# tusen-ai/RangeDet

Hardware: AMD Instinct MI355X
Metric: range-image frames/sec (64x2650, 8ch) at 1/2/4/8 GPU; Meta-Kernel HBM GB/s vs peak (higher is better)
Workload: dtype bf16

## Files before the change

include/rangedet_hip.h:

```cpp
#ifndef RANGEDET_HIP_H_
#define RANGEDET_HIP_H_
#include <stddef.h>
#include <stdint.h>

#ifdef __cplusplus
extern "C" {
#endif

#define RD_OK 0
#define RD_EINVAL (-1)
#define RD_ESHAPE (-2)
#define RD_EWORKSPACE (-3)
#define RD_EHIP (-4)

#define RD_F32 0
#define RD_BF16 1
#define RD_F16 2

#define RD_RELU_PRE 1
#define RD_ADD 2
#define RD_RELU_POST 4
#define RD_SCALE_FOLDED 8
#define RD_MFMA16 16

int rd_version(void);
const char* rd_last_error_string(void);

int rd_nchw_to_nhwc(const float* src, void* dst, int B, int C, int H, int W, int dst_cstride, int dst_coff,
                    int zero_pad, int dst_dtype, void* stream);
int rd_nhwc_to_nchw(const void* src, float* dst, int B, int C, int H, int W, int src_cstride, int src_coff,
                    int src_dtype, void* stream);

int rd_copy_rows(const void* src, long src_row_bytes, void* dst, long dst_row_bytes, long dst_offset_bytes, long bytes,
                 int rows, void* stream);

size_t rd_conv_packed_bytes(int ntaps, int cin, int cout, int dtype);
int rd_pack_conv_weight_host(const float* w_oihw_host, int cout, int cin, int kh, int kw, int dtype,
                             void* packed_host);
int rd_deconv_phase_taps(int kh, int kw, int stride_w, int pad_w, int phase);
int rd_pack_deconv_weight_host(const float* w_iohw_host, int cin, int cout, int kh, int kw, int stride_w,
                               int pad_w, int phase, int dtype, void* packed_host);
int rd_pack_deconv_weight_folded_host(const float* w_iohw_host, const float* fold_scale_host, int cin, int cout, int kh, int kw,
                                      int stride_w, int pad_w, int phase, int dtype, void* packed_host);

int rd_conv2d_bn_act(const void* x, int x_cstride, int x_coff, const void* w_packed, const float* scale,
                     const float* shift, const void* residual, int r_cstride, int r_coff, void* y,
                     int y_cstride, int y_coff, int B, int H, int Win, int cin, int cout, int kh, int kw,
                     int stride_w, int flags, int dtype, void* stream);
size_t rd_conv3x3_ex_packed_bytes(int cin, int cout, int stride_w, int x_cstride);
int rd_pack_conv3x3_ex_host(const float* w_oihw_host, const float* fold_scale_host, int cout, int cin, int stride_w,
                            int x_cstride, int dtype, void* packed_host);
int rd_pack_conv3x3_m16_host(const float* w_oihw_host, const float* fold_scale_host, int cout, int cin, int dtype, void* packed_host);
int rd_conv3x3_mfma16_ok(int cin, int cout, int stride_w, int W, int fused_output_conv);
size_t rd_conv1x1_sc_packed_bytes(int cin, int cout);
int rd_pack_conv1x1_sc_host(const float* w_oi_host, const float* fold_scale_host, int cout, int cin, int dtype,
                            void* packed_host);
int rd_conv3x3_bn_act_ex(const void* x, int x_cstride, int x_coff, const void* w_packed, const float* scale, const float* shift,
                         const void* residual, int r_cstride, int r_coff, const void* sc_x, int sc_cstride, int sc_coff,
                         int sc_cin, const void* sc_w_packed, void* y, int y_cstride, int y_coff, int B, int H, int Win, int cin,
                         int cout, int stride_w, int flags, int dtype, void* stream);
size_t rd_block64_packed_bytes(int cin);
int rd_pack_block64_host(const float* w1_oihw_host, const float* fold_scale1_host, const float* w2_oihw_host,
                         const float* fold_scale2_host, int cin, int dtype, void* packed_host);
int rd_block64_bn_act(const void* x, int x_cstride, int x_coff, int cin, const void* w_packed, const float* shift1, const float* shift2,
                      const void* sc_w_packed, void* y, int y_cstride, int y_coff, int B, int H, int W, int dtype, void* stream);
int rd_pack_block64_m16_host(const float* w1_oihw_host, const float* fold_scale1_host, const float* w2_oihw_host,
                             const float* fold_scale2_host, int dtype, void* packed_host);
int rd_pack_conv1x1_sc_m16_host(const float* w_oi_host, const float* fold_scale_host, int dtype, void* packed_host);
int rd_block64_m16_bn_act(const void* x, int x_cstride, int x_coff, const void* w_packed, const float* shift1, const float* shift2,
                          const void* sc_w_packed, void* y, int y_cstride, int y_coff, int B, int H, int W, int dtype, void* stream);

size_t rd_head_packed_bytes(void);
int rd_pack_head_weight_host(const float* w, int nout, int cin, int dtype, void* out_host);
size_t rd_head_m16_packed_bytes(void);
int rd_pack_head_weight_m16_host(const float* w, int nout, int cin, int dtype, void* out_host);
int rd_conv2d_bn_act_head_out(const void* x, int x_cstride, int x_coff, const void* w_packed, const float* scale,
                              const float* shift, int B, int H, int W, int cin, int flags, const void* head_w_packed,
                              const float* head_bias, float* out, long out_batch_stride, long n_off, int nout, int dtype,
                              void* stream);

int rd_conv3x3_bn_act_pair(const void* x0, int x0_coff, const void* w0_packed, const float* shift0, void* y0, int y0_coff,
                           const void* x1, int x1_coff, const void* w1_packed, const float* shift1, void* y1, int y1_coff,
                           int x_cstride, int y_cstride, int B, int H, int W, int cin, int flags, int dtype, void* stream);
int rd_conv2d_bn_act_head_out_pair(const void* x0, int x0_coff, const void* w0_packed, const float* shift0, const void* head_w0_packed,
                                   const float* head_bias0, float* out0, long out0_batch_stride, int nout0,
                                   const void* x1, int x1_coff, const void* w1_packed, const float* shift1, const void* head_w1_packed,
                                   const float* head_bias1, float* out1, long out1_batch_stride, int nout1,
                                   int x_cstride, long n_off, int B, int H, int W, int cin, int flags, int dtype, void* stream);

size_t rd_conv3x3_cat_packed_bytes(int cin1, int cin2, int cout);
int rd_pack_conv3x3_cat_host(const float* w, const float* fold_scale, int cout, int cin1, int cin2, int dtype, void* out_host);
int rd_conv3x3_bn_act_cat(const void* x1, int x1_cstride, int x1_coff, int cin1, const void* x2, int x2_cstride, int x2_coff, int cin2,
                          const void* w_packed, const float* shift, void* y, int y_cstride, int y_coff, int B, int H, int W, int cout,
                          int flags, int dtype, void* stream);

int rd_deconv2d_bn_act(const void* x, int x_cstride, int x_coff, const void* w_packed_phase,
                       const float* scale, const float* shift, const void* residual, int r_cstride,
                       int r_coff, void* y, int y_cstride, int y_coff, int B, int H, int Win, int cin,
                       int cout, int kh, int kw, int stride_w, int pad_w, int phase, int flags, int dtype,
                       void* stream);

int rd_deconv2d_all_phases_ok(int kh, int kw, int stride_w, int pad_w, int cout, int dtype);
int rd_deconv2d_bn_act_all(const void* x, int x_cstride, int x_coff, const void* w_packed_all, long w_phase_bytes,
                           const float* shift, const void* residual, int r_cstride, int r_coff, void* y, int y_cstride,
                           int y_coff, int B, int H, int Win, int cin, int cout, int kh, int kw, int stride_w, int pad_w,
                           int flags, int dtype, void* stream);

int rd_deconv2d_phase_pairs_ok(int kh, int kw, int stride_w, int pad_w, int cout, int dtype);
int rd_pack_deconv_phase_pair_host(const void* phase_a, const void* phase_b, int cin, int dtype, void* out);
int rd_deconv2d_bn_act_pairs(const void* x, int x_cstride, int x_coff, const void* w_packed_pairs, long w_pair_bytes,
                             const float* shift2, const void* residual, int r_cstride, int r_coff, void* y, int y_cstride,
                             int y_coff, int B, int H, int Win, int cin, int cout, int kh, int kw, int stride_w, int pad_w,
                             int flags, int dtype, void* stream);

int rd_head_out(const void* x, int x_cstride, int x_coff, const float* w, const float* bias, float* out,
                long out_batch_stride, long n_off, int B, int H, int W, int cin, int nout, int dtype,
                void* stream);

size_t rd_meta_packed_bytes(int dtype);
int rd_pack_meta_host(const float* w0, const float* b0, const float* w1, const float* b1, const float* s1,
                      const float* t1, const float* agg, const float* s2, const float* t2, int dtype,
                      void* packed_host);
int rd_meta_kernel_fwd(const void* data, int d_cstride, int d_coff, const float* coord_nchw,
                       const void* packed, void* y, int y_cstride, int y_coff, int B, int H, int W, int dtype,
                       void* stream);

size_t rd_sorted_foreground_workspace_bytes(long N, long k);
int rd_sorted_foreground(const float* cls_score, const float* bbox_delta, const float* pc, const float* mask,
                         int B, long N, long k, int D, int apply_sigmoid, float* out_score, float* out_delta,
                         float* out_pc, int* out_idx, void* ws, size_t ws_bytes, void* stream);

int rd_decode3d_bbox(const float* bbox_delta, const float* pc, float* out, int B, long N, int box_type,
                     int is_bin, void* stream);

size_t rd_score_filter_workspace_bytes(long n);
int rd_score_filter_dets(const float* scores, const float* boxes10, long n, float min_score, float* dets,
                         int* d_count, void* ws, size_t ws_bytes, void* stream);
int rd_score_filter_dets_batched(const float* scores, long scores_bstride, const float* boxes10, long boxes_bstride,
                                 long n, float min_score, float* dets, long dets_bstride, int* d_count, void* ws,
                                 size_t ws_bytes, int B, void* stream);

#define RD_WNMS_MAX_K 65536
#define RD_TIE_STABLE 0
#define RD_TIE_REFERENCE 1
#define RD_WNMS_DIAG_NO_SKIP 0x100
#define RD_WNMS_DIAG_TILE_W(n) (((n) & 0xff) << 16)
#define RD_WNMS_DIAG_MERGE_LDS(n) (((n) & 0x7f) << 24)
size_t rd_wnms_workspace_bytes(int Kcap);
int rd_wnms_4c(const float* dets, int Kcap, const int* d_count, const int* order, int tie_order, float thresh,
               float thresh_vote, int is3d, int hash_scale, float* out_dets, int* keep, int* d_nkeep, void* ws,
               size_t ws_bytes, void* stream);
int rd_wnms_4c_batched(const float* dets, long dets_bstride, int Kcap, const int* d_count, const int* order,
                       long order_bstride, int tie_order, float thresh, float thresh_vote, int is3d, int hash_scale,
                       float* out_dets, long out_bstride, int* keep, long keep_bstride, int* d_nkeep, void* ws,
                       size_t ws_bytes, int B, void* stream);
int rd_single_overlap(const float* dets_a, const float* dets_b, long n, int is3d, float* out, void* stream);
int rd_wnms_pair_skippable(const float* dets_a, const float* dets_b, long n, unsigned char* out, void* stream);

int rd_edge_atan2f(const float* y, const float* x, long n, float* out, void* stream);

int rd_wnms_order_host(const float* dets_host, int K, int* order_host);

int rd_dets12_to_8(const float* dets12, int Mcap, const int* d_count, float* out8, void* stream);
int rd_dets12_to_8_batched(const float* dets12, long dets12_bstride, int Mcap, const int* d_count, float* out8,
                           long out8_bstride, int B, void* stream);

int rd_rotated_iou_8pt(const float* boxes1, const float* boxes2, float* ious, long n1, long n2, void* stream);
int rd_batch_rotated_iou(const float* proposal, int p_stride, const float* gt_bbox, float* iou_map, int* argmax, int B, long N,
                         int n_gt, void* stream);
int rd_batch_rotated_iou_3d(const float* proposal, int p_stride, const float* gt_bbox7, float* iou_map, int* argmax, int B, long N,
                            int n_gt, void* stream);
int rd_rotated_iou_7(const float* boxes1, const float* boxes2, float* ious, long n1, long n2, void* stream);
int rd_batch_max_iou(const float* proposals, int p_stride, const float* gt8, float* out, long n, int n_gt,
                     void* stream);

size_t rd_nms3d_workspace_bytes(long N, int B);
int rd_gather_keep_scores(const float* score, long score_bstride, int k, const int* keep_idx, int max_keep, float* out, int B,
                          void* stream);
int rd_nms3d(const float* boxes, int B, long N, float iou_thres, int max_keep, int normal_iou, int* keep_idx,
             float* bbox_after_nms, void* ws, size_t ws_bytes, void* stream);

int rd_assign3d_v2(const float* pc, const float* bbox, const float* bbox_center, const float* bbox_radius, const float* mask,
                   const float* is_in_nlz, long N, int M, float max_x, float min_x, float max_y, float min_y, float max_z,
                   float min_z, float max_dist, int* out, void* stream);
size_t rd_get_point_num_workspace_bytes(void);
int rd_get_point_num(const float* bbox_inds, long N, float* out, void* ws, size_t ws_bytes, void* stream);

typedef struct {
  float clip_lo[7], clip_hi[7];
  float mean[8], sd[8];
  float interval_lo[3], interval_hi[3];
} rd_input_norm_t;
int rd_input_transform(const float* range_image, const float* pc_vehicle_frame, const float* inclination,
                       const rd_input_norm_t* norm_host, int B, int H, int W, int Hp, int Wp, float* input_data,
                       float* coord_s1, float* pc_s1, float* pc_s2, float* pc_s4, float* mask_s1, float* mask_s2,
                       float* mask_s4, void* stream);

#define RD_PROF_CONV 0
#define RD_PROF_META 1
#define RD_PROF_HEAD_OUT 2
#define RD_PROF_SORT 3
#define RD_PROF_DECODE 4
#define RD_PROF_WNMS 5
#define RD_PROF_LAYOUT 6
#define RD_PROF_CONV3 7
#define RD_PROF_BLOCK 8
#define RD_PROF_NKINDS 9
int rd_prof_enable(int on);
int rd_prof_reset(void);
int rd_prof_get(int kind, double* total_ms, long* launches);

#ifdef __cplusplus
}
#endif
#endif
```

rangedet_amd/csrc/k_block.h:

```cpp
#pragma once
#include "k_conv3.h"

namespace rd {

struct BlockArgs {
  const bf16_t* x; int x_cs, x_co; long x_bs;
  const unsigned char* w;
  const float* shift1; const float* shift2;
  const unsigned char* scw;
  bf16_t* y; int y_cs, y_co; long y_bs;
  const unsigned char* zero16;
  int H, W, B, ncol, nrow, ntiles, xcd;
  int nslots1;
};

constexpr int BK_R = 6;
constexpr int BK_XP = 36;
constexpr int BK_XPIECES = 7;
constexpr int BK_BUF = 4 * BK_XPIECES * 1024;
constexpr int BK_TP = 34;
constexpr int BK_SLAB = 4096;
constexpr size_t BK_LDS = 2 * BK_BUF + BK_R * BK_SLAB;

constexpr int bk_nsteps(bool first) { return first ? 23 : 36; }
constexpr int bk_unit(bool first, int g) { return first ? (g < 5 ? 0 : g < 14 ? 2 : 3) : g / 9; }
constexpr int bk_ord(bool first, int g) { return first ? (g < 5 ? g : (g - 5) % 9) : g % 9; }
constexpr bool bk_fetches(bool first, int g) { return bk_unit(first, g) == 3 || (!first && bk_unit(first, g) == 0); }
constexpr int bk_pieces_u(int s) { return s <= 1 ? 2 : s <= 4 ? 1 : 0; }
constexpr int bk_first_u(int s) { int n = 0; for (int t = 0; t < s; ++t) n += bk_pieces_u(t); return n; }
constexpr int bk_pieces(bool first, int g) { return bk_fetches(first, g) ? bk_pieces_u(bk_ord(first, g)) : 0; }
constexpr int bk_younger(bool first, int g) {
  const int G = bk_nsteps(first);
  int n = BK_R - 3;
  for (int d = 1; d <= BK_R - 2; ++d) n += bk_pieces(first, ((g - d) % G + G) % G);
  const int cap = 9 - 3 - 4;
  return (bk_fetches(first, g) && bk_ord(first, g) == 7 && n > cap) ? cap : n;
}

template <int DT, bool SC, bool FIRST = false, bool M16 = false>
__global__ __launch_bounds__(256, 2) void block64_stream_kernel(BlockArgs a) {
  static_assert(!FIRST || SC, "the first block changes the channel count: projection shortcut");
  static_assert(!(FIRST && M16), "the first block (five two-tap steps on one 16-channel slot) stays in the 32 x 32 x 16 form");
  HIP_DYNAMIC_SHARED(unsigned char, smem);
  constexpr int R = BK_R, SLAB = BK_SLAB, RING = 2 * BK_BUF, NCT = 2;
  constexpr int ROWB2 = BK_TP * 64;
  const int tid = threadIdx.x, lane = tid & 63, wave = __builtin_amdgcn_readfirstlane(tid >> 6);
  const int m = lane & 31, hi = lane >> 5;

  unsigned bz1[NCT], bz2[NCT];
#pragma unroll
  for (int j = 0; j < NCT; ++j) {
    const float t1 = a.shift1[32 * j + conv_row_perm(m)], t2 = a.shift2[32 * j + conv_row_perm(m)];
    const bf16_t h1 = H16<DT>::from_f32(t1), h2 = H16<DT>::from_f32(t2);
    const bf16_t l1 = H16<DT>::from_f32(t1 - H16<DT>::to_f32(h1)), l2 = H16<DT>::from_f32(t2 - H16<DT>::to_f32(h2));
    bz1[j] = hi ? 0u : ((unsigned)h1 | ((unsigned)l1 << 16));
    bz2[j] = hi ? 0u : ((unsigned)h2 | ((unsigned)l2 << 16));
  }

  unsigned bz1m = 0u, bz2m = 0u;
  if constexpr (M16) {
    const float t1 = a.shift1[conv_row16(lane >> 4, lane & 15)], t2 = a.shift2[conv_row16(lane >> 4, lane & 15)];
    const bf16_t h1 = H16<DT>::from_f32(t1), h2 = H16<DT>::from_f32(t2);
    const bf16_t l1 = H16<DT>::from_f32(t1 - H16<DT>::to_f32(h1)), l2 = H16<DT>::from_f32(t2 - H16<DT>::to_f32(h2));
    bz1m = (unsigned)h1 | ((unsigned)l1 << 16);
    bz2m = (unsigned)h2 | ((unsigned)l2 << 16);
  }

  const int G = gridDim.x, wg = blockIdx.x;
  const int ntl = (a.ntiles - wg + G - 1) / G;
  const int tiles_img = a.ncol * a.nrow;

#if defined(__HIP_DEVICE_COMPILE__)
  const unsigned lds0 = __builtin_amdgcn_readfirstlane((unsigned)(uintptr_t)(__attribute__((address_space(3))) void*)smem);
#endif
  auto dma_s = [&](const unsigned char* sbase, unsigned voff, int lds_off) {
#if defined(__HIP_DEVICE_COMPILE__)
    asm volatile("s_mov_b32 m0, %2\n\ts_nop 0\n\tglobal_load_lds_dwordx4 %0, %1"
                 :: "v"(voff), "s"(sbase), "s"(__builtin_amdgcn_readfirstlane(lds0 + (unsigned)lds_off)) : "memory");
#else
    __builtin_amdgcn_global_load_lds(sbase + voff, smem + lds_off, 16, 0, 0);
#endif
  };
  auto dma_v = [&](const void* vptr, int lds_off) {
#if defined(__HIP_DEVICE_COMPILE__)
    asm volatile("s_mov_b32 m0, %1\n\ts_nop 0\n\tglobal_load_lds_dwordx4 %0, off"
                 :: "v"(vptr), "s"(__builtin_amdgcn_readfirstlane(lds0 + (unsigned)lds_off)) : "memory");
#else
    __builtin_amdgcn_global_load_lds(vptr, smem + lds_off, 16, 0, 0);
#endif
  };

  const int xdq = (G >> 3) / a.nrow;
  const int g_ct = a.xcd ? (8 * xdq) % a.ncol : G % a.ncol, g_rb = a.xcd ? (G >> 3) % a.nrow : (G / a.ncol) % a.nrow,
            g_b = a.xcd ? (8 * xdq) / a.ncol : G / tiles_img;
  const int g_ct1 = (8 * xdq + 8) % a.ncol, g_b1 = (8 * xdq + 8) / a.ncol;
  auto tile_advance = [&](int& ct, int& rb, int& b) __attribute__((always_inline)) {
    int& d0 = a.xcd ? rb : ct;
    int& d1 = a.xcd ? ct : rb;
    const int r0 = a.xcd ? a.nrow : a.ncol, r1 = a.xcd ? a.ncol : a.nrow;
    d0 += a.xcd ? g_rb : g_ct;
    const int c1 = d0 >= r0 ? 1 : 0;
    d0 -= c1 ? r0 : 0;
    d1 += a.xcd ? (c1 ? g_ct1 : g_ct) : g_rb + c1;
    const int c2 = d1 >= r1 ? 1 : 0;
    d1 -= c2 ? r1 : 0;
    b += (a.xcd && c1 ? g_b1 : g_b) + c2;
  };
  const int xs0 = ((wg >> 3) / a.nrow) * 8 + (wg & 7);
  int f_ct = a.xcd ? xs0 % a.ncol : wg % a.ncol, f_rb = a.xcd ? (wg >> 3) % a.nrow : (wg / a.ncol) % a.nrow,
      f_b = a.xcd ? xs0 / a.ncol : wg / tiles_img;
  int c_ct = f_ct, c_rb = f_rb, c_b = f_b;

  int hk = 0, hc = 0;
  int hh0 = 0, hw0 = 0;
  const unsigned char* htile = nullptr;
  const unsigned char* hbase = nullptr;
  bool hnew = true;
  auto halo_begin = [&]() {
    if (hnew) {
      hh0 = f_rb * 8 - 2; hw0 = f_ct * 32 - 2;
      htile = (const unsigned char*)(a.x + (size_t)f_b * a.x_bs + a.x_co) + ((long)hh0 * a.W + hw0) * (long)a.x_cs * 2;
      hnew = false;
    }
    hbase = htile + hc * 64;
    if (!FIRST && hc == 0) hc = 1;
    else if (hk + 1 < ntl) { ++hk; hc = 0; tile_advance(f_ct, f_rb, f_b); hnew = true; }
  };
  auto halo_piece = [&](int buf, int j) {
    const int q = wave * BK_XPIECES + j;
    int ol = lane;
    asm volatile("" : "+v"(ol));
    const int pp = 16 * q + (ol >> 2), r = (pp * 1821) >> 16, cc = pp - BK_XP * r;
    const int hs = (ol & 3) ^ ((ol >> 4) & 3);
    const bool ok = pp < 12 * BK_XP && (unsigned)(hh0 + r) < (unsigned)a.H && (unsigned)(hw0 + cc) < (unsigned)a.W && (!FIRST || hs < a.nslots1);
    const unsigned char* src = hbase + (long)((r * a.W + cc) * a.x_cs * 2 + hs * 16);
    dma_v(ok ? (const void*)src : (const void*)a.zero16, buf + q * 1024);
  };
  int fslot = 0, fslab = 0;
  auto slab_piece = [&]() { dma_s(a.w + (size_t)fslab * SLAB + wave * 1024, lane * 16, RING + fslot * SLAB + wave * 1024); };
  auto slab_advance = [&]() {
    fslot = fslot + 1 == R ? 0 : fslot + 1;
    fslab = fslab + 1 == bk_nsteps(FIRST) ? 0 : fslab + 1;
  };

  int a1[3][3], a2[3];
#pragma unroll
  for (int dh = 0; dh < 3; ++dh)
#pragma unroll
    for (int dw = 0; dw < 3; ++dw) {
      const int P = 96 * wave + m + BK_XP * dh + dw;
      a1[dh][dw] = P * 64 + (((hi ^ (P >> 2)) & 3) << 4);
    }
#pragma unroll
  for (int d = 0; d < 3; ++d) {
    const int c = d + m;
    a2[d] = c * 64 + (((hi ^ (c >> 2)) & 3) << 4) + wave * 2 * ROWB2;
  }
  if constexpr (M16) {
    const int n16 = lane & 15, q16 = lane >> 4;
#pragma unroll
    for (int dh = 0; dh < 3; ++dh)
#pragma unroll
      for (int dw = 0; dw < 3; ++dw) {
        const int P = 96 * wave + n16 + BK_XP * dh + dw;
        a1[dh][dw] = P * 64 + (((q16 ^ (P >> 2)) & 3) << 4);
      }
#pragma unroll
    for (int d = 0; d < 3; ++d) {
      const int c = d + n16;
      a2[d] = c * 64 + (((q16 ^ (c >> 2)) & 3) << 4) + wave * 2 * ROWB2;
    }
  }
  const int boff = RING + lane * 16;

  f32x16 acc[M16 ? 1 : 3][M16 ? 1 : NCT];
  f32x4 acc6[M16 ? 6 : 1][M16 ? 4 : 1];
  s16x8 fa[2][3], fb[2][NCT];
  s16x8 fa16[6];
#define BK_FENCE() __builtin_amdgcn_sched_barrier(0)
#define BK_RD(F, FS, BUF, K, AADDR, BADDR, KS)                                                              \
  {                                                                                                         \
    if ((K) == 0) fa[BUF][0] = *(const s16x8*)(smem + (AADDR));                                              \
    else if ((K) <= NCT) fb[BUF][(K) - 1] = *(const s16x8*)(smem + (BADDR) + ((KS) * NCT + (K) - 1) * 1024);  \
    else fa[BUF][(K) - NCT] = *(const s16x8*)(smem + (AADDR) + ((K) - NCT) * (FS));                          \
    BK_FENCE();                                                                                             \
  }
#define BK_MM(BUF, N)                                                                                       \
  {                                                                                                         \
    acc[(N) / NCT][(N) % NCT] = H16<DT>::mfma(fb[BUF][(N) % NCT], fa[BUF][(N) / NCT], acc[(N) / NCT][(N) % NCT]); \
    BK_FENCE();                                                                                             \
  }
#define BK_SYNC(VMCNT, LGKM)                                      \
  {                                                               \
    asm volatile("" ::: "memory");                                \
    __builtin_amdgcn_s_waitcnt(C3_WAIT_IMM(VMCNT, LGKM));         \
    __builtin_amdgcn_s_barrier();                                 \
    asm volatile("" ::: "memory");                                \
    BK_FENCE();                                                   \
  }
#define BK_STEP(F, FS, G_, HB_, NF_, NFS_, A1_, ANEXT_)                                                            \
  {                                                                                                                \
    constexpr int NM_ = (F) * NCT, NR_ = (F) + NCT, NRN_ = (NF_) ? (NF_) + NCT : 0;                                \
    constexpr int NH_ = bk_pieces(FIRST, G_), NP_ = 1 + NH_, HF_ = bk_first_u(bk_ord(FIRST, G_)), YG_ = bk_younger(FIRST, G_); \
    const int acur_ = (A1_);                                                                                       \
    const int bcur_ = boff + rslot * SLAB;                                                                         \
    const int rnext_ = rslot + 1 == R ? 0 : rslot + 1;                                                             \
    const int anext_ = (ANEXT_);                                                                                   \
    const int bnext_ = boff + rnext_ * SLAB;                                                                       \
    BK_FENCE();                                                                                                    \
    _Pragma("unroll") for (int n = 0; n < NM_; ++n) {                                                              \
      BK_MM(0, n)                                                                                                  \
      if (n < NR_) BK_RD(F, FS, 1, n, acur_, bcur_, 1)                                                             \
    }                                                                                                              \
    _Pragma("unroll") for (int n = 0; n < NM_ / 2; ++n) {                                                          \
      BK_MM(1, n)                                                                                                  \
      if (n < NRN_) BK_RD(NF_, NFS_, 0, n, anext_, bnext_, 0)                                                      \
    }                                                                                                              \
    { _Pragma("unroll") for (int n = NM_ / 2; n < NRN_; ++n) BK_RD(NF_, NFS_, 0, n, anext_, bnext_, 0) }           \
    BK_SYNC(YG_, NRN_)                                                                                             \
    if (NH_ > 0 && bk_ord(FIRST, G_) == 0) halo_begin();                                                           \
    _Pragma("unroll") for (int n = NM_ / 2; n < NM_; ++n) {                                                        \
      BK_MM(1, n)                                                                                                  \
      _Pragma("unroll") for (int p = 0; p < NP_; ++p)                                                              \
        if (p * (NM_ / 2) / NP_ == n - NM_ / 2) {                                                                  \
          if (p == 0) slab_piece(); else halo_piece(HB_, HF_ + p - 1);                                             \
          BK_FENCE();                                                                                              \
        }                                                                                                          \
    }                                                                                                              \
    slab_advance();                                                                                                \
    rslot = rnext_;                                                                                                \
  }
#define BK_C1(U_, S_)                                                                                              \
  BK_STEP(3, 2048, 9 * (U_) + (S_), BK_BUF, (((U_) == 1 && (S_) == 8) ? 0 : 3), 2048,                              \
          (a1[(S_) / 3][(S_) % 3] + (U_) * BK_BUF) ^ 32,                                                           \
          ((S_) == 8 ? a1[0][0] + BK_BUF : a1[(((S_) + 1) % 9) / 3][((S_) + 1) % 3] + (U_) * BK_BUF))
#define BK_P1(S_)                                                                                                  \
  BK_STEP(3, 2048, (S_), 0, ((S_) == 4 ? 0 : 3), 2048, a1[((2 * (S_) + 1) % 9) / 3][(2 * (S_) + 1) % 3],           \
          a1[((2 * (S_) + 2) % 9) / 3][(2 * (S_) + 2) % 3])
#define BK_C2(C_, S_)                                                                                              \
  BK_STEP(2, ROWB2, (FIRST ? 5 : 18) + 9 * (C_) + (S_), 0, (((C_) == 1 && (S_) == 8) ? 3 : 2), (((C_) == 1 && (S_) == 8) ? 2048 : ROWB2), \
          (a2[(S_) % 3] + ((S_) / 3) * ROWB2 + (C_) * BK_BUF) ^ 32,                                                \
          ((S_) == 8 ? ((C_) == 1 ? a1[0][0] : a2[0] + BK_BUF) : a2[((S_) + 1) % 3] + ((((S_) + 1) % 9) / 3) * ROWB2 + (C_) * BK_BUF))

#define BK_RDW16(BUF, C, BADDR) { fb[BUF][C] = *(const s16x8*)(smem + (BADDR) + (C) * 1024); BK_FENCE(); }
#define BK_RDP16(HX, AADDR, FS) { fa16[HX] = *(const s16x8*)(smem + (AADDR) + ((HX) >> 1) * (FS) + ((HX) & 1) * 1024); BK_FENCE(); }
#define BK_MM16(BK, N)                                                                                             \
  {                                                                                                                \
    acc6[(N) >> 1][2 * (BK) + ((N) & 1)] = H16<DT>::mfma16(fb[BK][(N) & 1], fa16[(N) >> 1], acc6[(N) >> 1][2 * (BK) + ((N) & 1)]); \
    BK_FENCE();                                                                                                    \
  }
#define BK_STEP16(F, G_, HB_, NF_, NFS_, ANEXT_)                                                                   \
  {                                                                                                                \
    constexpr int NM_ = 2 * (F);                                                                                   \
    constexpr int NX_ = (NF_) > (F) ? (NF_) - (F) : 0;                                                             \
    constexpr int LG_ = (NF_) ? 2 + NX_ + ((NF_) < (F) / 2 ? (NF_) : (F) / 2) : 0;                                 \
    constexpr int NH_ = bk_pieces(FIRST, G_), NP_ = 1 + NH_, HF_ = bk_first_u(bk_ord(FIRST, G_)), YG_ = bk_younger(FIRST, G_); \
    const int bcur_ = boff + rslot * SLAB;                                                                         \
    const int rnext_ = rslot + 1 == R ? 0 : rslot + 1;                                                             \
    const int anext_ = (ANEXT_);                                                                                   \
    const int bnext_ = boff + rnext_ * SLAB;                                                                       \
    BK_FENCE();                                                                                                    \
    _Pragma("unroll") for (int n = 0; n < NM_; ++n) {                                                              \
      BK_MM16(0, n)                                                                                                \
      if (n < 2) BK_RDW16(1, n, bcur_ + 2048)                                                                      \
    }                                                                                                              \
    _Pragma("unroll") for (int n = 0; n < NM_ / 2; ++n) {                                                          \
      BK_MM16(1, n)                                                                                                \
      if ((NF_) && n < 2) BK_RDW16(0, n, bnext_)                                                                   \
      if (n < NX_) BK_RDP16((F) + n, anext_, NFS_)                                                                 \
      if ((n & 1) && (n >> 1) < (NF_)) BK_RDP16(n >> 1, anext_, NFS_)                                              \
    }                                                                                                              \
    BK_SYNC(YG_, LG_)                                                                                              \
    if (NH_ > 0 && bk_ord(FIRST, G_) == 0) halo_begin();                                                           \
    _Pragma("unroll") for (int n = NM_ / 2; n < NM_; ++n) {                                                        \
      BK_MM16(1, n)                                                                                                \
      _Pragma("unroll") for (int p = 0; p < NP_; ++p)                                                              \
        if (p * (NM_ / 2) / NP_ == n - NM_ / 2) {                                                                  \
          if (p == 0) slab_piece(); else halo_piece(HB_, HF_ + p - 1);                                             \
          BK_FENCE();                                                                                              \
        }                                                                                                          \
      if ((n & 1) && (n >> 1) < (NF_) && (n >> 1) < (F)) BK_RDP16(n >> 1, anext_, NFS_)                            \
    }                                                                                                              \
    slab_advance();                                                                                                \
    rslot = rnext_;                                                                                                \
  }
#define BK_C1M(U_, S_)                                                                                             \
  BK_STEP16(6, 9 * (U_) + (S_), BK_BUF, (((U_) == 1 && (S_) == 8) ? 0 : 6), 2048,                                  \
            ((S_) == 8 ? a1[0][0] + BK_BUF : a1[(((S_) + 1) % 9) / 3][((S_) + 1) % 3] + (U_) * BK_BUF))
#define BK_C2M(C_, S_)                                                                                             \
  BK_STEP16(4, 18 + 9 * (C_) + (S_), 0, (((C_) == 1 && (S_) == 8) ? 6 : 4), (((C_) == 1 && (S_) == 8) ? 2048 : ROWB2), \
            ((S_) == 8 ? ((C_) == 1 ? a1[0][0] : a2[0] + BK_BUF) : a2[((S_) + 1) % 3] + ((((S_) + 1) % 9) / 3) * ROWB2 + (C_) * BK_BUF))

  halo_begin();
#pragma unroll
  for (int j = 0; j < BK_XPIECES; ++j) halo_piece(0, j);
#pragma unroll 1
  for (int s0 = 0; s0 < R; ++s0) { slab_piece(); slab_advance(); }
  BK_SYNC(0, 0)
  int rslot = 0;
  if constexpr (M16) {
#pragma unroll
    for (int kk = 0; kk < 2; ++kk) BK_RDW16(0, kk, boff + rslot * SLAB)
#pragma unroll
    for (int kk = 0; kk < 6; ++kk) BK_RDP16(kk, a1[0][0], 2048)
  } else {
#pragma unroll
  for (int kk = 0; kk < 3 + NCT; ++kk) BK_RD(3, 2048, 0, kk, a1[0][0], boff + rslot * SLAB, 0)
  }

  for (int k = 0; k < ntl; ++k) {
    if constexpr (M16) {
      unsigned z0 = 0u, b1 = bz1m, b2 = bz2m;
      int oq = lane >> 4;
      asm volatile("" : "+v"(z0), "+v"(b1), "+v"(b2), "+v"(oq));
      typedef short s16x2 __attribute__((ext_vector_type(2)));
      typedef float f32x2 __attribute__((ext_vector_type(2)));
      auto init_acc = [&](unsigned bz, int NH) {
#pragma unroll
        for (int cb = 0; cb < 4; ++cb) {
          unsigned ob[4] = {oq == cb ? H16<DT>::ONE * 0x10001u : z0, z0, z0, z0};
          unsigned ab[4] = {bz, z0, z0, z0};
          s16x8 ones, bzv;
          memcpy(&ones, ob, 16);
          memcpy(&bzv, ab, 16);
          acc6[0][cb] = H16<DT>::mfma16(bzv, ones, f32x4{});
          BK_FENCE();
        }
#pragma unroll
        for (int h = 1; h < 6; ++h)
          if (h < NH) {
#pragma unroll
            for (int cb = 0; cb < 4; ++cb) acc6[h][cb] = acc6[0][cb];
          }
        BK_FENCE();
      };
      init_acc(b1, 6);
      BK_C1M(0, 0) BK_C1M(0, 1) BK_C1M(0, 2) BK_C1M(0, 3) BK_C1M(0, 4) BK_C1M(0, 5) BK_C1M(0, 6) BK_C1M(0, 7) BK_C1M(0, 8)
      BK_C1M(1, 0) BK_C1M(1, 1) BK_C1M(1, 2) BK_C1M(1, 3) BK_C1M(1, 4) BK_C1M(1, 5) BK_C1M(1, 6) BK_C1M(1, 7) BK_C1M(1, 8)
      const int ct = c_ct, rb = c_rb, b = c_b;
      tile_advance(c_ct, c_rb, c_b);
      {
        int el = lane;
        asm volatile("" : "+v"(el));
        const int en = el & 15, eq = el >> 4;
#pragma unroll
        for (int h = 0; h < 6; ++h) {
          const int J = 96 * wave + 16 * h + en, rr = (J * 1821) >> 16, cc = J - BK_XP * rr;
          const bool keep = cc < BK_TP && rr < 10;
          const bool inside = (unsigned)(rb * 8 - 1 + rr) < (unsigned)a.H && (unsigned)(ct * 32 - 1 + cc) < (unsigned)a.W;
          const int doff = (rr * BK_TP + cc) * 64 + (((eq ^ (cc >> 2)) & 3) << 4);
#pragma unroll
          for (int j = 0; j < 2; ++j) {
            BK_FENCE();
            unsigned pk[4];
#pragma unroll
            for (int w2 = 0; w2 < 4; ++w2) {
              const f32x4 av = acc6[h][2 * j + (w2 >> 1)];
              unsigned p2 = H16<DT>::pk(av[2 * (w2 & 1)], av[2 * (w2 & 1) + 1]);
              p2 = __builtin_bit_cast(unsigned, __builtin_elementwise_max(__builtin_bit_cast(s16x2, p2), (s16x2){0, 0}));
              pk[w2] = inside ? p2 : 0u;
            }
            if (keep) *(Slot16*)(smem + j * BK_BUF + doff) = Slot16{pk[0], pk[1], pk[2], pk[3]};
          }
        }
      }
      init_acc(b2, 4);
      BK_SYNC(63, 0)
#pragma unroll
      for (int kk = 0; kk < 2; ++kk) BK_RDW16(0, kk, boff + rslot * SLAB)
#pragma unroll
      for (int kk = 0; kk < 4; ++kk) BK_RDP16(kk, a2[0], ROWB2)
      BK_C2M(0, 0) BK_C2M(0, 1) BK_C2M(0, 2) BK_C2M(0, 3) BK_C2M(0, 4) BK_C2M(0, 5) BK_C2M(0, 6) BK_C2M(0, 7) BK_C2M(0, 8)
      BK_C2M(1, 0) BK_C2M(1, 1) BK_C2M(1, 2) BK_C2M(1, 3) BK_C2M(1, 4) BK_C2M(1, 5) BK_C2M(1, 6) BK_C2M(1, 7) BK_C2M(1, 8)
      {
        const int oh0 = rb * 8 + 2 * wave;
        int el = lane;
        asm volatile("" : "+v"(el));
        const int en = el & 15, eq = el >> 4;
        unsigned char* scr = smem + BK_BUF + wave * (BK_BUF / 4);
        bf16_t* __restrict__ yrow0 = a.y + (size_t)b * a.y_bs + (size_t)oh0 * a.W * a.y_cs + a.y_co;
        const bf16_t* __restrict__ rimg0 = a.x + (size_t)b * a.x_bs + a.x_co;
        if constexpr (SC) {
          const unsigned char* __restrict__ wq = a.scw + el * 16;
          s16x8 sxq[4][2];
#pragma unroll
          for (int h = 0; h < 4; ++h) {
            const int ow = ct * 32 + 16 * (h & 1) + en, oh = oh0 + (h >> 1);
            const bool live = ow < a.W && oh < a.H;
            const bf16_t* sp = rimg0 + (live ? ((size_t)oh * a.W + ow) * a.x_cs : 0) + 8 * eq;
#pragma unroll
            for (int ks = 0; ks < 2; ++ks) sxq[h][ks] = *(const s16x8*)(sp + 32 * ks);
          }
#pragma unroll
          for (int ks = 0; ks < 2; ++ks)
#pragma unroll
            for (int cb = 0; cb < 4; ++cb) {
              const s16x8 wf = *(const s16x8*)(wq + (size_t)(ks * 4 + cb) * 1024);
#pragma unroll
              for (int h = 0; h < 4; ++h) acc6[h][cb] = H16<DT>::mfma16(wf, sxq[h][ks], acc6[h][cb]);
            }
          BK_FENCE();
        }
        Slot16 rv[2][2][2];
        auto res_load = [&](int i, Slot16 (&dst)[2][2]) {
#pragma unroll
          for (int hf = 0; hf < 2; ++hf) {
            const int ow = ct * 32 + 16 * hf + en, oh = oh0 + i;
            const bool live = ow < a.W && oh < a.H;
            const bf16_t* rp = rimg0 + (live ? ((size_t)oh * a.W + (size_t)ow) * a.x_cs : 0) + 8 * eq;
#pragma unroll
            for (int p2 = 0; p2 < 2; ++p2) dst[hf][p2] = *(const Slot16*)(rp + 32 * p2);
          }
        };
        if constexpr (!SC) res_load(0, rv[0]);
#pragma unroll
        for (int i = 0; i < 2; ++i) {
          if constexpr (!SC) { if (i + 1 < 2) res_load(i + 1, rv[(i + 1) & 1]); }
#pragma unroll
          for (int hf = 0; hf < 2; ++hf)
#pragma unroll
            for (int p2 = 0; p2 < 2; ++p2) {
              BK_FENCE();
              unsigned pk[4];
#pragma unroll
              for (int w2 = 0; w2 < 4; ++w2) {
                const f32x4 av = acc6[2 * i + hf][2 * p2 + (w2 >> 1)];
                f32x2 v = {av[2 * (w2 & 1)], av[2 * (w2 & 1) + 1]};
                if constexpr (!SC) v += H16<DT>::unpk(rv[i & 1][hf][p2][w2]);
                const unsigned q2 = H16<DT>::pk(v[0], v[1]);
                pk[w2] = __builtin_bit_cast(unsigned, __builtin_elementwise_max(__builtin_bit_cast(s16x2, q2), (s16x2){0, 0}));
              }
              const int px = 16 * hf + en;
              *(Slot16*)(scr + px * 128 + (((4 * p2 + eq) ^ (px & 7)) << 4)) = Slot16{pk[0], pk[1], pk[2], pk[3]};
            }
          BK_FENCE();
          __builtin_amdgcn_wave_barrier();
#pragma unroll
          for (int it = 0; it < 4; ++it) {
            const int pr = it * 8 + el / 8, sl = el % 8;
            const Slot16 v = *(const Slot16*)(scr + pr * 128 + ((sl ^ (pr & 7)) << 4));
            const int ows = ct * 32 + pr;
            if (ows < a.W && oh0 + i < a.H)
              __builtin_nontemporal_store(v, (Slot16*)(yrow0 + (size_t)i * a.W * a.y_cs + (size_t)ows * a.y_cs + sl * 8));
          }
          __builtin_amdgcn_wave_barrier();
          BK_FENCE();
        }
      }
    } else {
    unsigned z0 = 0u;
    asm volatile("" : "+v"(z0));
    const unsigned one2 = hi ? z0 : H16<DT>::ONE * 0x10001u;
    s16x8 ones;
    {
      unsigned ob[4] = {one2, z0, z0, z0};
      memcpy(&ones, ob, 16);
    }
#pragma unroll
    for (int n = 0; n < 3 * NCT; ++n) {
      unsigned ab[4] = {bz1[n % NCT], z0, z0, z0};
      s16x8 bz;
      memcpy(&bz, ab, 16);
      acc[n / NCT][n % NCT] = H16<DT>::mfma(bz, ones, f32x16{});
    }
    BK_FENCE();
    if constexpr (FIRST) {
      BK_P1(0) BK_P1(1) BK_P1(2) BK_P1(3) BK_P1(4)
    } else {
      BK_C1(0, 0) BK_C1(0, 1) BK_C1(0, 2) BK_C1(0, 3) BK_C1(0, 4) BK_C1(0, 5) BK_C1(0, 6) BK_C1(0, 7) BK_C1(0, 8)
      BK_C1(1, 0) BK_C1(1, 1) BK_C1(1, 2) BK_C1(1, 3) BK_C1(1, 4) BK_C1(1, 5) BK_C1(1, 6) BK_C1(1, 7) BK_C1(1, 8)
    }

    const int ct = c_ct, rb = c_rb, b = c_b;
    tile_advance(c_ct, c_rb, c_b);
    {
      int em = m, ehi = hi;
      asm volatile("" : "+v"(em), "+v"(ehi));
      typedef short s16x2 __attribute__((ext_vector_type(2)));
#pragma unroll
      for (int i = 0; i < 3; ++i) {
        const int J = 96 * wave + 32 * i + em, rr = (J * 1821) >> 16, cc = J - BK_XP * rr;
        const bool keep = cc < BK_TP && rr < 10;
        const bool inside = (unsigned)(rb * 8 - 1 + rr) < (unsigned)a.H && (unsigned)(ct * 32 - 1 + cc) < (unsigned)a.W;
        const int doff = (rr * BK_TP + cc) * 64 + ((((2 * ehi) ^ (cc >> 2)) & 3) << 4);
#pragma unroll
        for (int j = 0; j < NCT; ++j) {
          BK_FENCE();
          unsigned pk[8];
#pragma unroll
          for (int q = 0; q < 8; ++q) {
            unsigned p2 = H16<DT>::pk(acc[i][j][2 * q], acc[i][j][2 * q + 1]);
            p2 = __builtin_bit_cast(unsigned, __builtin_elementwise_max(__builtin_bit_cast(s16x2, p2), (s16x2){0, 0}));
            pk[q] = inside ? p2 : 0u;
          }
          if (keep) {
            *(Slot16*)(smem + j * BK_BUF + doff) = Slot16{pk[0], pk[1], pk[2], pk[3]};
            *(Slot16*)(smem + j * BK_BUF + (doff ^ 16)) = Slot16{pk[4], pk[5], pk[6], pk[7]};
          }
        }
      }
    }
#pragma unroll
    for (int n = 0; n < 2 * NCT; ++n) {
      unsigned ab[4] = {bz2[n % NCT], z0, z0, z0};
      s16x8 bz;
      memcpy(&bz, ab, 16);
      acc[n / NCT][n % NCT] = H16<DT>::mfma(bz, ones, f32x16{});
    }
    BK_FENCE();
    BK_SYNC(63, 0)
#pragma unroll
    for (int kk = 0; kk < 2 + NCT; ++kk) BK_RD(2, ROWB2, 0, kk, a2[0], boff + rslot * SLAB, 0)
    BK_C2(0, 0) BK_C2(0, 1) BK_C2(0, 2) BK_C2(0, 3) BK_C2(0, 4) BK_C2(0, 5) BK_C2(0, 6) BK_C2(0, 7) BK_C2(0, 8)
    BK_C2(1, 0) BK_C2(1, 1) BK_C2(1, 2) BK_C2(1, 3) BK_C2(1, 4) BK_C2(1, 5) BK_C2(1, 6) BK_C2(1, 7) BK_C2(1, 8)

    {
      const int oh0 = rb * 8 + 2 * wave;
      int em = m, ehi = hi, el = lane;
      asm volatile("" : "+v"(em), "+v"(ehi), "+v"(el));
      typedef float f32x2 __attribute__((ext_vector_type(2)));
      typedef short s16x2 __attribute__((ext_vector_type(2)));
      unsigned char* scr = smem + BK_BUF + wave * (BK_BUF / 4);
      bf16_t* __restrict__ yrow0 = a.y + (size_t)b * a.y_bs + (size_t)oh0 * a.W * a.y_cs + a.y_co;
      const bf16_t* __restrict__ rimg0 = a.x + (size_t)b * a.x_bs + a.x_co;
      if constexpr (SC) {
        const bf16_t* __restrict__ sb = a.x + (size_t)b * a.x_bs + a.x_co + 8 * ehi;
        const unsigned char* __restrict__ wq = a.scw + el * 16;
        constexpr int SNK = FIRST ? 1 : 4;
        s16x8 sxq[2][SNK];
#pragma unroll
        for (int i = 0; i < 2; ++i) {
          const int ow = ct * 32 + em, oh = oh0 + i;
          const bool live = ow < a.W && oh < a.H;
          const bf16_t* sp = sb + (live ? ((size_t)oh * a.W + ow) * a.x_cs : 0);
#pragma unroll
          for (int ks = 0; ks < SNK; ++ks) sxq[i][ks] = *(const s16x8*)(sp + 16 * ks);
        }
#pragma unroll
        for (int ks = 0; ks < SNK; ++ks)
#pragma unroll
          for (int j = 0; j < NCT; ++j) {
            const s16x8 wf = *(const s16x8*)(wq + (size_t)(ks * NCT + j) * 1024);
#pragma unroll
            for (int i = 0; i < 2; ++i) acc[i][j] = H16<DT>::mfma(wf, sxq[i][ks], acc[i][j]);
          }
        BK_FENCE();
      }
      Slot16 rv[2][NCT][2];
      auto res_load = [&](int i, Slot16 (&dst)[NCT][2]) {
        const int ow = ct * 32 + em, oh = oh0 + i;
        const bool live = ow < a.W && oh < a.H;
        const bf16_t* rp = rimg0 + (live ? ((size_t)oh * a.W + (size_t)ow) * a.x_cs : 0) + 16 * ehi;
#pragma unroll
        for (int j = 0; j < NCT; ++j) {
          dst[j][0] = *(const Slot16*)(rp + j * 32);
          dst[j][1] = *(const Slot16*)(rp + j * 32 + 8);
        }
      };
      if constexpr (!SC) res_load(0, rv[0]);
#pragma unroll
      for (int i = 0; i < 2; ++i) {
        if constexpr (!SC) { if (i + 1 < 2) res_load(i + 1, rv[(i + 1) & 1]); }
#pragma unroll
        for (int j = 0; j < NCT; ++j) {
          BK_FENCE();
          const int cb = j * 32 + 16 * ehi;
          unsigned pk[8];
#pragma unroll
          for (int q = 0; q < 8; ++q) {
            f32x2 v = {acc[i][j][2 * q], acc[i][j][2 * q + 1]};
            if constexpr (!SC) v += H16<DT>::unpk(rv[i & 1][j][q >> 2][q & 3]);
            unsigned p2 = H16<DT>::pk(v[0], v[1]);
            pk[q] = __builtin_bit_cast(unsigned, __builtin_elementwise_max(__builtin_bit_cast(s16x2, p2), (s16x2){0, 0}));
          }
#pragma unroll
          for (int u = 0; u < 2; ++u)
            *(Slot16*)(scr + em * 128 + ((((cb >> 3) + u) ^ (em & 7)) << 4)) = Slot16{pk[4 * u], pk[4 * u + 1], pk[4 * u + 2], pk[4 * u + 3]};
        }
        BK_FENCE();
        __builtin_amdgcn_wave_barrier();
#pragma unroll
        for (int it = 0; it < 4; ++it) {
          const int pr = it * 8 + el / 8, sl = el % 8;
          const Slot16 v = *(const Slot16*)(scr + pr * 128 + ((sl ^ (pr & 7)) << 4));
          const int ows = ct * 32 + pr;
          if (ows < a.W && oh0 + i < a.H)
            __builtin_nontemporal_store(v, (Slot16*)(yrow0 + (size_t)i * a.W * a.y_cs + (size_t)ows * a.y_cs + sl * 8));
        }
        __builtin_amdgcn_wave_barrier();
        BK_FENCE();
      }
    }
    }
  }
  __builtin_amdgcn_s_waitcnt(RD_VMCNT_IMM(0));
#undef BK_C2M
#undef BK_C1M
#undef BK_STEP16
#undef BK_MM16
#undef BK_RDP16
#undef BK_RDW16
#undef BK_C2
#undef BK_P1
#undef BK_C1
#undef BK_STEP
#undef BK_SYNC
#undef BK_MM
#undef BK_RD
#undef BK_FENCE
}

inline bool block64_first(int cin) { return cin <= 16; }
inline size_t block64_body_bytes(int cin) { return (size_t)bk_nsteps(block64_first(cin)) * BK_SLAB; }
inline size_t block64_packed_bytes(int cin) { return block64_body_bytes(cin) + RD_CONV_TAIL; }
inline void pack_block64_m16(const float* w1, const float* s1, const float* w2, const float* s2, int dt, void* out) {
  memset(out, 0, block64_packed_bytes(64));
  pack_taps_frag16(9, 64, 64, out, [&](int co, int ci, int t) { return (s1 ? s1[co] : 1.f) * w1[((size_t)co * 64 + ci) * 9 + t]; }, dt);
  pack_taps_frag16(9, 64, 64, (unsigned char*)out + 18 * BK_SLAB, [&](int co, int ci, int t) { return (s2 ? s2[co] : 1.f) * w2[((size_t)co * 64 + ci) * 9 + t]; }, dt);
}
inline void pack_sc_frag16(const float* w, const float* scale, void* out, int dt = RD_BF16) {
  bf16_t* o = (bf16_t*)out;
  for (int ks = 0; ks < 2; ++ks)
    for (int cb = 0; cb < 4; ++cb)
      for (int lane = 0; lane < 64; ++lane) {
        const int co = conv_row16(cb, lane & 15);
        for (int j = 0; j < 8; ++j) {
          const int ci = 32 * ks + 8 * (lane >> 4) + j;
          *o++ = h16_from_f32(dt, (scale ? scale[co] : 1.f) * w[(size_t)co * 64 + ci]);
        }
      }
}
inline void pack_block64(const float* w1, const float* s1, const float* w2, const float* s2, int cin, int dt, void* out) {
  memset(out, 0, block64_packed_bytes(cin));
  if (block64_first(cin))
    pack_body_frag(3, cin, 64, out, [&](int co, int ci, int dh, int dw) { return (s1 ? s1[co] : 1.f) * w1[(((size_t)co * cin + ci) * 3 + dh) * 3 + dw]; }, dt);
  else
    pack_taps_frag(9, 64, 64, out, [&](int co, int ci, int t) { return (s1 ? s1[co] : 1.f) * w1[((size_t)co * 64 + ci) * 9 + t]; }, dt);
  pack_taps_frag(9, 64, 64, (unsigned char*)out + block64_body_bytes(cin) - 18 * BK_SLAB,
                 [&](int co, int ci, int t) { return (s2 ? s2[co] : 1.f) * w2[((size_t)co * 64 + ci) * 9 + t]; }, dt);
}

inline int launch_block64(const void* x, int x_cs, int x_co, int cin, const void* w, const float* shift1, const float* shift2, const void* sc_w,
                          void* y, int y_cs, int y_co, int B, int H, int W, int dt, hipStream_t st, bool m16 = false) {
  RD_REQUIRE(is_h16(dt), RD_EINVAL, "block64: dtype %d (RD_BF16 or RD_F16)", dt);
  const bool first = block64_first(cin);
  RD_REQUIRE(!m16 || !first, RD_ESHAPE, "block64: the 16 x 16 x 32 form takes 64 input channels");
  RD_REQUIRE(cin == 64 || (first && cin >= 1), RD_ESHAPE, "block64: %d input channels (64, or at most 16 for the network's first block)", cin);
  RD_REQUIRE(!first || sc_w, RD_EINVAL, "block64: a block that changes the channel count needs its projection shortcut");
  BlockArgs a;
  memset(&a, 0, sizeof(a));
  a.x = (const bf16_t*)x; a.x_cs = x_cs; a.x_co = x_co; a.x_bs = (long)H * W * x_cs;
  a.w = (const unsigned char*)w; a.shift1 = shift1; a.shift2 = shift2; a.scw = (const unsigned char*)sc_w;
  a.y = (bf16_t*)y; a.y_cs = y_cs; a.y_co = y_co; a.y_bs = (long)H * W * y_cs;
  a.zero16 = (const unsigned char*)w + block64_body_bytes(cin);
  a.H = H; a.W = W; a.B = B;
  a.nslots1 = std::min(2, (x_cs - x_co) / 8);
  a.ncol = (W + 31) / 32; a.nrow = (H + 7) / 8; a.ntiles = a.ncol * a.nrow * B;
  const int grid = std::min(a.ntiles, conv_num_cus() * 2);
  a.xcd = dev_switches().conv_xcd && (a.ncol * B) % 8 == 0 && grid % 8 == 0;
  ProfScope ps(RD_PROF_BLOCK, st);
  static std::atomic<unsigned long long> seen{0};
  once_per_device(seen, [] {
    allow_big_lds(block64_stream_kernel<RD_F16, false>); allow_big_lds(block64_stream_kernel<RD_BF16, false>);
    allow_big_lds(block64_stream_kernel<RD_F16, true>); allow_big_lds(block64_stream_kernel<RD_BF16, true>);
    allow_big_lds(block64_stream_kernel<RD_F16, true, true>); allow_big_lds(block64_stream_kernel<RD_BF16, true, true>);
    allow_big_lds(block64_stream_kernel<RD_F16, false, false, true>); allow_big_lds(block64_stream_kernel<RD_BF16, false, false, true>);
    allow_big_lds(block64_stream_kernel<RD_F16, true, false, true>); allow_big_lds(block64_stream_kernel<RD_BF16, true, false, true>);
  });
#define BK_GO(DT_)                                                                                                         \
  {                                                                                                                        \
    if (m16 && sc_w) hipLaunchKernelGGL((block64_stream_kernel<DT_, true, false, true>), dim3(grid), dim3(256), BK_LDS, st, a);  \
    else if (m16) hipLaunchKernelGGL((block64_stream_kernel<DT_, false, false, true>), dim3(grid), dim3(256), BK_LDS, st, a);    \
    else if (first) hipLaunchKernelGGL((block64_stream_kernel<DT_, true, true>), dim3(grid), dim3(256), BK_LDS, st, a);    \
    else if (sc_w) hipLaunchKernelGGL((block64_stream_kernel<DT_, true>), dim3(grid), dim3(256), BK_LDS, st, a);           \
    else hipLaunchKernelGGL((block64_stream_kernel<DT_, false>), dim3(grid), dim3(256), BK_LDS, st, a);                    \
  }
  if (dt == RD_F16) BK_GO(RD_F16) else BK_GO(RD_BF16)
#undef BK_GO
  return check_launch("block64_stream_kernel");
}

}
```

rangedet_amd/csrc/rd_api.hip:

```cpp
#include "k_conv1.h"
#include "k_block.h"
#include "k_assign.h"
#include "k_input.h"
#include "k_nms3d.h"
#include "k_meta.h"
#include "k_misc.h"
#include "k_riou.h"
#include "k_sort.h"
#include "k_wnms.h"

#include <algorithm>
#include <string>
#include <numeric>

using namespace rd;

namespace rd {
inline size_t align256(size_t v) { return (v + 255) & ~(size_t)255; }
inline size_t wnms_ws_bytes(int cap) {
  const size_t nw = (size_t)(cap + 63) / 64;
  return align256((size_t)cap * PREP_F * 4) + 3 * align256((size_t)cap * nw * 8) + 4 * align256((size_t)cap * 4) +
         align256(((size_t)cap + 2) * 8 + 3 * ((size_t)cap / 32 + 2) * 4) + align256(nw * 8) + 256 + align256(sort_ws_bytes(cap)) + 256;
}
inline WnmsWs wnms_ws_carve(void* ws, int cap) {
  WnmsWs w;
  const size_t nw = (size_t)(cap + 63) / 64;
  unsigned char* p = (unsigned char*)(((uintptr_t)ws + 255) & ~(uintptr_t)255);
  w.nwcap = (int)nw;
  w.prep = (float*)p; p += align256((size_t)cap * PREP_F * 4);
  w.thr = (unsigned long long*)p; p += align256((size_t)cap * nw * 8);
  w.vote = (unsigned long long*)p; p += align256((size_t)cap * nw * 8);
  w.snap = (unsigned long long*)p; p += align256((size_t)cap * nw * 8);
  w.keep_q = (int*)p; p += align256((size_t)cap * 4);
  w.order = (int*)p; p += align256((size_t)cap * 4);
  w.alive = (int*)p; p += align256((size_t)cap * 4);
  w.ovf = (int*)p; p += align256((size_t)cap * 4);
  w.scratch = (int*)p; p += align256(((size_t)cap + 2) * 8 + 3 * ((size_t)cap / 32 + 2) * 4);
  w.supp_state = (unsigned long long*)p; p += align256(nw * 8);
  w.nalive = (int*)p; w.novf = (int*)p + 1; p += 256;
  w.sort_ws = p;
  return w;
}
inline void allow_conv_lds() {
  static std::atomic<unsigned long long> seen{0};
  once_per_device(seen, [] {
    allow_big_lds(conv_taps_kernel<RD_BF16, 4, 3>); allow_big_lds(conv_taps_kernel<RD_BF16, 4, 8>);
    allow_big_lds(conv_taps_kernel<RD_F16, 4, 3>); allow_big_lds(conv_taps_kernel<RD_F16, 4, 8>);
    allow_big_lds(conv_taps_kernel<RD_F32, 4, 8>); allow_big_lds(conv_taps_kernel<RD_F32, 4, 3>);
  });
}
}

extern "C" {

int rd_version(void) { return 100; }
const char* rd_last_error_string(void) { return rd::err_buf(); }

int rd_nchw_to_nhwc(const float* src, void* dst, int B, int C, int H, int W, int dst_cstride, int dst_coff,
                    int zero_pad, int dst_dtype, void* stream) {
  RD_REQUIRE(src && dst, RD_EINVAL, "nchw_to_nhwc: null pointer");
  RD_REQUIRE(B > 0 && C > 0 && H > 0 && W > 0 && zero_pad >= 0, RD_ESHAPE, "nchw_to_nhwc: bad shape");
  RD_REQUIRE(dst_coff >= 0 && dst_coff + C + zero_pad <= dst_cstride, RD_ESHAPE, "nchw_to_nhwc: channels exceed stride");
  hipStream_t st = (hipStream_t)stream;
  const long HW = (long)H * W, total = (long)B * (C + zero_pad) * HW;
  const int grid = (int)std::min<long>((total + 255) / 256, 8192);
  ProfScope ps(RD_PROF_LAYOUT, st);
  {
    const int ch = ch_per_slot(dst_dtype), ctot = C + zero_pad;
    if ((is_h16(dst_dtype) || dst_dtype == RD_F32) && ctot % ch == 0 && ctot / ch <= 2 && dst_cstride % ch == 0 && dst_coff % ch == 0) {
      const long npix = (long)B * HW;
      const int g2 = (int)std::min<long>((npix + 255) / 256, 8192);
#define RD_PX(DT, NS) hipLaunchKernelGGL((nchw_to_nhwc_px_kernel<DT, NS>), dim3(g2), dim3(256), 0, st, src, dst, C, HW, dst_cstride, dst_coff, npix)
      if (dst_dtype == RD_BF16) { if (ctot / ch == 1) RD_PX(RD_BF16, 1); else RD_PX(RD_BF16, 2); }
      else if (dst_dtype == RD_F16) { if (ctot / ch == 1) RD_PX(RD_F16, 1); else RD_PX(RD_F16, 2); }
      else { if (ctot / ch == 1) RD_PX(RD_F32, 1); else RD_PX(RD_F32, 2); }
#undef RD_PX
      return check_launch("nchw_to_nhwc");
    }
  }
  if (dst_dtype == RD_BF16)
    hipLaunchKernelGGL(nchw_to_nhwc_kernel<RD_BF16>, dim3(grid), dim3(256), 0, st, src, dst, C, HW, dst_cstride, dst_coff, zero_pad, total);
  else if (dst_dtype == RD_F16)
    hipLaunchKernelGGL(nchw_to_nhwc_kernel<RD_F16>, dim3(grid), dim3(256), 0, st, src, dst, C, HW, dst_cstride, dst_coff, zero_pad, total);
  else if (dst_dtype == RD_F32)
    hipLaunchKernelGGL(nchw_to_nhwc_kernel<RD_F32>, dim3(grid), dim3(256), 0, st, src, dst, C, HW, dst_cstride, dst_coff, zero_pad, total);
  else
    return rd::fail(RD_EINVAL, "nchw_to_nhwc: dtype %d", dst_dtype);
  return check_launch("nchw_to_nhwc");
}
int rd_copy_rows(const void* src, long src_row_bytes, void* dst, long dst_row_bytes, long dst_offset_bytes, long bytes,
                 int rows, void* stream) {
  RD_REQUIRE(src && dst, RD_EINVAL, "copy_rows: null pointer");
  RD_REQUIRE(rows > 0 && bytes > 0 && src_row_bytes >= bytes && dst_row_bytes >= dst_offset_bytes + bytes && dst_offset_bytes >= 0,
             RD_ESHAPE, "copy_rows: bad geometry");
  ProfScope ps(RD_PROF_LAYOUT, (hipStream_t)stream);
  if (hipMemcpy2DAsync((char*)dst + dst_offset_bytes, (size_t)dst_row_bytes, src, (size_t)src_row_bytes, (size_t)bytes,
                       (size_t)rows, hipMemcpyDeviceToDevice, (hipStream_t)stream) != hipSuccess)
    return rd::fail(RD_EHIP, "copy_rows: hipMemcpy2DAsync failed");
  return RD_OK;
}
int rd_nhwc_to_nchw(const void* src, float* dst, int B, int C, int H, int W, int src_cstride, int src_coff,
                    int src_dtype, void* stream) {
  RD_REQUIRE(src && dst, RD_EINVAL, "nhwc_to_nchw: null pointer");
  RD_REQUIRE(B > 0 && C > 0 && H > 0 && W > 0, RD_ESHAPE, "nhwc_to_nchw: bad shape");
  RD_REQUIRE(src_coff >= 0 && src_coff + C <= src_cstride, RD_ESHAPE, "nhwc_to_nchw: channels exceed stride");
  hipStream_t st = (hipStream_t)stream;
  const long HW = (long)H * W, total = (long)B * C * HW;
  const int grid = (int)std::min<long>((total + 255) / 256, 8192);
  ProfScope ps(RD_PROF_LAYOUT, st);
  if (src_dtype == RD_BF16)
    hipLaunchKernelGGL(nhwc_to_nchw_kernel<RD_BF16>, dim3(grid), dim3(256), 0, st, src, dst, C, HW, src_cstride, src_coff, total);
  else if (src_dtype == RD_F16)
    hipLaunchKernelGGL(nhwc_to_nchw_kernel<RD_F16>, dim3(grid), dim3(256), 0, st, src, dst, C, HW, src_cstride, src_coff, total);
  else if (src_dtype == RD_F32)
    hipLaunchKernelGGL(nhwc_to_nchw_kernel<RD_F32>, dim3(grid), dim3(256), 0, st, src, dst, C, HW, src_cstride, src_coff, total);
  else
    return rd::fail(RD_EINVAL, "nhwc_to_nchw: dtype %d", src_dtype);
  return check_launch("nhwc_to_nchw");
}

size_t rd_conv_packed_bytes(int ntaps, int cin, int cout, int dtype) { return conv_packed_bytes(ntaps, cin, cout, dtype); }
int rd_pack_conv_weight_host(const float* w, int cout, int cin, int kh, int kw, int dtype, void* out) {
  RD_REQUIRE(w && out, RD_EINVAL, "pack_conv: null pointer");
  RD_REQUIRE(dtype == RD_F32 || is_h16(dtype), RD_EINVAL, "pack_conv: dtype");
  RD_REQUIRE(kh * kw >= 1 && kh * kw <= 9 && (kh & 1) && (kw & 1), RD_ESHAPE, "pack_conv: kernel (%d,%d)", kh, kw);
  TapList tl = conv_taps(kh, kw);
  auto get = [&](int co, int ci, int t) { return w[(((size_t)co * cin + ci) * kh + tl.kh[t]) * kw + tl.kw[t]]; };
  memset(out, 0, conv_packed_bytes(tl.n, cin, cout, dtype));
  if (is_h16(dtype)) pack_taps_frag(tl.n, cin, cout, out, get, dtype);
  else pack_taps(tl.n, cin, cout, dtype, out, get);
  return RD_OK;
}
static bool deconv_embeds_3x3(const TapList& tl) {
  for (int t = 0; t < tl.n; ++t)
    if (tl.dh[t] < -1 || tl.dh[t] > 1 || tl.dw[t] < -1 || tl.dw[t] > 1) return false;
  return tl.n >= 1 && tl.n <= 9;
}
static int deconv_tap_set(const TapList& tl) {
  if (tl.n != 6 || !deconv_embeds_3x3(tl)) return 0;
  for (int ts = 1; ts <= 2; ++ts) {
    bool seen[6] = {false, false, false, false, false, false};
    bool ok = true;
    for (int t = 0; t < 6 && ok; ++t) {
      const int c = tl.dw[t] - (ts == 1 ? -1 : 0);
      if (c < 0 || c > 1) ok = false;
      else seen[(tl.dh[t] + 1) * 2 + c] = true;
    }
    for (int i = 0; i < 6 && ok; ++i) ok = seen[i];
    if (ok) return ts;
  }
  return 0;
}
static TapList deconv_taps_sorted(int kh, int kw, int s, int pad_w, int phase) {
  TapList tl = deconv_taps(kh, kw, s, pad_w, phase);
  if (tl.n > 9) return tl;
  for (int i = 1; i < tl.n; ++i)
    for (int j = i; j > 0 && (tl.dh[j] < tl.dh[j - 1] || (tl.dh[j] == tl.dh[j - 1] && tl.dw[j] < tl.dw[j - 1])); --j) {
      std::swap(tl.dh[j], tl.dh[j - 1]); std::swap(tl.dw[j], tl.dw[j - 1]);
      std::swap(tl.kh[j], tl.kh[j - 1]); std::swap(tl.kw[j], tl.kw[j - 1]);
    }
  return tl;
}
int rd_deconv_phase_taps(int kh, int kw, int stride_w, int pad_w, int phase) {
  if (stride_w < 1 || phase < 0 || phase >= stride_w) return RD_EINVAL;
  TapList tl = deconv_taps(kh, kw, stride_w, pad_w, phase);
  if (tl.n > 9) return RD_ESHAPE;
  return (deconv_embeds_3x3(tl) && !deconv_tap_set(tl)) ? 9 : tl.n;
}
int rd_pack_deconv_weight_host(const float* w, int cin, int cout, int kh, int kw, int stride_w, int pad_w,
                               int phase, int dtype, void* out) {
  return rd_pack_deconv_weight_folded_host(w, nullptr, cin, cout, kh, kw, stride_w, pad_w, phase, dtype, out);
}
int rd_pack_deconv_weight_folded_host(const float* w, const float* fold_scale, int cin, int cout, int kh, int kw, int stride_w,
                                      int pad_w, int phase, int dtype, void* out) {
  RD_REQUIRE(w && out, RD_EINVAL, "pack_deconv: null pointer");
  RD_REQUIRE(dtype == RD_F32 || is_h16(dtype), RD_EINVAL, "pack_deconv: dtype");
  RD_REQUIRE(stride_w >= 1 && phase >= 0 && phase < stride_w, RD_EINVAL, "pack_deconv: phase");
  TapList tl = deconv_taps_sorted(kh, kw, stride_w, pad_w, phase);
  RD_REQUIRE(tl.n >= 1 && tl.n <= 9, RD_ESHAPE, "pack_deconv: %d taps", tl.n);
  const bool emb = deconv_embeds_3x3(tl) && !deconv_tap_set(tl);
  auto get = [&](int co, int ci, int t) -> float {
    if (emb) {
      int src = -1;
      for (int u = 0; u < tl.n; ++u)
        if (tl.dh[u] == t / 3 - 1 && tl.dw[u] == t % 3 - 1) src = u;
      if (src < 0) return 0.f;
      t = src;
    }
    return (fold_scale ? fold_scale[co] : 1.f) * w[(((size_t)ci * cout + co) * kh + tl.kh[t]) * kw + tl.kw[t]];
  };
  const int nt = emb ? 9 : tl.n;
  memset(out, 0, conv_packed_bytes(nt, cin, cout, dtype));
  if (is_h16(dtype)) pack_taps_frag(nt, cin, cout, out, get, dtype);
  else pack_taps(nt, cin, cout, dtype, out, get);
  return RD_OK;
}

int rd_conv2d_bn_act(const void* x, int x_cstride, int x_coff, const void* w_packed, const float* scale,
                     const float* shift, const void* residual, int r_cstride, int r_coff, void* y, int y_cstride,
                     int y_coff, int B, int H, int Win, int cin, int cout, int kh, int kw, int stride_w, int flags,
                     int dtype, void* stream) {
  RD_REQUIRE(x && w_packed && y, RD_EINVAL, "conv2d: null pointer");
  RD_REQUIRE((kh == 1 && kw == 1) || (kh == 3 && kw == 3), RD_ESHAPE, "conv2d: kernel (%d,%d) not in {1x1,3x3}", kh, kw);
  RD_REQUIRE(stride_w == 1 || stride_w == 2, RD_ESHAPE, "conv2d: stride_w %d", stride_w);
  RD_REQUIRE(y_coff >= 0 && y_coff + cout <= y_cstride, RD_ESHAPE, "conv2d: y channels exceed stride");
  const int pad = (kw - 1) / 2;
  const int Wout = (Win + 2 * pad - kw) / stride_w + 1;
  RD_REQUIRE(!(flags & RD_SCALE_FOLDED), RD_EINVAL, "conv2d: RD_SCALE_FOLDED is taken by rd_conv3x3_bn_act_ex / rd_conv2d_bn_act_head_out / rd_deconv2d_bn_act");
  TapList tl = conv_taps(kh, kw);
  allow_conv_lds();
  return launch_conv(tl, x, x_cstride, x_coff, w_packed, scale, shift, residual, r_cstride, r_coff, y, y_cstride,
                     y_coff, B, H, Win, Wout, Wout, cin, cout, stride_w, 1, 0, flags, dtype, (hipStream_t)stream);
}
static int ex_view_cin(int cin, int x_cstride, int stride_w) { return stride_w == 2 ? x_cstride + cin : cin; }
size_t rd_conv3x3_ex_packed_bytes(int cin, int cout, int stride_w, int x_cstride) {
  return conv_packed_bytes(stride_w == 2 ? 6 : 9, ex_view_cin(cin, x_cstride, stride_w), cout, RD_BF16);
}
int rd_pack_conv3x3_ex_host(const float* w, const float* fold_scale, int cout, int cin, int stride_w, int x_cstride, int dtype,
                            void* out) {
  RD_REQUIRE(w && out, RD_EINVAL, "pack_conv3x3_ex: null pointer");
  RD_REQUIRE(is_h16(dtype), RD_EINVAL, "pack_conv3x3_ex: dtype %d (RD_BF16 or RD_F16)", dtype);
  RD_REQUIRE(stride_w == 1 || stride_w == 2, RD_ESHAPE, "pack_conv3x3_ex: stride_w %d", stride_w);
  RD_REQUIRE(cout == 64 || cout == 128, RD_ESHAPE, "pack_conv3x3_ex: cout %d", cout);
  RD_REQUIRE(stride_w == 1 || (x_cstride >= cin && x_cstride % 8 == 0), RD_ESHAPE, "pack_conv3x3_ex: x_cstride %d for cin %d", x_cstride, cin);
  auto wv = [&](int co, int ci, int dh, int dw) {
    return (fold_scale ? fold_scale[co] : 1.f) * w[(((size_t)co * cin + ci) * 3 + (dh + 1)) * 3 + (dw + 1)];
  };
  memset(out, 0, rd_conv3x3_ex_packed_bytes(cin, cout, stride_w, x_cstride));
  auto wv2 = [&](int co, int c2, int dh, int dw2) -> float {
    if (c2 < cin) return dw2 == 0 ? wv(co, c2, dh, 0) : 0.f;
    if (c2 >= x_cstride && c2 - x_cstride < cin) return wv(co, c2 - x_cstride, dh, dw2 == -1 ? -1 : 1);
    return 0.f;
  };
  if (stride_w == 1) {
    if (conv3_body_small(cin, fold_scale != nullptr))
      pack_body_frag(3, cin, cout, out, [&](int co, int ci, int dh, int dw) { return wv(co, ci, dh - 1, dw - 1); }, dtype);
    else
      pack_taps_frag(9, cin, cout, out, [&](int co, int ci, int t) { return wv(co, ci, t / 3 - 1, t % 3 - 1); }, dtype);
  } else if (conv3_body_s2(cin, x_cstride, fold_scale != nullptr)) {
    pack_body_frag(1, x_cstride + cin, cout, out, [&](int co, int c2, int dh, int dw) { return wv2(co, c2, dh - 1, dw - 1); }, dtype);
  } else {
    pack_taps_frag(6, x_cstride + cin, cout, out, [&](int co, int c2, int s) -> float { return wv2(co, c2, s / 2 - 1, s % 2 - 1); }, dtype);
  }
  return RD_OK;
}
int rd_pack_conv3x3_m16_host(const float* w, const float* fold_scale, int cout, int cin, int dtype, void* out) {
  RD_REQUIRE(w && out, RD_EINVAL, "pack_conv3x3_m16: null pointer");
  RD_REQUIRE(is_h16(dtype), RD_EINVAL, "pack_conv3x3_m16: dtype %d (RD_BF16 or RD_F16)", dtype);
  RD_REQUIRE(cout == 128 && cin >= 32 && cin % 32 == 0, RD_ESHAPE, "pack_conv3x3_m16: cout %d (128), cin %d (a multiple of 32)", cout, cin);
  memset(out, 0, rd_conv3x3_ex_packed_bytes(cin, cout, 1, cin));
  pack_taps_frag16(9, cin, cout, out, [&](int co, int ci, int t) {
    return (fold_scale ? fold_scale[co] : 1.f) * w[(((size_t)co * cin + ci) * 3 + t / 3) * 3 + t % 3];
  }, dtype);
  return RD_OK;
}
int rd_conv3x3_mfma16_ok(int cin, int cout, int stride_w, int W, int fused_output_conv) {
  return conv3_mfma16_ok(cin, cout, stride_w, W, fused_output_conv != 0) ? 1 : 0;
}
size_t rd_conv1x1_sc_packed_bytes(int cin, int cout) { return sc_frag_bytes(cin, cout); }
int rd_pack_conv1x1_sc_host(const float* w, const float* fold_scale, int cout, int cin, int dtype, void* out) {
  RD_REQUIRE(w && out, RD_EINVAL, "pack_conv1x1_sc: null pointer");
  RD_REQUIRE(is_h16(dtype), RD_EINVAL, "pack_conv1x1_sc: dtype %d (RD_BF16 or RD_F16)", dtype);
  RD_REQUIRE((cout == 64 || cout == 128) && cin >= 1 && cin <= 128, RD_ESHAPE, "pack_conv1x1_sc: cout %d, cin %d (1..128)", cout, cin);
  pack_sc_frag(w, fold_scale, cin, cout, out, dtype);
  return RD_OK;
}
int rd_conv3x3_bn_act_ex(const void* x, int x_cstride, int x_coff, const void* w_packed, const float* scale, const float* shift,
                         const void* residual, int r_cstride, int r_coff, const void* sc_x, int sc_cstride, int sc_coff,
                         int sc_cin, const void* sc_w_packed, void* y, int y_cstride, int y_coff, int B, int H, int Win, int cin,
                         int cout, int stride_w, int flags, int dtype, void* stream) {
  RD_REQUIRE(x && w_packed && y, RD_EINVAL, "conv3x3_ex: null pointer");
  RD_REQUIRE(is_h16(dtype), RD_EINVAL, "conv3x3_ex: dtype %d (RD_BF16 or RD_F16)", dtype);
  RD_REQUIRE(B > 0 && H > 0 && Win > 0 && cin > 0 && (cout == 64 || cout == 128), RD_ESHAPE, "conv3x3_ex: shape / cout %d", cout);
  RD_REQUIRE(stride_w == 1 || (stride_w == 2 && Win % 2 == 0), RD_ESHAPE, "conv3x3_ex: stride_w %d with Win %d (stride 2 needs an even width)", stride_w, Win);
  RD_REQUIRE(y_coff >= 0 && y_coff + cout <= y_cstride, RD_ESHAPE, "conv3x3_ex: y channels exceed stride");
  RD_REQUIRE(x_cstride % 8 == 0 && x_coff % 8 == 0 && x_coff + cin_slots(cin, RD_BF16) * 8 <= x_cstride, RD_ESHAPE, "conv3x3_ex: x channel stride/offset");
  RD_REQUIRE(!(sc_x && residual) && !(sc_x && !sc_w_packed), RD_EINVAL, "conv3x3_ex: shortcut conv and residual are exclusive");
  RD_REQUIRE(!((flags & RD_ADD) && !residual && !sc_x), RD_EINVAL, "conv3x3_ex: RD_ADD without residual / shortcut");
  RD_REQUIRE(!dev_switches().conv_v1, RD_EINVAL, "conv3x3_ex: needs the persistent 3x3 kernel (RD_CONV_V1 is set)");
  allow_conv_lds();
  const int v = stride_w;
  const int Wv = Win / v;
  Conv3Args e;
  memset(&e, 0, sizeof(e));
  int fl = flags;
  if (sc_x) {
    RD_REQUIRE(sc_cin >= 1 && sc_cin <= 128 && sc_cstride % 8 == 0 && sc_coff % 8 == 0 && sc_coff + ((sc_cin + 15) / 16) * 16 <= sc_cstride,
               RD_ESHAPE, "conv3x3_ex: shortcut input channels %d (stride %d, offset %d)", sc_cin, sc_cstride, sc_coff);
    e.sx = (const bf16_t*)sc_x; e.s_cs = sc_cstride * v; e.s_co = sc_coff; e.s_bs = (long)H * Wv * sc_cstride * v;
    e.scw = (const unsigned char*)sc_w_packed; e.s_nks = (sc_cin + 15) / 16;
    fl &= ~RD_ADD;
    fl |= RD_SCALE_FOLDED;
  }
  RD_REQUIRE(!(fl & RD_SCALE_FOLDED) || !scale, RD_EINVAL, "conv3x3_ex: folded weights take no scale array");
  const bool m16 = (fl & RD_MFMA16) != 0;
  fl &= ~RD_MFMA16;
  const bool folded = (fl & RD_SCALE_FOLDED) != 0;
  RD_REQUIRE(!m16 || (folded && !sc_x && conv3_mfma16_ok(cin, cout, stride_w, Win, false)), RD_ESHAPE,
             "conv3x3_ex: RD_MFMA16 takes folded weights of rd_pack_conv3x3_m16_host: stride 1, cout 128, cin a multiple of 32, no fused shortcut (rd_conv3x3_mfma16_ok)");
  const int body = m16 ? C3_BODY_M16 : stride_w == 2 ? conv3_body_s2(cin, x_cstride, folded) : (sc_x ? 0 : conv3_body_small(cin, folded));
  RD_REQUIRE(!(stride_w == 1 && sc_x && conv3_body_small(cin, folded)), RD_ESHAPE, "conv3x3_ex: at most 16 input channels together with a fused shortcut is not a launch form");
  return launch_conv3(x, x_cstride * v, x_coff, w_packed, scale, shift, residual, r_cstride, r_coff, y, y_cstride, y_coff, B, H,
                      Wv, ex_view_cin(cin, x_cstride, stride_w), cout, fl, 1, (hipStream_t)stream, stride_w == 2 ? 1 : 0,
                      sc_x ? &e : nullptr, dtype, nullptr, nullptr, nullptr, body);
}

size_t rd_block64_packed_bytes(int cin) { return block64_packed_bytes(cin); }
int rd_pack_block64_host(const float* w1, const float* fold_scale1, const float* w2, const float* fold_scale2, int cin, int dtype, void* out) {
  RD_REQUIRE(w1 && w2 && out, RD_EINVAL, "pack_block64: null pointer");
  RD_REQUIRE(is_h16(dtype), RD_EINVAL, "pack_block64: dtype %d (RD_BF16 or RD_F16)", dtype);
  RD_REQUIRE(cin == 64 || (cin >= 1 && cin <= 16), RD_ESHAPE, "pack_block64: %d input channels (64, or at most 16)", cin);
  pack_block64(w1, fold_scale1, w2, fold_scale2, cin, dtype, out);
  return RD_OK;
}
int rd_block64_bn_act(const void* x, int x_cstride, int x_coff, int cin, const void* w_packed, const float* shift1, const float* shift2,
                      const void* sc_w_packed, void* y, int y_cstride, int y_coff, int B, int H, int W, int dtype, void* stream) {
  RD_REQUIRE(x && w_packed && shift1 && shift2 && y, RD_EINVAL, "block64: null pointer");
  RD_REQUIRE(is_h16(dtype), RD_EINVAL, "block64: dtype %d (RD_BF16 or RD_F16)", dtype);
  RD_REQUIRE(B > 0 && H > 0 && W > 0, RD_ESHAPE, "block64: shape");
  RD_REQUIRE(cin == 64 || (cin >= 1 && cin <= 16), RD_ESHAPE, "block64: %d input channels (64, or at most 16 for the network's first block)", cin);
  RD_REQUIRE(x_cstride % 8 == 0 && x_coff % 8 == 0 && x_coff >= 0 && x_coff + cin_slots(cin, RD_BF16) * 8 <= x_cstride, RD_ESHAPE, "block64: x channel stride / offset");
  RD_REQUIRE(cin > 16 || x_coff + 16 <= x_cstride, RD_ESHAPE, "block64: the first block reads 16 channels per pixel (x_coff %d + 16 > x_cstride %d)", x_coff, x_cstride);
  RD_REQUIRE(y_cstride % 8 == 0 && y_coff % 8 == 0 && y_coff >= 0 && y_coff + 64 <= y_cstride, RD_ESHAPE, "block64: y channel stride / offset");
  RD_REQUIRE(x != y, RD_EINVAL, "block64: in-place (a tile's halo is another tile's output)");
  return launch_block64(x, x_cstride, x_coff, cin, w_packed, shift1, shift2, sc_w_packed, y, y_cstride, y_coff, B, H, W, dtype, (hipStream_t)stream);
}

int rd_pack_block64_m16_host(const float* w1, const float* fold_scale1, const float* w2, const float* fold_scale2, int dtype, void* out) {
  RD_REQUIRE(w1 && w2 && out, RD_EINVAL, "pack_block64_m16: null pointer");
  RD_REQUIRE(is_h16(dtype), RD_EINVAL, "pack_block64_m16: dtype %d (RD_BF16 or RD_F16)", dtype);
  pack_block64_m16(w1, fold_scale1, w2, fold_scale2, dtype, out);
  return RD_OK;
}
int rd_pack_conv1x1_sc_m16_host(const float* w, const float* fold_scale, int dtype, void* out) {
  RD_REQUIRE(w && out, RD_EINVAL, "pack_conv1x1_sc_m16: null pointer");
  RD_REQUIRE(is_h16(dtype), RD_EINVAL, "pack_conv1x1_sc_m16: dtype %d (RD_BF16 or RD_F16)", dtype);
  pack_sc_frag16(w, fold_scale, out, dtype);
  return RD_OK;
}
int rd_block64_m16_bn_act(const void* x, int x_cstride, int x_coff, const void* w_packed, const float* shift1, const float* shift2,
                          const void* sc_w_packed, void* y, int y_cstride, int y_coff, int B, int H, int W, int dtype, void* stream) {
  RD_REQUIRE(x && w_packed && shift1 && shift2 && y, RD_EINVAL, "block64_m16: null pointer");
  RD_REQUIRE(is_h16(dtype), RD_EINVAL, "block64_m16: dtype %d (RD_BF16 or RD_F16)", dtype);
  RD_REQUIRE(B > 0 && H > 0 && W > 0, RD_ESHAPE, "block64_m16: shape");
  RD_REQUIRE(x_cstride % 8 == 0 && x_coff % 8 == 0 && x_coff >= 0 && x_coff + 64 <= x_cstride, RD_ESHAPE, "block64_m16: x channel stride / offset");
  RD_REQUIRE(y_cstride % 8 == 0 && y_coff % 8 == 0 && y_coff >= 0 && y_coff + 64 <= y_cstride, RD_ESHAPE, "block64_m16: y channel stride / offset");
  RD_REQUIRE(x != y, RD_EINVAL, "block64_m16: in-place (a tile's halo is another tile's output)");
  return launch_block64(x, x_cstride, x_coff, 64, w_packed, shift1, shift2, sc_w_packed, y, y_cstride, y_coff, B, H, W, dtype, (hipStream_t)stream, true);
}

size_t rd_conv3x3_cat_packed_bytes(int cin1, int cin2, int cout) { return conv_packed_bytes(9, cin1 + cin2, cout, RD_BF16); }
int rd_pack_conv3x3_cat_host(const float* w, const float* fold_scale, int cout, int cin1, int cin2, int dtype, void* out) {
  RD_REQUIRE(w && out, RD_EINVAL, "pack_conv3x3_cat: null pointer");
  RD_REQUIRE(is_h16(dtype), RD_EINVAL, "pack_conv3x3_cat: dtype %d (RD_BF16 or RD_F16)", dtype);
  RD_REQUIRE((cout == 64 || cout == 128) && cin1 > 0 && cin1 % 32 == 0 && cin2 > 0 && cin2 % 8 == 0, RD_ESHAPE,
             "pack_conv3x3_cat: cout %d, cin1 %d (multiple of 32), cin2 %d (multiple of 8)", cout, cin1, cin2);
  const int cin = cin1 + cin2;
  auto wv = [&](int co, int ci, int dh, int dw) {
    return (fold_scale ? fold_scale[co] : 1.f) * w[(((size_t)co * cin + ci) * 3 + (dh + 1)) * 3 + (dw + 1)];
  };
  memset(out, 0, rd_conv3x3_cat_packed_bytes(cin1, cin2, cout));
  const int body = conv3_body_cat(cin1, cin2, fold_scale != nullptr);
  if (body) pack_body_frag(body, cin, cout, out, [&](int co, int ci, int dh, int dw) { return wv(co, ci, dh - 1, dw - 1); }, dtype);
  else pack_taps_frag(9, cin, cout, out, [&](int co, int ci, int t) { return wv(co, ci, t / 3 - 1, t % 3 - 1); }, dtype);
  return RD_OK;
}
int rd_conv3x3_bn_act_cat(const void* x1, int x1_cstride, int x1_coff, int cin1, const void* x2, int x2_cstride, int x2_coff, int cin2,
                          const void* w_packed, const float* shift, void* y, int y_cstride, int y_coff, int B, int H, int W, int cout,
                          int flags, int dtype, void* stream) {
  RD_REQUIRE(x1 && x2 && w_packed && y && shift, RD_EINVAL, "conv3x3_cat: null pointer");
  RD_REQUIRE(is_h16(dtype), RD_EINVAL, "conv3x3_cat: dtype %d (RD_BF16 or RD_F16)", dtype);
  RD_REQUIRE((flags & RD_SCALE_FOLDED) && !(flags & RD_ADD), RD_EINVAL, "conv3x3_cat: needs RD_SCALE_FOLDED weights, takes no residual");
  RD_REQUIRE(B > 0 && H > 0 && W > 0 && (cout == 64 || cout == 128), RD_ESHAPE, "conv3x3_cat: shape / cout %d", cout);
  RD_REQUIRE(cin1 > 0 && cin1 % 32 == 0 && cin2 > 0 && cin2 % 8 == 0, RD_ESHAPE, "conv3x3_cat: cin1 %d (multiple of 32), cin2 %d (multiple of 8)", cin1, cin2);
  RD_REQUIRE(y_coff >= 0 && y_coff + cout <= y_cstride, RD_ESHAPE, "conv3x3_cat: y channels exceed stride");
  RD_REQUIRE(x1_cstride % 8 == 0 && x1_coff % 8 == 0 && x1_coff + cin1 <= x1_cstride && x2_cstride % 8 == 0 && x2_coff % 8 == 0 &&
             x2_coff + cin2 <= x2_cstride, RD_ESHAPE, "conv3x3_cat: channel stride/offset");
  const DevSwitches& sw_ = dev_switches();
  RD_REQUIRE(!sw_.conv_v1 && sw_.conv_wide && sw_.conv_w30 && (cout == 64 ? sw_.conv_th4 != 3 : (sw_.conv_th4 && sw_.conv_w30 == 2)), RD_ESHAPE,
             "conv3x3_cat: needs the 8 x 32 tile form of the persistent 3x3 kernel (a dev switch turned it off)");
  allow_conv_lds();
  Conv3Src2 s2;
  s2.x = x2; s2.cs = x2_cstride; s2.co = x2_coff; s2.cin1 = cin1; s2.cin2 = cin2;
  return launch_conv3(x1, x1_cstride, x1_coff, w_packed, nullptr, shift, nullptr, 0, 0, y, y_cstride, y_coff, B, H, W, cin1 + cin2, cout, flags,
                      1, (hipStream_t)stream, 0, nullptr, dtype, nullptr, nullptr, &s2, conv3_body_cat(cin1, cin2, true));
}

size_t rd_head_packed_bytes(void) { return 16384; }
int rd_pack_head_weight_host(const float* w, int nout, int cin, int dtype, void* out_host) {
  RD_REQUIRE(w && out_host, RD_EINVAL, "pack_head_weight: null pointer");
  RD_REQUIRE(is_h16(dtype), RD_EINVAL, "pack_head_weight: dtype %d (RD_BF16 or RD_F16)", dtype);
  RD_REQUIRE(nout >= 1 && nout <= 8 && cin >= 1 && cin <= 128, RD_ESHAPE, "pack_head_weight: nout %d (1..8), cin %d (1..128)", nout, cin);
  pack_head_frag(w, nout, cin, out_host, dtype);
  return RD_OK;
}
size_t rd_head_m16_packed_bytes(void) { return 8192; }
int rd_pack_head_weight_m16_host(const float* w, int nout, int cin, int dtype, void* out_host) {
  RD_REQUIRE(w && out_host, RD_EINVAL, "pack_head_weight_m16: null pointer");
  RD_REQUIRE(is_h16(dtype), RD_EINVAL, "pack_head_weight_m16: dtype %d (RD_BF16 or RD_F16)", dtype);
  RD_REQUIRE(nout >= 1 && nout <= 8 && cin >= 1 && cin <= 128, RD_ESHAPE, "pack_head_weight_m16: nout %d (1..8), cin %d (1..128)", nout, cin);
  pack_head_frag16(w, nout, cin, out_host, dtype);
  return RD_OK;
}
int rd_conv2d_bn_act_head_out(const void* x, int x_cstride, int x_coff, const void* w_packed, const float* scale,
                              const float* shift, int B, int H, int W, int cin, int flags, const void* head_w_packed,
                              const float* head_bias, float* out, long out_batch_stride, long n_off, int nout, int dtype,
                              void* stream) {
  RD_REQUIRE(x && w_packed && head_w_packed && head_bias && out, RD_EINVAL, "conv2d_head_out: null pointer");
  RD_REQUIRE(is_h16(dtype), RD_EINVAL, "conv2d_head_out: dtype %d (RD_BF16 or RD_F16)", dtype);
  RD_REQUIRE(B > 0 && H > 0 && W > 0 && cin > 0 && nout >= 1 && nout <= 8, RD_ESHAPE, "conv2d_head_out: shape / nout %d (1..8)", nout);
  RD_REQUIRE(!(flags & RD_ADD), RD_EINVAL, "conv2d_head_out: no residual in a head tower");
  RD_REQUIRE(x_cstride % 8 == 0 && x_coff % 8 == 0 && x_coff + cin_slots(cin, RD_BF16) * 8 <= x_cstride, RD_ESHAPE,
             "conv2d_head_out: x channel stride/offset");
  RD_REQUIRE(!dev_switches().conv_v1, RD_EINVAL, "conv2d_head_out: needs the persistent 3x3 kernel (RD_CONV_V1 is set)");
  RD_REQUIRE(!conv3_body_small(cin, (flags & RD_SCALE_FOLDED) != 0), RD_ESHAPE, "conv2d_head_out: cin %d (the packed image of a conv with <= 16 input channels is not this launch form's)", cin);
  const bool m16 = (flags & RD_MFMA16) != 0;
  RD_REQUIRE(!m16 || ((flags & RD_SCALE_FOLDED) && conv3_mfma16_ok(cin, 128, 1, W, true)), RD_ESHAPE,
             "conv2d_head_out: RD_MFMA16 (weights of rd_pack_conv3x3_m16_host) is not a launch form for cin %d at width %d (rd_conv3x3_mfma16_ok)", cin, W);
  allow_conv_lds();
  Conv3Args h;
  memset(&h, 0, sizeof(h));
  h.hw = (const unsigned char*)head_w_packed; h.hb = head_bias; h.ho = out; h.ho_bs = out_batch_stride; h.ho_off = n_off; h.hn = nout;
  return launch_conv3(x, x_cstride, x_coff, w_packed, scale, shift, nullptr, 0, 0, nullptr, 128, 0, B, H, W, cin, 128, flags & ~RD_MFMA16, 1,
                      (hipStream_t)stream, 0, &h, dtype, nullptr, nullptr, nullptr, m16 ? C3_BODY_M16 : 0);
}

static int pair_checks(const char* fn, const void* x0, const void* x1, const void* w0, const void* w1, const float* shift0,
                       const float* shift1, int x_cstride, int x0_coff, int x1_coff, int B, int H, int W, int cin, int flags,
                       int dtype) {
  RD_REQUIRE(x0 && x1 && w0 && w1 && shift0 && shift1, RD_EINVAL, "%s: null pointer", fn);
  RD_REQUIRE(is_h16(dtype), RD_EINVAL, "%s: dtype %d (RD_BF16 or RD_F16)", fn, dtype);
  RD_REQUIRE(B > 0 && H > 0 && W > 0 && cin > 0, RD_ESHAPE, "%s: shape", fn);
  RD_REQUIRE((flags & RD_SCALE_FOLDED) && !(flags & RD_ADD), RD_EINVAL, "%s: needs RD_SCALE_FOLDED weights, takes no residual", fn);
  RD_REQUIRE(x_cstride % 8 == 0 && x0_coff % 8 == 0 && x1_coff % 8 == 0 && x0_coff + cin_slots(cin, RD_BF16) * 8 <= x_cstride &&
             x1_coff + cin_slots(cin, RD_BF16) * 8 <= x_cstride, RD_ESHAPE, "%s: x channel stride/offset", fn);
  RD_REQUIRE(!dev_switches().conv_v1, RD_EINVAL, "%s: needs the persistent 3x3 kernel (RD_CONV_V1 is set)", fn);
  RD_REQUIRE(cin > 16, RD_ESHAPE, "%s: cin %d (more than 16 input channels)", fn, cin);
  return RD_OK;
}
int rd_conv3x3_bn_act_pair(const void* x0, int x0_coff, const void* w0_packed, const float* shift0, void* y0, int y0_coff,
                           const void* x1, int x1_coff, const void* w1_packed, const float* shift1, void* y1, int y1_coff,
                           int x_cstride, int y_cstride, int B, int H, int W, int cin, int flags, int dtype, void* stream) {
  if (int rc = pair_checks("conv3x3_pair", x0, x1, w0_packed, w1_packed, shift0, shift1, x_cstride, x0_coff, x1_coff, B, H, W, cin, flags, dtype)) return rc;
  RD_REQUIRE(y0 && y1, RD_EINVAL, "conv3x3_pair: null output");
  RD_REQUIRE(y0_coff >= 0 && y1_coff >= 0 && y0_coff + 128 <= y_cstride && y1_coff + 128 <= y_cstride, RD_ESHAPE, "conv3x3_pair: y channels exceed stride");
  allow_conv_lds();
  if (!conv3_pair_eligible(128, flags, W)) {
    if (int rc = launch_conv3(x0, x_cstride, x0_coff, w0_packed, nullptr, shift0, nullptr, 0, 0, y0, y_cstride, y0_coff, B, H, W, cin, 128,
                              flags, 1, (hipStream_t)stream, 0, nullptr, dtype)) return rc;
    return launch_conv3(x1, x_cstride, x1_coff, w1_packed, nullptr, shift1, nullptr, 0, 0, y1, y_cstride, y1_coff, B, H, W, cin, 128, flags, 1,
                        (hipStream_t)stream, 0, nullptr, dtype);
  }
  Conv3Second g;
  memset(&g, 0, sizeof(g));
  g.x = x1; g.x_co = x1_coff; g.w = w1_packed; g.shift = shift1; g.y = y1; g.y_co = y1_coff;
  return launch_conv3(x0, x_cstride, x0_coff, w0_packed, nullptr, shift0, nullptr, 0, 0, y0, y_cstride, y0_coff, B, H, W, cin, 128, flags, 1,
                      (hipStream_t)stream, 0, nullptr, dtype, &g);
}
int rd_conv2d_bn_act_head_out_pair(const void* x0, int x0_coff, const void* w0_packed, const float* shift0, const void* head_w0_packed,
                                   const float* head_bias0, float* out0, long out0_batch_stride, int nout0,
                                   const void* x1, int x1_coff, const void* w1_packed, const float* shift1, const void* head_w1_packed,
                                   const float* head_bias1, float* out1, long out1_batch_stride, int nout1,
                                   int x_cstride, long n_off, int B, int H, int W, int cin, int flags, int dtype, void* stream) {
  if (int rc = pair_checks("conv2d_head_out_pair", x0, x1, w0_packed, w1_packed, shift0, shift1, x_cstride, x0_coff, x1_coff, B, H, W, cin, flags, dtype)) return rc;
  RD_REQUIRE(head_w0_packed && head_w1_packed && head_bias0 && head_bias1 && out0 && out1, RD_EINVAL, "conv2d_head_out_pair: null pointer");
  RD_REQUIRE(nout0 >= 1 && nout0 <= 8 && nout1 >= 1 && nout1 <= 8, RD_ESHAPE, "conv2d_head_out_pair: nout %d / %d (1..8)", nout0, nout1);
  allow_conv_lds();
  Conv3Args h;
  memset(&h, 0, sizeof(h));
  h.hw = (const unsigned char*)head_w0_packed; h.hb = head_bias0; h.ho = out0; h.ho_bs = out0_batch_stride; h.ho_off = n_off; h.hn = nout0;
  if (!conv3_pair_eligible(128, flags, W, true)) {
    if (int rc = launch_conv3(x0, x_cstride, x0_coff, w0_packed, nullptr, shift0, nullptr, 0, 0, nullptr, 128, 0, B, H, W, cin, 128, flags, 1,
                              (hipStream_t)stream, 0, &h, dtype)) return rc;
    h.hw = (const unsigned char*)head_w1_packed; h.hb = head_bias1; h.ho = out1; h.ho_bs = out1_batch_stride; h.hn = nout1;
    return launch_conv3(x1, x_cstride, x1_coff, w1_packed, nullptr, shift1, nullptr, 0, 0, nullptr, 128, 0, B, H, W, cin, 128, flags, 1,
                        (hipStream_t)stream, 0, &h, dtype);
  }
  Conv3Second g;
  memset(&g, 0, sizeof(g));
  g.x = x1; g.x_co = x1_coff; g.w = w1_packed; g.shift = shift1;
  g.hw = head_w1_packed; g.hb = head_bias1; g.ho = out1; g.ho_bs = out1_batch_stride; g.hn = nout1;
  return launch_conv3(x0, x_cstride, x0_coff, w0_packed, nullptr, shift0, nullptr, 0, 0, nullptr, 128, 0, B, H, W, cin, 128, flags, 1,
                      (hipStream_t)stream, 0, &h, dtype, &g);
}

int rd_deconv2d_bn_act(const void* x, int x_cstride, int x_coff, const void* w_packed_phase, const float* scale,
                       const float* shift, const void* residual, int r_cstride, int r_coff, void* y, int y_cstride,
                       int y_coff, int B, int H, int Win, int cin, int cout, int kh, int kw, int stride_w, int pad_w,
                       int phase, int flags, int dtype, void* stream) {
  RD_REQUIRE(x && w_packed_phase && y, RD_EINVAL, "deconv2d: null pointer");
  RD_REQUIRE(kh == 3, RD_ESHAPE, "deconv2d: kernel height %d (only 3, pad 1, stride 1)", kh);
  RD_REQUIRE(stride_w >= 1 && phase >= 0 && phase < stride_w, RD_EINVAL, "deconv2d: phase %d of stride %d", phase, stride_w);
  RD_REQUIRE(y_coff >= 0 && y_coff + cout <= y_cstride, RD_ESHAPE, "deconv2d: y channels exceed stride");
  const int Wout = (Win - 1) * stride_w - 2 * pad_w + kw;
  RD_REQUIRE(Wout > phase, RD_ESHAPE, "deconv2d: empty phase");
  const int Wq = (Wout - phase + stride_w - 1) / stride_w;
  TapList tl = deconv_taps_sorted(kh, kw, stride_w, pad_w, phase);
  RD_REQUIRE(tl.n >= 1 && tl.n <= 9, RD_ESHAPE, "deconv2d: %d taps per phase unsupported", tl.n);
  allow_conv_lds();
  if (deconv_embeds_3x3(tl)) {
    const int ts = deconv_tap_set(tl);
    if (!ts) tl = conv_taps(3, 3);
    if (is_h16(dtype) && Wout == stride_w * Win && (cout == 64 || cout == 128) && !dev_switches().conv_v1 &&
        conv3_has_form(dtype, (flags & RD_SCALE_FOLDED) != 0)) {
      const bf16_t* r = (const bf16_t*)residual;
      return launch_conv3(x, x_cstride, x_coff, w_packed_phase, scale, shift, r, r_cstride * stride_w,
                          r_coff + phase * r_cstride, y, y_cstride * stride_w, y_coff + phase * y_cstride, B, H, Win, cin,
                          cout, flags, 1, (hipStream_t)stream, ts, nullptr, dtype);
    }
  }
  RD_REQUIRE(!(flags & RD_SCALE_FOLDED), RD_ESHAPE, "deconv2d: RD_SCALE_FOLDED needs the persistent 3x3 kernel (bf16, cout 64/128, "
             "taps inside the 3x3 window, Wout == stride_w * Win)");
  return launch_conv(tl, x, x_cstride, x_coff, w_packed_phase, scale, shift, residual, r_cstride, r_coff, y,
                     y_cstride, y_coff, B, H, Win, Wq, Wout, cin, cout, 1, stride_w, phase, flags, dtype,
                     (hipStream_t)stream);
}

int rd_deconv2d_all_phases_ok(int kh, int kw, int stride_w, int pad_w, int cout, int dtype) {
  if (!is_h16(dtype) || kh != 3 || stride_w < 2 || stride_w > 8 || !conv3_phases_eligible(cout, RD_SCALE_FOLDED)) return 0;
  if (kw - 2 * pad_w != stride_w) return 0;
  for (int p = 0; p < stride_w; ++p)
    if (!deconv_tap_set(deconv_taps_sorted(kh, kw, stride_w, pad_w, p))) return 0;
  return 1;
}
int rd_deconv2d_bn_act_all(const void* x, int x_cstride, int x_coff, const void* w_packed_all, long w_phase_bytes,
                           const float* shift, const void* residual, int r_cstride, int r_coff, void* y, int y_cstride,
                           int y_coff, int B, int H, int Win, int cin, int cout, int kh, int kw, int stride_w, int pad_w,
                           int flags, int dtype, void* stream) {
  RD_REQUIRE(x && w_packed_all && y, RD_EINVAL, "deconv2d_all: null pointer");
  RD_REQUIRE(is_h16(dtype), RD_EINVAL, "deconv2d_all: dtype %d (RD_BF16 or RD_F16)", dtype);
  RD_REQUIRE(flags & RD_SCALE_FOLDED, RD_EINVAL, "deconv2d_all: needs RD_SCALE_FOLDED weights (rd_pack_deconv_weight_folded_host)");
  RD_REQUIRE(!((flags & RD_ADD) && !residual), RD_EINVAL, "deconv2d_all: RD_ADD without residual");
  RD_REQUIRE(B > 0 && H > 0 && Win > 0 && cin > 0, RD_ESHAPE, "deconv2d_all: shape");
  RD_REQUIRE(y_coff >= 0 && y_coff + cout <= y_cstride, RD_ESHAPE, "deconv2d_all: y channels exceed stride");
  RD_REQUIRE(x_cstride % 8 == 0 && x_coff % 8 == 0 && x_coff + cin_slots(cin, RD_BF16) * 8 <= x_cstride, RD_ESHAPE, "deconv2d_all: x channel stride/offset");
  RD_REQUIRE(rd_deconv2d_all_phases_ok(kh, kw, stride_w, pad_w, cout, dtype), RD_ESHAPE,
             "deconv2d_all: kernel (%d,%d) stride %d pad %d cout %d is not a set of two-column 3x2 phases (use rd_deconv2d_bn_act per phase)",
             kh, kw, stride_w, pad_w, cout);
  RD_REQUIRE(w_phase_bytes >= (long)conv_packed_bytes(6, cin, cout, RD_BF16) && w_phase_bytes % 16 == 0, RD_EINVAL, "deconv2d_all: w_phase_bytes");
  allow_conv_lds();
  Conv3Phases ph;
  ph.nph = stride_w; ph.ts_mask = 0; ph.y_pc = y_cstride; ph.r_pc = r_cstride; ph.w_pb = w_phase_bytes;
  for (int p = 0; p < stride_w; ++p)
    if (deconv_tap_set(deconv_taps_sorted(kh, kw, stride_w, pad_w, p)) == 2) ph.ts_mask |= 1 << p;
  return launch_conv3(x, x_cstride, x_coff, w_packed_all, nullptr, shift, residual, r_cstride * stride_w, r_coff, y, y_cstride * stride_w,
                      y_coff, B, H, Win, cin, cout, flags, 1, (hipStream_t)stream, 3, nullptr, dtype, nullptr, &ph);
}

int rd_deconv2d_phase_pairs_ok(int kh, int kw, int stride_w, int pad_w, int cout, int dtype) {
  if (!rd_deconv2d_all_phases_ok(kh, kw, stride_w, pad_w, cout, dtype) || cout != 64 || stride_w % 2) return 0;
  if (!rd_deconv2d_all_phases_ok(kh, kw, stride_w, pad_w, 128, dtype)) return 0;
  for (int p = 0; p < stride_w; p += 2)
    if (deconv_tap_set(deconv_taps_sorted(kh, kw, stride_w, pad_w, p)) != deconv_tap_set(deconv_taps_sorted(kh, kw, stride_w, pad_w, p + 1))) return 0;
  return 1;
}
int rd_pack_deconv_phase_pair_host(const void* phase_a, const void* phase_b, int cin, int dtype, void* out) {
  RD_REQUIRE(phase_a && phase_b && out, RD_EINVAL, "pack_deconv_pair: null pointer");
  RD_REQUIRE(is_h16(dtype) && cin > 0, RD_EINVAL, "pack_deconv_pair: dtype %d / cin %d", dtype, cin);
  const size_t body = conv_packed_body_bytes(6, cin, 64, RD_BF16), blocks = body / 2048;
  for (size_t i = 0; i < blocks; ++i) {
    memcpy((unsigned char*)out + i * 4096, (const unsigned char*)phase_a + i * 2048, 2048);
    memcpy((unsigned char*)out + i * 4096 + 2048, (const unsigned char*)phase_b + i * 2048, 2048);
  }
  memset((unsigned char*)out + 2 * body, 0, 2 * RD_CONV_TAIL);
  return RD_OK;
}
int rd_deconv2d_bn_act_pairs(const void* x, int x_cstride, int x_coff, const void* w_packed_pairs, long w_pair_bytes,
                             const float* shift2, const void* residual, int r_cstride, int r_coff, void* y, int y_cstride,
                             int y_coff, int B, int H, int Win, int cin, int cout, int kh, int kw, int stride_w, int pad_w,
                             int flags, int dtype, void* stream) {
  RD_REQUIRE(x && w_packed_pairs && y && shift2, RD_EINVAL, "deconv2d_pairs: null pointer");
  RD_REQUIRE(is_h16(dtype), RD_EINVAL, "deconv2d_pairs: dtype %d (RD_BF16 or RD_F16)", dtype);
  RD_REQUIRE(flags & RD_SCALE_FOLDED, RD_EINVAL, "deconv2d_pairs: needs RD_SCALE_FOLDED weights (rd_pack_deconv_weight_folded_host)");
  RD_REQUIRE(!((flags & RD_ADD) && !residual), RD_EINVAL, "deconv2d_pairs: RD_ADD without residual");
  RD_REQUIRE(B > 0 && H > 0 && Win > 0 && cin > 0, RD_ESHAPE, "deconv2d_pairs: shape");
  RD_REQUIRE(x_cstride % 8 == 0 && x_coff % 8 == 0 && x_coff + cin_slots(cin, RD_BF16) * 8 <= x_cstride, RD_ESHAPE, "deconv2d_pairs: x channel stride/offset");
  RD_REQUIRE(rd_deconv2d_phase_pairs_ok(kh, kw, stride_w, pad_w, cout, dtype), RD_ESHAPE,
             "deconv2d_pairs: kernel (%d,%d) stride %d pad %d cout %d has no phase pairs (use rd_deconv2d_bn_act_all)", kh, kw, stride_w, pad_w, cout);
  RD_REQUIRE(y_cstride == cout && y_coff == 0 && (!residual || (r_cstride == cout && r_coff == 0)), RD_ESHAPE,
             "deconv2d_pairs: the output / residual must be dense %d-channel tensors (two phases are one 128-channel write)", cout);
  RD_REQUIRE(w_pair_bytes >= (long)conv_packed_bytes(6, cin, 2 * cout, RD_BF16) && w_pair_bytes % 16 == 0, RD_EINVAL, "deconv2d_pairs: w_pair_bytes");
  allow_conv_lds();
  Conv3Phases ph;
  ph.nph = stride_w / 2; ph.ts_mask = 0; ph.y_pc = 2 * cout; ph.r_pc = 2 * cout; ph.w_pb = w_pair_bytes;
  for (int p = 0; p < stride_w; p += 2)
    if (deconv_tap_set(deconv_taps_sorted(kh, kw, stride_w, pad_w, p)) == 2) ph.ts_mask |= 1 << (p / 2);
  return launch_conv3(x, x_cstride, x_coff, w_packed_pairs, nullptr, shift2, residual, r_cstride * stride_w, r_coff, y, y_cstride * stride_w,
                      y_coff, B, H, Win, cin, 2 * cout, flags, 1, (hipStream_t)stream, 3, nullptr, dtype, nullptr, &ph);
}

int rd_head_out(const void* x, int x_cstride, int x_coff, const float* w, const float* bias, float* out,
                long out_batch_stride, long n_off, int B, int H, int W, int cin, int nout, int dtype, void* stream) {
  RD_REQUIRE(x && w && bias && out, RD_EINVAL, "head_out: null pointer");
  RD_REQUIRE(cin % 8 == 0 && cin <= 128 && cin > 0, RD_ESHAPE, "head_out: cin %d (multiple of 8, <= 128)", cin);
  RD_REQUIRE(nout == 1 || nout == 7 || nout == 8, RD_ESHAPE, "head_out: nout %d not in {1,7,8}", nout);
  RD_REQUIRE(dtype == RD_F32 || is_h16(dtype), RD_EINVAL, "head_out: dtype");
  hipStream_t st = (hipStream_t)stream;
  const long HW = (long)H * W;
  dim3 grid((unsigned)std::min<long>((HW + 31) / 32, 4096), B);
  ProfScope ps(RD_PROF_HEAD_OUT, st);
  if (is_h16(dtype) && nout > 1 && cin % 16 == 0 && x_cstride % 8 == 0 && x_coff % 8 == 0) {
    dim3 g2((unsigned)std::min<long>((HW + 127) / 128, 2048), B);
#define RD_HOM(NO, DT_) hipLaunchKernelGGL((head_out_mfma_kernel<NO, DT_>), g2, dim3(256), 0, st, (const bf16_t*)x, x_cstride, x_coff, w, bias, out, out_batch_stride, n_off, HW, cin)
    if (dtype == RD_F16) { if (nout == 7) RD_HOM(7, RD_F16); else RD_HOM(8, RD_F16); }
    else { if (nout == 7) RD_HOM(7, RD_BF16); else RD_HOM(8, RD_BF16); }
#undef RD_HOM
    return check_launch("head_out");
  }
#define RD_HO(DT, NO) hipLaunchKernelGGL((head_out_kernel<DT, NO>), grid, dim3(256), 0, st, x, x_cstride, x_coff, w, bias, out, out_batch_stride, n_off, HW, cin)
  if (dtype == RD_BF16) { if (nout == 1) RD_HO(RD_BF16, 1); else if (nout == 7) RD_HO(RD_BF16, 7); else RD_HO(RD_BF16, 8); }
  else if (dtype == RD_F16) { if (nout == 1) RD_HO(RD_F16, 1); else if (nout == 7) RD_HO(RD_F16, 7); else RD_HO(RD_F16, 8); }
  else { if (nout == 1) RD_HO(RD_F32, 1); else if (nout == 7) RD_HO(RD_F32, 7); else RD_HO(RD_F32, 8); }
#undef RD_HO
  return check_launch("head_out");
}

size_t rd_meta_packed_bytes(int dtype) { return meta_layout(dtype).total; }
int rd_pack_meta_host(const float* w0, const float* b0, const float* w1, const float* b1, const float* s1,
                      const float* t1, const float* agg, const float* s2, const float* t2, int dtype, void* out) {
  RD_REQUIRE(w0 && b0 && w1 && b1 && s1 && t1 && agg && s2 && t2 && out, RD_EINVAL, "pack_meta: null pointer");
  RD_REQUIRE(dtype == RD_F32 || is_h16(dtype), RD_EINVAL, "pack_meta: dtype");
  pack_meta(w0, b0, w1, b1, s1, t1, agg, s2, t2, dtype, out);
  return RD_OK;
}
int rd_meta_kernel_fwd(const void* data, int d_cstride, int d_coff, const float* coord_nchw, const void* packed,
                       void* y, int y_cstride, int y_coff, int B, int H, int W, int dtype, void* stream) {
  RD_REQUIRE(data && coord_nchw && packed && y, RD_EINVAL, "meta_kernel: null pointer");
  RD_REQUIRE(B > 0 && H > 0 && W > 0, RD_ESHAPE, "meta_kernel: empty shape");
  RD_REQUIRE(dtype == RD_F32 || is_h16(dtype), RD_EINVAL, "meta_kernel: dtype");
  const int ch = ch_per_slot(dtype);
  RD_REQUIRE(d_cstride % ch == 0 && d_coff % ch == 0 && y_cstride % ch == 0 && y_coff % ch == 0, RD_ESHAPE,
             "meta_kernel: channel strides/offsets must be 16-byte multiples");
  RD_REQUIRE(d_coff + 64 <= d_cstride && y_coff + 64 <= y_cstride, RD_ESHAPE, "meta_kernel: needs 64 channels");
  hipStream_t st = (hipStream_t)stream;
  MetaArgs a;
  a.data = data; a.d_cs = d_cstride; a.d_co = d_coff; a.coord = coord_nchw; a.packed = (const unsigned char*)packed;
  a.y = y; a.y_cs = y_cstride; a.y_co = y_coff; a.B = B; a.H = H; a.W = W;
  constexpr int WAVES = 8;
  a.tiles_h = (H + WAVES - 1) / WAVES;
  a.tiles_w = (W + 31) / 32;
  a.ntiles = B * a.tiles_h * a.tiles_w;
  a.r0 = 0; a.m0 = a.m1 = a.m2 = 0;
  const size_t consts = 9 * 64 * 4 * 2 + 1024;
  ProfScope ps(RD_PROF_META, st);
  if (is_h16(dtype)) {
    const size_t lds = meta_layout(dtype).wbytes + consts + (size_t)(WAVES + 2) * 34 * 128 + 4096;
    static std::atomic<unsigned long long> seen{0};
    once_per_device(seen, [] { allow_big_lds(meta16_kernel<WAVES, RD_BF16>); allow_big_lds(meta16_kernel<WAVES, RD_F16>); });
    const dim3 mgrid(std::min(a.ntiles, conv_num_cus())), mblock(WAVES * 64);
    const int strips = a.tiles_w * B;
    a.r0 = dev_switches().conv_xcd && strips % 8 == 0 ? 8 : strips;
    RD_REQUIRE((unsigned long long)a.ntiles * (unsigned)std::max(a.r0, std::max(a.tiles_h, a.tiles_w)) < (1ull << 32), RD_ESHAPE,
               "meta_kernel: %d tiles exceed the range of the tile decode", a.ntiles);
    a.m0 = meta_magic(a.r0); a.m1 = meta_magic(a.tiles_h); a.m2 = meta_magic(a.tiles_w);
    RD_REQUIRE((long)H * W < (1l << 23) && (long)H * W * d_cstride < (1l << 31) && W < (1 << 23) && d_cstride < (1 << 23), RD_ESHAPE,
               "meta_kernel: image of %d x %d pixels x %d channels exceeds the 32-bit halo offsets", H, W, d_cstride);
    if (dtype == RD_F16) hipLaunchKernelGGL((meta16_kernel<WAVES, RD_F16>), mgrid, mblock, lds, st, a);
    else hipLaunchKernelGGL((meta16_kernel<WAVES, RD_BF16>), mgrid, mblock, lds, st, a);
  } else {
    const size_t lds = consts + (size_t)(WAVES + 2) * 34 * 256;
    static std::atomic<unsigned long long> seen32{0};
    once_per_device(seen32, [] { allow_big_lds(meta_kernel<RD_F32, WAVES>); });
    hipLaunchKernelGGL((meta_kernel<RD_F32, WAVES>), dim3(std::min(a.ntiles, 512)), dim3(WAVES * 64), lds, st, a);
  }
  return check_launch("meta_kernel");
}

size_t rd_sorted_foreground_workspace_bytes(long N, long k) { (void)k; return (sort_ws_bytes(N) + 256 + 255) & ~(size_t)255; }
int rd_sorted_foreground(const float* cls_score, const float* bbox_delta, const float* pc, const float* mask, int B,
                         long N, long k, int D, int apply_sigmoid, float* out_score, float* out_delta, float* out_pc,
                         int* out_idx, void* ws, size_t ws_bytes, void* stream) {
  RD_REQUIRE(cls_score && bbox_delta && pc && out_score && out_delta && out_pc && ws, RD_EINVAL, "sorted_foreground: null pointer");
  RD_REQUIRE(B > 0 && N > 0 && k > 0 && D > 0, RD_ESHAPE, "sorted_foreground: empty shape");
  RD_REQUIRE(N >= k, RD_ESHAPE, "sorted_foreground: N (%ld) < num_fgs (%ld)", N, k);
  RD_REQUIRE(N < (1L << 31), RD_ESHAPE, "sorted_foreground: N too large");
  RD_REQUIRE(ws_bytes >= rd_sorted_foreground_workspace_bytes(N, k), RD_EWORKSPACE, "sorted_foreground: workspace %zu < %zu",
             ws_bytes, rd_sorted_foreground_workspace_bytes(N, k));
  hipStream_t st = (hipStream_t)stream;
  void* wsa = (void*)(((uintptr_t)ws + 255) & ~(uintptr_t)255);
  SortWs s = sort_ws_carve(wsa, N);
  ProfScope ps(RD_PROF_SORT, st);
  const size_t per = rd_sorted_foreground_workspace_bytes(N, k);
  const bool wide = ws_bytes >= per * (size_t)B;
  const long stride = wide ? (long)(per / 4) : 0;
  const int nb = wide ? B : 1;
  for (int b0 = 0; b0 < B; b0 += nb) {
    hipLaunchKernelGGL(sort_keygen_kernel, dim3((unsigned)((N + 255) / 256), nb), dim3(256), 0, st, cls_score + (size_t)b0 * N,
                       mask ? mask + (size_t)b0 * N : nullptr, N, apply_sigmoid, s.keysA, s.idxA, stride);
    unsigned *rk, *ri;
    int rc = radix_topk_pairs(s, N, k, st, nb, stride, &rk, &ri);
    if (rc != RD_OK) return rc;
    hipLaunchKernelGGL(sort_gather_kernel, dim3((unsigned)((k + 255) / 256), nb), dim3(256), 0, st, rk, ri, k, D,
                       bbox_delta + (size_t)b0 * N * D, pc + (size_t)b0 * N * 3, out_score + (size_t)b0 * k,
                       out_delta + (size_t)b0 * k * D, out_pc + (size_t)b0 * k * 3, out_idx ? out_idx + (size_t)b0 * k : nullptr,
                       stride, N);
  }
  return check_launch("sorted_foreground");
}

int rd_decode3d_bbox(const float* bbox_delta, const float* pc, float* out, int B, long N, int box_type, int is_bin,
                     void* stream) {
  RD_REQUIRE(bbox_delta && pc && out, RD_EINVAL, "decode3d: null pointer");
  RD_REQUIRE(B > 0 && N > 0, RD_ESHAPE, "decode3d: empty shape");
  RD_REQUIRE((is_bin && box_type == 7) || (!is_bin && box_type == 8), RD_ESHAPE,
             "decode3d: box_type %d with is_bin=%d (8 for regular, 7 for bin)", box_type, is_bin);
  hipStream_t st = (hipStream_t)stream;
  const long n = (long)B * N;
  ProfScope ps(RD_PROF_DECODE, st);
  hipLaunchKernelGGL(decode3d_kernel, dim3((unsigned)((n + 255) / 256)), dim3(256), 0, st, bbox_delta, pc, out, n, box_type, is_bin);
  return check_launch("decode3d");
}

size_t rd_score_filter_workspace_bytes(long n) { return (size_t)((n + 255) / 256 + 8) * 4 + 256; }
int rd_score_filter_dets_batched(const float* scores, long scores_bstride, const float* boxes10, long boxes_bstride,
                                 long n, float min_score, float* dets, long dets_bstride, int* d_count, void* ws,
                                 size_t ws_bytes, int B, void* stream) {
  RD_REQUIRE(scores && boxes10 && dets && d_count && ws, RD_EINVAL, "score_filter: null pointer");
  RD_REQUIRE(n > 0 && B > 0, RD_ESHAPE, "score_filter: empty input");
  const size_t per = rd_score_filter_workspace_bytes(n);
  RD_REQUIRE(ws_bytes >= per * (size_t)B, RD_EWORKSPACE, "score_filter: workspace %zu < %zu", ws_bytes, per * (size_t)B);
  hipStream_t st = (hipStream_t)stream;
  int* blk = (int*)(((uintptr_t)ws + 255) & ~(uintptr_t)255);
  const int nblk = (int)((n + 255) / 256);
  const long blk_bs = nblk + 8;
  ProfScope ps(RD_PROF_WNMS, st);
  hipLaunchKernelGGL(filter_count_kernel, dim3(nblk, B), dim3(256), 0, st, scores, n, min_score, blk, scores_bstride, blk_bs);
  hipLaunchKernelGGL(filter_scan_kernel, dim3(B), dim3(256), 0, st, blk, nblk, d_count, blk_bs);
  hipLaunchKernelGGL(filter_scatter_kernel, dim3(nblk, B), dim3(256), 0, st, scores, boxes10, n, min_score, blk, dets,
                     scores_bstride, boxes_bstride, blk_bs, dets_bstride);
  return check_launch("score_filter");
}
int rd_score_filter_dets(const float* scores, const float* boxes10, long n, float min_score, float* dets, int* d_count,
                         void* ws, size_t ws_bytes, void* stream) {
  return rd_score_filter_dets_batched(scores, 0, boxes10, 0, n, min_score, dets, 0, d_count, ws, ws_bytes, 1, stream);
}

size_t rd_wnms_workspace_bytes(int Kcap) { return Kcap > 0 ? wnms_ws_bytes(Kcap) : 0; }
int rd_wnms_4c_batched(const float* dets, long dets_bstride, int Kcap, const int* d_count, const int* order,
                       long order_bstride, int tie_order, float thresh, float thresh_vote, int is3d, int hash_scale,
                       float* out_dets, long out_bstride, int* keep, long keep_bstride, int* d_nkeep, void* ws,
                       size_t ws_bytes, int B, void* stream) {
  RD_REQUIRE(dets && out_dets && keep && d_nkeep && ws, RD_EINVAL, "wnms_4c: null pointer");
  RD_REQUIRE(Kcap > 0 && Kcap <= RD_WNMS_MAX_K, RD_ESHAPE, "wnms_4c: Kcap %d not in [1, %d]", Kcap, RD_WNMS_MAX_K);
  RD_REQUIRE(B > 0, RD_ESHAPE, "wnms_4c: batch %d", B);
  const int diag = tie_order & ~0xff;
  tie_order &= 0xff;
  RD_REQUIRE(tie_order == RD_TIE_STABLE || tie_order == RD_TIE_REFERENCE, RD_EINVAL, "wnms_4c: tie_order %d", tie_order);
  RD_REQUIRE(!(diag & ~(RD_WNMS_DIAG_NO_SKIP | (0xff << 16) | (0x7f << 24))), RD_EINVAL, "wnms_4c: unknown diagnostic bits 0x%x", diag);
  const size_t per = rd_wnms_workspace_bytes(Kcap);
  RD_REQUIRE(ws_bytes >= per * (size_t)B, RD_EWORKSPACE, "wnms_4c: workspace %zu < %zu", ws_bytes, per * (size_t)B);
  RD_REQUIRE(order || B == 1 || tie_order == RD_TIE_REFERENCE, RD_EINVAL,
             "wnms_4c: the batched call needs an explicit processing order or RD_TIE_REFERENCE");
  hipStream_t st = (hipStream_t)stream;
  static std::atomic<unsigned long long> seen_lds{0};
  once_per_device(seen_lds, [] {
    allow_big_lds(wnms_tie_order_kernel); allow_big_lds(wnms_scan_kernel); allow_big_lds(wnms_scan4_kernel); allow_big_lds(wnms_merge_kernel);
  });
  WnmsWs w = wnms_ws_carve(ws, Kcap);
  ProfScope ps(RD_PROF_WNMS, st);
  WnmsBatch bs;
  bs.dets = dets_bstride; bs.order = order_bstride; bs.prep = (long)(per / 4); bs.words = (long)(per / 8);
  bs.ints = (long)(per / 4); bs.keep = keep_bstride; bs.out = out_bstride;
  const int* ord = order;
  if (!ord && tie_order == RD_TIE_REFERENCE) {
    const size_t lds = TIE_STACK_BYTES + (Kcap <= TIE_LDS_K ? (size_t)Kcap * 8 + 3 * ((size_t)Kcap / 32 + 2) * 4 : 0);
    hipLaunchKernelGGL(wnms_tie_order_kernel, dim3(1, 1, B), dim3(256), lds, st, dets, Kcap, d_count, w.order, bs, (long)(per / 4),
                       w.scratch);
    ord = w.order;
    bs.order = (long)(per / 4);
  } else if (!ord) {
    void* swa = (void*)(((uintptr_t)w.sort_ws + 255) & ~(uintptr_t)255);
    SortWs s = sort_ws_carve(swa, Kcap);
    hipLaunchKernelGGL(sort_keygen_dets_kernel, dim3((Kcap + 255) / 256), dim3(256), 0, st, dets, Kcap, d_count, s.keysA, s.idxA);
    int rc = radix_sort_pairs(s, Kcap, st);
    if (rc != RD_OK) return rc;
    if (hipMemcpyAsync(w.order, s.idxA, (size_t)Kcap * 4, hipMemcpyDeviceToDevice, st) != hipSuccess)
      return rd::fail(RD_EHIP, "wnms_4c: order copy");
    ord = w.order;
    bs.order = 0;
  }
  const int nb = (Kcap + 63) / 64;
  hipLaunchKernelGGL(wnms_prep_kernel, dim3((Kcap + 255) / 256, 1, B), dim3(256), 0, st, dets, ord, Kcap, d_count, w.prep, bs,
                     (float)hash_scale, w.novf);
  const int e_tw = (diag >> 16) & 0xff, e_ml = (diag >> 24) & 0x7f;
  const int tile_w = std::min(w.nwcap, e_tw ? std::max(1, e_tw) : 256);
  const size_t scan_lds = ((size_t)w.nwcap + (size_t)64 * tile_w) * 8;
  const int R1 = 256, nb1 = R1 / 64;
  const bool one_round = dev_switches().wnms_one_round;
  const bool two = Kcap >= 4 * R1 && !one_round;
  const int ct = dev_switches().wnms_ct == 32 ? 32 : dev_switches().wnms_ct == 16 ? 16 : 8;
  const int pgrid = std::min(2048, std::max(64, nb * (64 / ct) * std::min(nb, 16)));
  const int allow_skip = thresh >= 1e-3f && thresh_vote >= 1e-3f && !is3d && !dev_switches().wnms_no_skip && !(diag & RD_WNMS_DIAG_NO_SKIP);
  auto pairs = [&](const int* rows, const int* nrows, const unsigned long long* supp, int rb_end) {
    auto k = dev_switches().wnms_bal ? (ct == 8 ? wnms_pairs_kernel<8, true> : ct == 16 ? wnms_pairs_kernel<16, true> : wnms_pairs_kernel<32, true>)
                                     : (ct == 8 ? wnms_pairs_kernel<8, false> : ct == 16 ? wnms_pairs_kernel<16, false> : wnms_pairs_kernel<32, false>);
    hipLaunchKernelGGL(k, dim3(pgrid, 1, B), dim3(64), 0, st, w.prep, Kcap, d_count, thresh, thresh_vote, is3d, w.thr, w.vote,
                       w.nwcap, bs, rows, nrows, supp, 0, rb_end, allow_skip);
  };
  pairs(nullptr, nullptr, nullptr, two ? nb1 : nb);
  const bool scan4 = w.nwcap <= 128 && !e_tw && !dev_switches().wnms_scan1;
  const int tile_words = 64 * 128;
  const size_t scan4_lds = ((size_t)w.nwcap + tile_words) * 8;
  auto scan = [&](int c_begin, int c_end, unsigned long long* state) {
    if (scan4)
      hipLaunchKernelGGL(wnms_scan4_kernel, dim3(1, 1, B), dim3(256), scan4_lds, st, w.thr, w.snap, Kcap, d_count, w.nwcap, ord,
                         w.keep_q, keep, d_nkeep, bs, c_begin, c_end, state, tile_words);
    else
      hipLaunchKernelGGL(wnms_scan_kernel, dim3(1, 1, B), dim3(64), scan_lds, st, w.thr, w.snap, Kcap, d_count, w.nwcap, ord,
                         w.keep_q, keep, d_nkeep, bs, c_begin, c_end, state, tile_w);
  };
  scan(0, two ? nb1 : nb, two ? w.supp_state : (unsigned long long*)nullptr);
  if (two) {
    hipLaunchKernelGGL(wnms_alive_kernel, dim3(1, 1, B), dim3(256), 0, st, w.supp_state, Kcap, d_count, R1, w.alive, w.nalive, bs);
    pairs((const int*)w.alive, (const int*)w.nalive, (const unsigned long long*)w.supp_state, 0);
    scan(nb1, nb, w.supp_state);
  }
  const int lds_cap = std::min(Kcap + 2, e_ml ? std::max(4, e_ml) : 2048);
  hipLaunchKernelGGL(wnms_merge_kernel, dim3(std::min(Kcap, 4096), 1, B), dim3(64), (size_t)lds_cap * 8, st, dets, ord, w.vote,
                     w.snap, Kcap, d_count, w.nwcap, w.keep_q, d_nkeep, out_dets, bs, lds_cap, w.ovf, w.novf);
  if (Kcap + 2 > lds_cap)
    hipLaunchKernelGGL(wnms_merge_big_kernel, dim3(1, 1, B), dim3(64), 0, st, dets, ord, w.vote, w.snap, Kcap, d_count, w.nwcap,
                       w.keep_q, out_dets, bs, (const int*)w.ovf, (const int*)w.novf, w.scratch);
  return check_launch("wnms_4c");
}
int rd_wnms_4c(const float* dets, int Kcap, const int* d_count, const int* order, int tie_order, float thresh,
               float thresh_vote, int is3d, int hash_scale, float* out_dets, int* keep, int* d_nkeep, void* ws,
               size_t ws_bytes, void* stream) {
  return rd_wnms_4c_batched(dets, 0, Kcap, d_count, order, 0, tie_order, thresh, thresh_vote, is3d, hash_scale, out_dets, 0,
                            keep, 0, d_nkeep, ws, ws_bytes, 1, stream);
}
int rd_single_overlap(const float* dets_a, const float* dets_b, long n, int is3d, float* out, void* stream) {
  RD_REQUIRE(n >= 0 && (n == 0 || (dets_a && dets_b && out)), RD_EINVAL, "single_overlap: bad arguments");
  if (n == 0) return RD_OK;
  hipLaunchKernelGGL(single_overlap_kernel, dim3((unsigned)((n + 63) / 64)), dim3(64), 0, (hipStream_t)stream, dets_a, dets_b, n,
                     is3d, out);
  return check_launch("single_overlap");
}
int rd_wnms_pair_skippable(const float* dets_a, const float* dets_b, long n, unsigned char* out, void* stream) {
  RD_REQUIRE(dets_a && dets_b && out && n >= 0, RD_EINVAL, "wnms_pair_skippable: null pointer");
  if (n == 0) return RD_OK;
  hipLaunchKernelGGL(pair_skippable_kernel, dim3((unsigned)((n + 63) / 64)), dim3(64), 0, (hipStream_t)stream, dets_a, dets_b, n, out);
  return check_launch("wnms_pair_skippable");
}
namespace rd {
__global__ void atan2f_kernel(const float* y, const float* x, long n, float* out) {
  const long i = (long)blockIdx.x * blockDim.x + threadIdx.x;
  if (i < n) out[i] = fdlibm_atan2f(y[i], x[i]);
}
}
int rd_edge_atan2f(const float* y, const float* x, long n, float* out, void* stream) {
  RD_REQUIRE(y && x && out && n >= 0, RD_EINVAL, "edge_atan2f: null pointer");
  if (n == 0) return RD_OK;
  hipLaunchKernelGGL(atan2f_kernel, dim3((unsigned)((n + 255) / 256)), dim3(256), 0, (hipStream_t)stream, y, x, n, out);
  return check_launch("edge_atan2f");
}
int rd_wnms_order_host(const float* dets_host, int K, int* order_host) {
  RD_REQUIRE(K >= 0 && (K == 0 || (dets_host && order_host)), RD_EINVAL, "wnms_order_host: bad arguments");
  std::iota(order_host, order_host + K, 0);
  std::sort(order_host, order_host + K, [&](int i, int j) { return dets_host[i * 12 + 11] > dets_host[j * 12 + 11]; });
  return RD_OK;
}

int rd_dets12_to_8_batched(const float* dets12, long dets12_bstride, int Mcap, const int* d_count, float* out8,
                           long out8_bstride, int B, void* stream) {
  RD_REQUIRE(dets12 && out8, RD_EINVAL, "dets12_to_8: null pointer");
  RD_REQUIRE(Mcap > 0 && B > 0, RD_ESHAPE, "dets12_to_8: empty input");
  hipLaunchKernelGGL(dets12_to_8_kernel, dim3((Mcap + 255) / 256, B), dim3(256), 0, (hipStream_t)stream, dets12, Mcap, d_count,
                     out8, dets12_bstride, out8_bstride);
  return check_launch("dets12_to_8");
}
int rd_dets12_to_8(const float* dets12, int Mcap, const int* d_count, float* out8, void* stream) {
  return rd_dets12_to_8_batched(dets12, 0, Mcap, d_count, out8, 0, 1, stream);
}

int rd_gather_keep_scores(const float* score, long score_bstride, int k, const int* keep_idx, int max_keep, float* out, int B,
                          void* stream) {
  RD_REQUIRE(score && keep_idx && out, RD_EINVAL, "gather_keep_scores: null pointer");
  RD_REQUIRE(k > 0 && max_keep > 0 && B > 0, RD_ESHAPE, "gather_keep_scores: empty input");
  hipLaunchKernelGGL(gather_keep_scores_kernel, dim3((max_keep + 255) / 256, B), dim3(256), 0, (hipStream_t)stream, score,
                     score_bstride, k, keep_idx, max_keep, out);
  return check_launch("gather_keep_scores");
}

int rd_rotated_iou_8pt(const float* boxes1, const float* boxes2, float* ious, long n1, long n2, void* stream) {
  RD_REQUIRE(boxes1 && boxes2 && ious, RD_EINVAL, "rotated_iou: null pointer");
  RD_REQUIRE(n1 > 0 && n2 > 0, RD_ESHAPE, "rotated_iou: empty input");
  hipLaunchKernelGGL(riou8_kernel, dim3((unsigned)((n1 * n2 + 255) / 256)), dim3(256), 0, (hipStream_t)stream, boxes1, boxes2, ious, n1, n2);
  return check_launch("rotated_iou_8pt");
}
int rd_batch_rotated_iou(const float* proposal, int p_stride, const float* gt_bbox, float* iou_map, int* argmax, int B, long N,
                         int n_gt, void* stream) {
  RD_REQUIRE(proposal && gt_bbox && iou_map, RD_EINVAL, "batch_rotated_iou: null pointer");
  RD_REQUIRE(B > 0 && B <= 65535 && N > 0 && n_gt > 0 && n_gt <= 256 && p_stride >= 8, RD_ESHAPE,
             "batch_rotated_iou: B %d, N %ld, n_gt %d (<= 256), proposal row %d floats (>= 8)", B, N, n_gt, p_stride);
  hipLaunchKernelGGL(batch_riou_kernel, dim3((unsigned)((N + 255) / 256), B), dim3(256), 0, (hipStream_t)stream, proposal, p_stride,
                     N * (long)p_stride, gt_bbox, (long)n_gt * 8, iou_map, argmax, N, n_gt);
  return check_launch("batch_rotated_iou");
}
int rd_rotated_iou_7(const float* boxes1, const float* boxes2, float* ious, long n1, long n2, void* stream) {
  RD_REQUIRE(boxes1 && boxes2 && ious, RD_EINVAL, "rotated_iou_7: null pointer");
  if (n1 * n2 == 0) return RD_OK;
  hipLaunchKernelGGL(riou7_kernel, dim3((unsigned)((n1 * n2 + 255) / 256)), dim3(256), 0, (hipStream_t)stream, boxes1, boxes2, ious, n1, n2);
  return check_launch("rotated_iou_7");
}
int rd_batch_rotated_iou_3d(const float* proposal, int p_stride, const float* gt_bbox7, float* iou_map, int* argmax, int B, long N,
                            int n_gt, void* stream) {
  RD_REQUIRE(proposal && gt_bbox7 && iou_map, RD_EINVAL, "batch_rotated_iou_3d: null pointer");
  RD_REQUIRE(B > 0 && N > 0 && p_stride >= 10, RD_ESHAPE, "batch_rotated_iou_3d: proposal rows need the 8 corners + z0, z1 (stride %d)", p_stride);
  RD_REQUIRE(n_gt >= 1 && n_gt <= 256, RD_ESHAPE, "batch_rotated_iou_3d: n_gt %d (1..256; the config pads to 200)", n_gt);
  ProfScope ps(RD_PROF_DECODE, (hipStream_t)stream);
  hipLaunchKernelGGL(batch_riou3d_kernel, dim3((unsigned)((N + 255) / 256), B), dim3(256), 0, (hipStream_t)stream, proposal, p_stride,
                     (long)N * p_stride, gt_bbox7, (long)n_gt * 7, iou_map, argmax, N, n_gt);
  return check_launch("batch_rotated_iou_3d");
}
int rd_batch_max_iou(const float* proposals, int p_stride, const float* gt8, float* out, long n, int n_gt, void* stream) {
  return rd_batch_rotated_iou(proposals, p_stride, gt8, out, nullptr, 1, n, n_gt, stream);
}

size_t rd_nms3d_workspace_bytes(long N, int B) {
  if (N <= 0 || N > (1 << 18) || B <= 0) return 0;
  return nms3d_frame_bytes((int)N) * (size_t)B;
}
int rd_nms3d(const float* boxes, int B, long N, float iou_thres, int max_keep, int normal_iou, int* keep_idx,
             float* bbox_after_nms, void* ws, size_t ws_bytes, void* stream) {
  RD_REQUIRE(boxes && keep_idx && bbox_after_nms && ws, RD_EINVAL, "nms3d: null pointer");
  RD_REQUIRE(B > 0 && B <= 65535 && N > 0 && N <= (1 << 18) && max_keep > 0, RD_ESHAPE, "nms3d: B %d, N %ld (<= 262144), max_keep %d", B, N, max_keep);
  RD_REQUIRE(ws_bytes >= rd_nms3d_workspace_bytes(N, B), RD_EWORKSPACE, "nms3d: workspace %zu < %zu bytes", ws_bytes, rd_nms3d_workspace_bytes(N, B));
  RD_REQUIRE(((uintptr_t)ws & 7) == 0, RD_EINVAL, "nms3d: workspace must be 8-byte aligned");
  Nms3dArgs a;
  a.boxes = boxes; a.ws = (unsigned char*)ws; a.ws_frame = nms3d_frame_bytes((int)N);
  a.keep = keep_idx; a.out = bbox_after_nms;
  a.N = (int)N; a.ncw = (int)((N + 63) / 64); a.max_keep = max_keep; a.normal_iou = normal_iou ? 1 : 0; a.thresh = iou_thres;
  hipStream_t st = (hipStream_t)stream;
  ProfScope ps(RD_PROF_WNMS, st);
  const int gi = (std::max(std::max(a.ncw, max_keep), 2) + 255) / 256;
  hipLaunchKernelGGL(nms3d_init_kernel, dim3(gi, B), dim3(256), 0, st, a);
  for (int r0 = 0, blk = 64; r0 < a.N; r0 += blk, blk = std::min(2 * blk, NMS3D_RB)) {
    const int rows = std::min(blk, a.N - r0);
    hipLaunchKernelGGL(nms3d_pairs_kernel, dim3((a.N + NMS3D_SEG - 1) / NMS3D_SEG, rows, B), dim3(256), 0, st, a, r0);
    hipLaunchKernelGGL(nms3d_scan_kernel, dim3(B), dim3(256), (size_t)a.ncw * 8, st, a, r0, blk);
  }
  return check_launch("nms3d");
}

int rd_assign3d_v2(const float* pc, const float* bbox, const float* bbox_center, const float* bbox_radius, const float* mask,
                   const float* is_in_nlz, long N, int M, float max_x, float min_x, float max_y, float min_y, float max_z,
                   float min_z, float max_dist, int* out, void* stream) {
  RD_REQUIRE(pc && bbox && bbox_center && bbox_radius && mask && is_in_nlz && out, RD_EINVAL, "assign3d_v2: null pointer");
  RD_REQUIRE(N > 0 && M > 0 && M <= ASSIGN_MAX_BOXES, RD_ESHAPE, "assign3d_v2: N %ld, M %d (1..%d)", N, M, ASSIGN_MAX_BOXES);
  AssignArgs a;
  a.pc = pc; a.bbox = bbox; a.center = bbox_center; a.radius = bbox_radius; a.mask = mask; a.nlz = is_in_nlz; a.out = out;
  a.N = N; a.M = M;
  a.max_x = max_x; a.min_x = min_x; a.max_y = max_y; a.min_y = min_y; a.max_z = max_z; a.min_z = min_z; a.max_dist = max_dist;
  hipLaunchKernelGGL(assign3d_kernel, dim3((unsigned)((N + 255) / 256)), dim3(256), (size_t)M * 14 * 4, (hipStream_t)stream, a);
  return check_launch("assign3d_v2");
}
size_t rd_get_point_num_workspace_bytes(void) { return POINT_NUM_MAX_BOXES * sizeof(int); }
int rd_get_point_num(const float* bbox_inds, long N, float* out, void* ws, size_t ws_bytes, void* stream) {
  RD_REQUIRE(bbox_inds && out && ws, RD_EINVAL, "get_point_num: null pointer");
  RD_REQUIRE(N > 0, RD_ESHAPE, "get_point_num: N %ld", N);
  RD_REQUIRE(ws_bytes >= rd_get_point_num_workspace_bytes(), RD_EWORKSPACE, "get_point_num: workspace %zu < %zu bytes", ws_bytes,
             rd_get_point_num_workspace_bytes());
  hipStream_t st = (hipStream_t)stream;
  if (hipMemsetAsync(ws, 0, rd_get_point_num_workspace_bytes(), st) != hipSuccess) return fail(RD_EHIP, "get_point_num: memset failed");
  const unsigned g = (unsigned)std::min<long>((N + 255) / 256, 1024);
  hipLaunchKernelGGL(point_num_count_kernel, dim3(g), dim3(256), 0, st, bbox_inds, N, (int*)ws);
  hipLaunchKernelGGL(point_num_gather_kernel, dim3((unsigned)((N + 255) / 256)), dim3(256), 0, st, bbox_inds, N, (const int*)ws, out);
  return check_launch("get_point_num");
}

int rd_input_transform(const float* range_image, const float* pc_vehicle_frame, const float* inclination,
                       const rd_input_norm_t* norm_host, int B, int H, int W, int Hp, int Wp, float* input_data,
                       float* coord_s1, float* pc_s1, float* pc_s2, float* pc_s4, float* mask_s1, float* mask_s2,
                       float* mask_s4, void* stream) {
  RD_REQUIRE(range_image && pc_vehicle_frame && inclination && norm_host && input_data && coord_s1 && pc_s1 && pc_s2 && pc_s4 &&
                 mask_s1 && mask_s2 && mask_s4, RD_EINVAL, "input_transform: null pointer");
  RD_REQUIRE(B > 0 && H > 2 && W > 2 && Hp >= H && Wp >= W && Wp % 4 == 0, RD_ESHAPE,
             "input_transform: shape (%d,%d,%d) -> (%d,%d)", B, H, W, Hp, Wp);
  InputArgs a;
  a.ri = range_image; a.pc = pc_vehicle_frame; a.incl = inclination;
  a.data = input_data; a.coord = coord_s1;
  a.pcs[0] = pc_s1; a.pcs[1] = pc_s2; a.pcs[2] = pc_s4;
  a.msk[0] = mask_s1; a.msk[1] = mask_s2; a.msk[2] = mask_s4;
  a.B = B; a.H = H; a.W = W; a.Hp = Hp; a.Wp = Wp;
  a.n = *norm_host;
  hipStream_t st = (hipStream_t)stream;
  ProfScope ps(RD_PROF_LAYOUT, st);
  hipLaunchKernelGGL(input_transform_kernel, dim3((unsigned)(((long)Hp * Wp + 255) / 256), B), dim3(256), 0, st, a);
  return check_launch("input_transform");
}

int rd_dev_conv_trace_set(unsigned long long* device_buf, long nwords) {
  if (device_buf && nwords < (long)CONV_TRACE_CAP) return RD_EINVAL;
  conv_trace_slot() = device_buf;
  return RD_OK;
}
int rd_dev_conv_trace_read(unsigned long long* out, long n) {
  if (!conv_trace_buf() || n > (long)CONV_TRACE_CAP) return RD_EINVAL;
  return hipMemcpy(out, conv_trace_buf(), n * 8, hipMemcpyDeviceToHost) == hipSuccess ? RD_OK : RD_EHIP;
}
int rd_prof_enable(int on) {
  Prof& p = prof();
  std::lock_guard<std::mutex> g(p.mu);
  p.on = on != 0;
  return RD_OK;
}
int rd_prof_reset(void) {
  Prof& p = prof();
  std::lock_guard<std::mutex> g(p.mu);
  p.drain();
  for (int k = 0; k < RD_PROF_NKINDS; ++k) { p.total[k] = 0; p.count[k] = 0; }
  return RD_OK;
}
int rd_prof_get(int kind, double* total_ms, long* launches) {
  RD_REQUIRE(kind >= 0 && kind < RD_PROF_NKINDS && total_ms && launches, RD_EINVAL, "prof_get: bad arguments");
  Prof& p = prof();
  std::lock_guard<std::mutex> g(p.mu);
  p.drain();
  *total_ms = p.total[kind];
  *launches = p.count[kind];
  return RD_OK;
}

}
```

rangedet_amd/csrc/rd_common.h:

```cpp
#pragma once
#include <hip/hip_runtime.h>

#include <cstdarg>
#include <cstdint>
#include <cstdio>
#include <cstdlib>
#include <cstring>
#include <mutex>
#include <type_traits>
#include <vector>

#include <atomic>
#include "../../include/rangedet_hip.h"

namespace rd {

inline char* err_buf() {
  static thread_local char buf[512] = "";
  return buf;
}
inline int fail(int code, const char* fmt, ...) {
  va_list ap;
  va_start(ap, fmt);
  vsnprintf(err_buf(), 512, fmt, ap);
  va_end(ap);
  return code;
}
#define RD_REQUIRE(cond, code, ...) \
  do {                              \
    if (!(cond)) return rd::fail(code, __VA_ARGS__); \
  } while (0)

inline int check_launch(const char* what) {
  hipError_t e = hipGetLastError();
  if (e != hipSuccess) return fail(RD_EHIP, "%s: %s", what, hipGetErrorString(e));
  return RD_OK;
}

struct DevSwitches {
  bool conv_v1;
  int conv_th4;
  int conv_w30, conv_head30;
  int conv_hb3;
  int conv_wide;
  int conv_xcd;
  int conv_body;
  bool sort_no_select;
  bool wnms_one_round;
  int wnms_bal;
  bool wnms_scan1;
  int wnms_ct;
  bool wnms_no_skip;
};
constexpr DevSwitches kDevSwitchDefaults = {false, 1, 2, 1, 1, 1, 1, 1, false, false, 0, false, 8, false};
#ifdef RD_DEV_SWITCHES
inline const DevSwitches& dev_switches() {
  static const DevSwitches s = [] {
    auto num = [](const char* name, int dflt) { const char* e = getenv(name); return e ? atoi(e) : dflt; };
    DevSwitches d = kDevSwitchDefaults;
    d.conv_v1 = getenv("RD_CONV_V1") != nullptr;
    d.conv_th4 = num("RD_CONV_TH4", 1);
    d.conv_w30 = num("RD_CONV_W30", 2);
    d.conv_head30 = num("RD_CONV_HEAD30", 1);
    d.conv_hb3 = num("RD_CONV_HB3", 1);
    d.conv_wide = num("RD_CONV_WIDE", 1);
    d.conv_body = num("RD_CONV_BODY", 1);
    d.conv_xcd = num("RD_CONV_XCD", 1);
    d.sort_no_select = getenv("RD_SORT_NO_SELECT") != nullptr;
    d.wnms_one_round = getenv("RD_WNMS_ONE_ROUND") != nullptr;
    d.wnms_ct = num("RD_WNMS_CT", 8);
    d.wnms_scan1 = getenv("RD_WNMS_SCAN1") != nullptr;
    d.wnms_no_skip = getenv("RD_WNMS_NO_SKIP") != nullptr;
    d.wnms_bal = num("RD_WNMS_BAL", 0);
    return d;
  }();
  return s;
}
#else
inline constexpr const DevSwitches& dev_switches() { return kDevSwitchDefaults; }
#endif

template <class K>
inline void allow_big_lds(K kernel) {
  if (hipFuncSetAttribute((const void*)kernel, hipFuncAttributeMaxDynamicSharedMemorySize, 160 * 1024) != hipSuccess)
    (void)hipGetLastError();
}
template <class F>
inline void once_per_device(std::atomic<unsigned long long>& seen, F f) {
  int dev = 0;
  if (hipGetDevice(&dev) != hipSuccess) { (void)hipGetLastError(); f(); return; }
  if (dev < 0 || dev >= 64) { f(); return; }
  const unsigned long long bit = 1ull << dev;
  if (seen.load(std::memory_order_acquire) & bit) return;
  f();
  seen.fetch_or(bit, std::memory_order_release);
}

struct Prof {
  bool on = false;
  std::mutex mu;
  struct Span { hipEvent_t a, b; int kind; };
  std::vector<Span> spans;
  std::vector<hipEvent_t> pool;
  double total[RD_PROF_NKINDS] = {0};
  long count[RD_PROF_NKINDS] = {0};
  hipEvent_t get() {
    if (!pool.empty()) { hipEvent_t e = pool.back(); pool.pop_back(); return e; }
    hipEvent_t e;
    hipEventCreate(&e);
    return e;
  }
  void drain() {
    for (auto& s : spans) {
      hipEventSynchronize(s.b);
      float ms = 0;
      hipEventElapsedTime(&ms, s.a, s.b);
      total[s.kind] += ms;
      count[s.kind] += 1;
      pool.push_back(s.a);
      pool.push_back(s.b);
    }
    spans.clear();
  }
};
inline Prof& prof() {
  static Prof p;
  return p;
}
struct ProfScope {
  hipEvent_t a = nullptr;
  int kind;
  hipStream_t st;
  ProfScope(int k, hipStream_t s) : kind(k), st(s) {
    Prof& p = prof();
    if (!p.on) return;
    std::lock_guard<std::mutex> g(p.mu);
    a = p.get();
    hipEventRecord(a, st);
  }
  ~ProfScope() {
    if (!a) return;
    Prof& p = prof();
    std::lock_guard<std::mutex> g(p.mu);
    hipEvent_t b = p.get();
    hipEventRecord(b, st);
    p.spans.push_back({a, b, kind});
  }
};

typedef unsigned short bf16_t;
typedef float f32x16 __attribute__((ext_vector_type(16)));
typedef float f32x4 __attribute__((ext_vector_type(4)));
typedef short s16x8 __attribute__((ext_vector_type(8)));

__host__ __device__ __forceinline__ bf16_t f32_to_bf16(float f) {
#if defined(__HIP_DEVICE_COMPILE__)
  return __builtin_bit_cast(unsigned short, (__bf16)f);
#endif
  unsigned u;
  memcpy(&u, &f, 4);
  if ((u & 0x7fffffffu) > 0x7f800000u) return (bf16_t)((u >> 16) | 0x40);
  u += 0x7fffu + ((u >> 16) & 1u);
  return (bf16_t)(u >> 16);
}
__host__ __device__ __forceinline__ unsigned f32x2_to_bf16x2(float a, float b) {
#if defined(__HIP_DEVICE_COMPILE__)
  typedef float f32x2_t __attribute__((ext_vector_type(2)));
  typedef __bf16 bf16x2_t __attribute__((ext_vector_type(2)));
  const f32x2_t v = {a, b};
  return __builtin_bit_cast(unsigned, __builtin_convertvector(v, bf16x2_t));
#else
  return (unsigned)f32_to_bf16(a) | ((unsigned)f32_to_bf16(b) << 16);
#endif
}
__host__ __device__ __forceinline__ float bf16_to_f32(bf16_t h) {
  unsigned u = (unsigned)h << 16;
  float f;
  memcpy(&f, &u, 4);
  return f;
}

typedef unsigned short f16_t;
typedef _Float16 h16x8 __attribute__((ext_vector_type(8)));
__host__ __device__ __forceinline__ f16_t f32_to_f16(float f) { return __builtin_bit_cast(unsigned short, (_Float16)f); }
__host__ __device__ __forceinline__ float f16_to_f32(f16_t h) { return (float)__builtin_bit_cast(_Float16, h); }
__host__ __device__ __forceinline__ unsigned f32x2_to_f16x2(float a, float b) {
#if defined(__HIP_DEVICE_COMPILE__)
  typedef float f32x2_t __attribute__((ext_vector_type(2)));
  typedef _Float16 f16x2_t __attribute__((ext_vector_type(2)));
  const f32x2_t v = {a, b};
  return __builtin_bit_cast(unsigned, __builtin_convertvector(v, f16x2_t));
#else
  return (unsigned)f32_to_f16(a) | ((unsigned)f32_to_f16(b) << 16);
#endif
}

typedef float f32x2_t_ __attribute__((ext_vector_type(2)));
template <int DT> struct H16;
template <> struct H16<RD_BF16> {
  static constexpr unsigned short ONE = 0x3F80;
  __host__ __device__ static __forceinline__ unsigned short from_f32(float v) { return f32_to_bf16(v); }
  __host__ __device__ static __forceinline__ float to_f32(unsigned short h) { return bf16_to_f32(h); }
  __host__ __device__ static __forceinline__ unsigned pk(float a, float b) { return f32x2_to_bf16x2(a, b); }
  __host__ __device__ static __forceinline__ f32x2_t_ unpk(unsigned u) {
    unsigned lo = u << 16, hi = u & 0xffff0000u;
    return f32x2_t_{__builtin_bit_cast(float, lo), __builtin_bit_cast(float, hi)};
  }
  __device__ static __forceinline__ f32x16 mfma(s16x8 a, s16x8 b, f32x16 c) { return __builtin_amdgcn_mfma_f32_32x32x16_bf16(a, b, c, 0, 0, 0); }
  __device__ static __forceinline__ f32x4 mfma16(s16x8 a, s16x8 b, f32x4 c) { return __builtin_amdgcn_mfma_f32_16x16x32_bf16(a, b, c, 0, 0, 0); }
};
template <> struct H16<RD_F16> {
  static constexpr unsigned short ONE = 0x3C00;
  __host__ __device__ static __forceinline__ unsigned short from_f32(float v) { return f32_to_f16(v); }
  __host__ __device__ static __forceinline__ float to_f32(unsigned short h) { return f16_to_f32(h); }
  __host__ __device__ static __forceinline__ unsigned pk(float a, float b) { return f32x2_to_f16x2(a, b); }
  __host__ __device__ static __forceinline__ f32x2_t_ unpk(unsigned u) {
    return f32x2_t_{f16_to_f32((unsigned short)(u & 0xffffu)), f16_to_f32((unsigned short)(u >> 16))};
  }
  __device__ static __forceinline__ f32x16 mfma(s16x8 a, s16x8 b, f32x16 c) {
    return __builtin_amdgcn_mfma_f32_32x32x16_f16(__builtin_bit_cast(h16x8, a), __builtin_bit_cast(h16x8, b), c, 0, 0, 0);
  }
  __device__ static __forceinline__ f32x4 mfma16(s16x8 a, s16x8 b, f32x4 c) {
    return __builtin_amdgcn_mfma_f32_16x16x32_f16(__builtin_bit_cast(h16x8, a), __builtin_bit_cast(h16x8, b), c, 0, 0, 0);
  }
};
inline bool is_h16(int dt) { return dt == RD_BF16 || dt == RD_F16; }
inline unsigned short h16_from_f32(int dt, float v) { return dt == RD_F16 ? f32_to_f16(v) : f32_to_bf16(v); }
inline float h16_to_f32(int dt, unsigned short h) { return dt == RD_F16 ? f16_to_f32(h) : bf16_to_f32(h); }

template <int DT> struct Elem;
template <> struct Elem<RD_F32> {
  typedef float T;
  static constexpr int CH = 4;
  __host__ __device__ static float from_f32(float v) { return v; }
  __host__ __device__ static float to_f32(float v) { return v; }
};
template <> struct Elem<RD_BF16> {
  typedef bf16_t T;
  static constexpr int CH = 8;
  __host__ __device__ static bf16_t from_f32(float v) { return f32_to_bf16(v); }
  __host__ __device__ static float to_f32(bf16_t v) { return bf16_to_f32(v); }
};
template <> struct Elem<RD_F16> {
  typedef f16_t T;
  static constexpr int CH = 8;
  __host__ __device__ static f16_t from_f32(float v) { return f32_to_f16(v); }
  __host__ __device__ static float to_f32(f16_t v) { return f16_to_f32(v); }
};
inline int elem_size(int dt) { return dt == RD_F32 ? 4 : 2; }
inline int ch_per_slot(int dt) { return dt == RD_F32 ? 4 : 8; }
inline int round_up(int a, int b) { return (a + b - 1) / b * b; }

typedef unsigned Slot16 __attribute__((ext_vector_type(4)));


__device__ __forceinline__ void lds_dma16(const void* gsrc, void* lds_dst_uniform) {
#if defined(__HIP_DEVICE_COMPILE__)
  const unsigned lds_addr = __builtin_amdgcn_readfirstlane(
      (unsigned)(uintptr_t)(__attribute__((address_space(3))) void*)lds_dst_uniform);
  unsigned keep;
  asm volatile("s_mov_b32 %0, m0\n\ts_mov_b32 m0, %2\n\ts_nop 0\n\tglobal_load_lds_dwordx4 %1, off\n\ts_mov_b32 m0, %0"
               : "=&s"(keep)
               : "v"(gsrc), "s"(lds_addr)
               : "memory");
#else
  __builtin_amdgcn_global_load_lds((const __attribute__((address_space(1))) void*)gsrc,
                                   (__attribute__((address_space(3))) void*)lds_dst_uniform, 16, 0, 0);
#endif
}

__host__ __device__ inline float fdlibm_atanf(float x) {
  _Pragma("clang fp contract(off)")
  const float hi_[4] = {4.6364760399e-01f, 7.8539812565e-01f, 9.8279368877e-01f, 1.5707962513e+00f};
  const float lo_[4] = {5.0121582440e-09f, 3.7748947079e-08f, 3.4473217170e-08f, 7.5497894159e-08f};
  const float t0 = 3.3333334327e-01f, t1 = -2.0000000298e-01f, t2 = 1.4285714924e-01f, t3 = -1.1111110449e-01f, t4 = 9.0908870101e-02f,
              t5 = -7.6918758452e-02f, t6 = 6.6610731184e-02f, t7 = -5.8335702866e-02f, t8 = 4.9768779427e-02f, t9 = -3.6531571299e-02f,
              t10 = 1.6285819933e-02f;
  const int hx = __builtin_bit_cast(int, x), ix = hx & 0x7fffffff;
  int id;
  if (ix >= 0x4c000000) {
    if (ix > 0x7f800000) return x + x;
    return hx > 0 ? hi_[3] + lo_[3] : -hi_[3] - lo_[3];
  }
  if (ix < 0x3ee00000) {
    if (ix < 0x31000000) return x;
    id = -1;
  } else {
    x = __builtin_fabsf(x);
    if (ix < 0x3f980000) {
      if (ix < 0x3f300000) { id = 0; x = (2.0f * x - 1.0f) / (2.0f + x); }
      else { id = 1; x = (x - 1.0f) / (x + 1.0f); }
    } else {
      if (ix < 0x401c0000) { id = 2; x = (x - 1.5f) / (1.0f + 1.5f * x); }
      else { id = 3; x = -1.0f / x; }
    }
  }
  const float z = x * x, w = z * z;
  const float s1 = z * (t0 + w * (t2 + w * (t4 + w * (t6 + w * (t8 + w * t10)))));
  const float s2 = w * (t1 + w * (t3 + w * (t5 + w * (t7 + w * t9))));
  if (id < 0) return x - x * (s1 + s2);
  const float r = hi_[id] - ((x * (s1 + s2) - lo_[id]) - x);
  return hx < 0 ? -r : r;
}
__host__ __device__ inline float fdlibm_atan2f(float y, float x) {
  _Pragma("clang fp contract(off)")
  const float tiny = 1.0e-30f, pi_o_4 = 7.8539818525e-01f, pi_o_2 = 1.5707963705e+00f, pi = 3.1415927410e+00f, pi_lo = -8.7422776573e-08f;
  const int hx = __builtin_bit_cast(int, x), ix = hx & 0x7fffffff;
  const int hy = __builtin_bit_cast(int, y), iy = hy & 0x7fffffff;
  if (ix > 0x7f800000 || iy > 0x7f800000) return x + y;
  if (hx == 0x3f800000) return fdlibm_atanf(y);
  const int m = ((hy >> 31) & 1) | ((hx >> 30) & 2);
  if (iy == 0) return m < 2 ? y : (m == 2 ? pi + tiny : -pi - tiny);
  if (ix == 0) return hy < 0 ? -pi_o_2 - tiny : pi_o_2 + tiny;
  if (ix == 0x7f800000) {
    if (iy == 0x7f800000) return m == 0 ? pi_o_4 + tiny : m == 1 ? -pi_o_4 - tiny : m == 2 ? 3.0f * pi_o_4 + tiny : -3.0f * pi_o_4 - tiny;
    return m == 0 ? 0.0f : m == 1 ? -0.0f : m == 2 ? pi + tiny : -pi - tiny;
  }
  if (iy == 0x7f800000) return hy < 0 ? -pi_o_2 - tiny : pi_o_2 + tiny;
  const int k = (iy - ix) >> 23;
  float z;
  if (k > 60) z = pi_o_2 + 0.5f * pi_lo;
  else if (hx < 0 && k < -60) z = 0.0f;
  else z = fdlibm_atanf(__builtin_fabsf(y / x));
  switch (m) {
    case 0: return z;
    case 1: return __builtin_bit_cast(float, __builtin_bit_cast(unsigned, z) ^ 0x80000000u);
    case 2: return pi - (z - pi_lo);
    default: return (z - pi_lo) - pi;
  }
}

}
```

rangedet_amd/lib.py:

```python
import ctypes
import os

import numpy as np

RD_OK, RD_EINVAL, RD_ESHAPE, RD_EWORKSPACE, RD_EHIP = 0, -1, -2, -3, -4
RD_F32, RD_BF16, RD_F16 = 0, 1, 2
H16 = (RD_BF16, RD_F16)
RD_RELU_PRE, RD_ADD, RD_RELU_POST, RD_SCALE_FOLDED, RD_MFMA16 = 1, 2, 4, 8, 16
RD_WNMS_MAX_K = 65536
RD_WNMS_DIAG_NO_SKIP = 0x100


def RD_WNMS_DIAG_TILE_W(n):
    return (n & 0xff) << 16


def RD_WNMS_DIAG_MERGE_LDS(n):
    return (n & 0x7f) << 24

RD_TIE_STABLE, RD_TIE_REFERENCE = 0, 1
PROF_KINDS = {"conv": 0, "meta": 1, "head_out": 2, "sort": 3, "decode": 4, "wnms": 5, "layout": 6, "conv3": 7, "block": 8}

_HERE = os.path.dirname(os.path.abspath(__file__))
DEFAULT_PATH = os.environ.get("RANGEDET_HIP_LIB") or os.path.join(_HERE, "librangedet_hip.so")

c_int, c_long, c_float, c_size_t, c_void_p = ctypes.c_int, ctypes.c_long, ctypes.c_float, ctypes.c_size_t, ctypes.c_void_p

SIGNATURES = {
    "rd_version": (c_int, []),
    "rd_last_error_string": (ctypes.c_char_p, []),
    "rd_nchw_to_nhwc": (c_int, [c_void_p, c_void_p, c_int, c_int, c_int, c_int, c_int, c_int, c_int, c_int, c_void_p]),
    "rd_nhwc_to_nchw": (c_int, [c_void_p, c_void_p, c_int, c_int, c_int, c_int, c_int, c_int, c_int, c_void_p]),
    "rd_copy_rows": (c_int, [c_void_p, c_long, c_void_p, c_long, c_long, c_long, c_int, c_void_p]),
    "rd_conv_packed_bytes": (c_size_t, [c_int, c_int, c_int, c_int]),
    "rd_pack_conv_weight_host": (c_int, [c_void_p, c_int, c_int, c_int, c_int, c_int, c_void_p]),
    "rd_deconv_phase_taps": (c_int, [c_int, c_int, c_int, c_int, c_int]),
    "rd_pack_deconv_weight_host": (c_int, [c_void_p, c_int, c_int, c_int, c_int, c_int, c_int, c_int, c_int, c_void_p]),
    "rd_pack_deconv_weight_folded_host": (c_int, [c_void_p, c_void_p, c_int, c_int, c_int, c_int, c_int, c_int, c_int, c_int, c_void_p]),
    "rd_conv2d_bn_act": (c_int, [c_void_p, c_int, c_int, c_void_p, c_void_p, c_void_p, c_void_p, c_int, c_int, c_void_p,
                                 c_int, c_int, c_int, c_int, c_int, c_int, c_int, c_int, c_int, c_int, c_int, c_int, c_void_p]),
    "rd_conv3x3_ex_packed_bytes": (c_size_t, [c_int, c_int, c_int, c_int]),
    "rd_pack_conv3x3_ex_host": (c_int, [c_void_p, c_void_p, c_int, c_int, c_int, c_int, c_int, c_void_p]),
    "rd_pack_conv3x3_m16_host": (c_int, [c_void_p, c_void_p, c_int, c_int, c_int, c_void_p]),
    "rd_conv3x3_mfma16_ok": (c_int, [c_int, c_int, c_int, c_int, c_int]),
    "rd_conv1x1_sc_packed_bytes": (c_size_t, [c_int, c_int]),
    "rd_pack_conv1x1_sc_host": (c_int, [c_void_p, c_void_p, c_int, c_int, c_int, c_void_p]),
    "rd_conv3x3_bn_act_ex": (c_int, [c_void_p, c_int, c_int, c_void_p, c_void_p, c_void_p, c_void_p, c_int, c_int, c_void_p, c_int,
                                     c_int, c_int, c_void_p, c_void_p, c_int, c_int, c_int, c_int, c_int, c_int, c_int, c_int,
                                     c_int, c_int, c_void_p]),
    "rd_deconv2d_bn_act": (c_int, [c_void_p, c_int, c_int, c_void_p, c_void_p, c_void_p, c_void_p, c_int, c_int, c_void_p,
                                   c_int, c_int, c_int, c_int, c_int, c_int, c_int, c_int, c_int, c_int, c_int, c_int,
                                   c_int, c_int, c_void_p]),
    "rd_conv3x3_cat_packed_bytes": (c_size_t, [c_int, c_int, c_int]),
    "rd_pack_conv3x3_cat_host": (c_int, [c_void_p, c_void_p, c_int, c_int, c_int, c_int, c_void_p]),
    "rd_conv3x3_bn_act_cat": (c_int, [c_void_p, c_int, c_int, c_int, c_void_p, c_int, c_int, c_int, c_void_p, c_void_p, c_void_p, c_int, c_int,
                                      c_int, c_int, c_int, c_int, c_int, c_int, c_void_p]),
    "rd_deconv2d_all_phases_ok": (c_int, [c_int, c_int, c_int, c_int, c_int, c_int]),
    "rd_deconv2d_bn_act_all": (c_int, [c_void_p, c_int, c_int, c_void_p, c_long, c_void_p, c_void_p, c_int, c_int, c_void_p,
                                       c_int, c_int, c_int, c_int, c_int, c_int, c_int, c_int, c_int, c_int, c_int, c_int,
                                       c_int, c_void_p]),
    "rd_deconv2d_phase_pairs_ok": (c_int, [c_int, c_int, c_int, c_int, c_int, c_int]),
    "rd_pack_deconv_phase_pair_host": (c_int, [c_void_p, c_void_p, c_int, c_int, c_void_p]),
    "rd_deconv2d_bn_act_pairs": (c_int, [c_void_p, c_int, c_int, c_void_p, c_long, c_void_p, c_void_p, c_int, c_int, c_void_p,
                                         c_int, c_int, c_int, c_int, c_int, c_int, c_int, c_int, c_int, c_int, c_int, c_int,
                                         c_int, c_void_p]),
    "rd_block64_packed_bytes": (c_size_t, [c_int]),
    "rd_pack_block64_host": (c_int, [c_void_p, c_void_p, c_void_p, c_void_p, c_int, c_int, c_void_p]),
    "rd_pack_block64_m16_host": (c_int, [c_void_p, c_void_p, c_void_p, c_void_p, c_int, c_void_p]),
    "rd_pack_conv1x1_sc_m16_host": (c_int, [c_void_p, c_void_p, c_int, c_void_p]),
    "rd_block64_m16_bn_act": (c_int, [c_void_p, c_int, c_int, c_void_p, c_void_p, c_void_p, c_void_p, c_void_p, c_int, c_int, c_int, c_int,
                                      c_int, c_int, c_void_p]),
    "rd_block64_bn_act": (c_int, [c_void_p, c_int, c_int, c_int, c_void_p, c_void_p, c_void_p, c_void_p, c_void_p, c_int, c_int, c_int, c_int,
                                  c_int, c_int, c_void_p]),
    "rd_head_packed_bytes": (c_size_t, []),
    "rd_head_m16_packed_bytes": (c_size_t, []),
    "rd_pack_head_weight_host": (c_int, [c_void_p, c_int, c_int, c_int, c_void_p]),
    "rd_pack_head_weight_m16_host": (c_int, [c_void_p, c_int, c_int, c_int, c_void_p]),
    "rd_conv2d_bn_act_head_out": (c_int, [c_void_p, c_int, c_int, c_void_p, c_void_p, c_void_p, c_int, c_int, c_int, c_int, c_int,
                                          c_void_p, c_void_p, c_void_p, c_long, c_long, c_int, c_int, c_void_p]),
    "rd_conv3x3_bn_act_pair": (c_int, [c_void_p, c_int, c_void_p, c_void_p, c_void_p, c_int] * 2 +
                               [c_int, c_int, c_int, c_int, c_int, c_int, c_int, c_int, c_void_p]),
    "rd_conv2d_bn_act_head_out_pair": (c_int, [c_void_p, c_int, c_void_p, c_void_p, c_void_p, c_void_p, c_void_p, c_long, c_int] * 2 +
                                       [c_int, c_long, c_int, c_int, c_int, c_int, c_int, c_int, c_void_p]),
    "rd_head_out": (c_int, [c_void_p, c_int, c_int, c_void_p, c_void_p, c_void_p, c_long, c_long, c_int, c_int, c_int,
                            c_int, c_int, c_int, c_void_p]),
    "rd_meta_packed_bytes": (c_size_t, [c_int]),
    "rd_pack_meta_host": (c_int, [c_void_p] * 9 + [c_int, c_void_p]),
    "rd_meta_kernel_fwd": (c_int, [c_void_p, c_int, c_int, c_void_p, c_void_p, c_void_p, c_int, c_int, c_int, c_int,
                                   c_int, c_int, c_void_p]),
    "rd_sorted_foreground_workspace_bytes": (c_size_t, [c_long, c_long]),
    "rd_sorted_foreground": (c_int, [c_void_p, c_void_p, c_void_p, c_void_p, c_int, c_long, c_long, c_int, c_int,
                                     c_void_p, c_void_p, c_void_p, c_void_p, c_void_p, c_size_t, c_void_p]),
    "rd_decode3d_bbox": (c_int, [c_void_p, c_void_p, c_void_p, c_int, c_long, c_int, c_int, c_void_p]),
    "rd_score_filter_workspace_bytes": (c_size_t, [c_long]),
    "rd_score_filter_dets": (c_int, [c_void_p, c_void_p, c_long, c_float, c_void_p, c_void_p, c_void_p, c_size_t, c_void_p]),
    "rd_score_filter_dets_batched": (c_int, [c_void_p, c_long, c_void_p, c_long, c_long, c_float, c_void_p, c_long, c_void_p,
                                             c_void_p, c_size_t, c_int, c_void_p]),
    "rd_wnms_workspace_bytes": (c_size_t, [c_int]),
    "rd_wnms_4c_batched": (c_int, [c_void_p, c_long, c_int, c_void_p, c_void_p, c_long, c_int, c_float, c_float, c_int, c_int,
                                   c_void_p, c_long, c_void_p, c_long, c_void_p, c_void_p, c_size_t, c_int, c_void_p]),
    "rd_dets12_to_8_batched": (c_int, [c_void_p, c_long, c_int, c_void_p, c_void_p, c_long, c_int, c_void_p]),
    "rd_wnms_4c": (c_int, [c_void_p, c_int, c_void_p, c_void_p, c_int, c_float, c_float, c_int, c_int, c_void_p, c_void_p,
                           c_void_p, c_void_p, c_size_t, c_void_p]),
    "rd_single_overlap": (c_int, [c_void_p, c_void_p, c_long, c_int, c_void_p, c_void_p]),
    "rd_wnms_order_host": (c_int, [c_void_p, c_int, c_void_p]),
    "rd_edge_atan2f": (c_int, [c_void_p, c_void_p, c_long, c_void_p, c_void_p]),
    "rd_wnms_pair_skippable": (c_int, [c_void_p, c_void_p, c_long, c_void_p, c_void_p]),
    "rd_dets12_to_8": (c_int, [c_void_p, c_int, c_void_p, c_void_p, c_void_p]),
    "rd_rotated_iou_8pt": (c_int, [c_void_p, c_void_p, c_void_p, c_long, c_long, c_void_p]),
    "rd_batch_rotated_iou": (c_int, [c_void_p, c_int, c_void_p, c_void_p, c_void_p, c_int, c_long, c_int, c_void_p]),
    "rd_batch_rotated_iou_3d": (c_int, [c_void_p, c_int, c_void_p, c_void_p, c_void_p, c_int, c_long, c_int, c_void_p]),
    "rd_rotated_iou_7": (c_int, [c_void_p, c_void_p, c_void_p, c_long, c_long, c_void_p]),
    "rd_batch_max_iou": (c_int, [c_void_p, c_int, c_void_p, c_void_p, c_long, c_int, c_void_p]),
    "rd_gather_keep_scores": (c_int, [c_void_p, c_long, c_int, c_void_p, c_int, c_void_p, c_int, c_void_p]),
    "rd_nms3d_workspace_bytes": (c_size_t, [c_long, c_int]),
    "rd_nms3d": (c_int, [c_void_p, c_int, c_long, c_float, c_int, c_int, c_void_p, c_void_p, c_void_p, c_size_t, c_void_p]),
    "rd_assign3d_v2": (c_int, [c_void_p] * 6 + [c_long, c_int] + [c_float] * 7 + [c_void_p, c_void_p]),
    "rd_get_point_num_workspace_bytes": (c_size_t, []),
    "rd_get_point_num": (c_int, [c_void_p, c_long, c_void_p, c_void_p, c_size_t, c_void_p]),
    "rd_input_transform": (c_int, [c_void_p, c_void_p, c_void_p, c_void_p, c_int, c_int, c_int, c_int, c_int] + [c_void_p] * 8 + [c_void_p]),
    "rd_prof_enable": (c_int, [c_int]),
    "rd_prof_reset": (c_int, []),
    "rd_prof_get": (c_int, [c_int, ctypes.POINTER(ctypes.c_double), ctypes.POINTER(c_long)]),
}


class RangeDetError(RuntimeError):
    def __init__(self, code, msg):
        super().__init__("librangedet_hip error %d: %s" % (code, msg))
        self.code = code


def ptr(x):
    if x is None:
        return None
    if isinstance(x, int):
        return x
    if isinstance(x, np.ndarray):
        return x.ctypes.data
    if hasattr(x, "data_ptr"):
        return x.data_ptr()
    raise TypeError("cannot take the address of %r" % type(x))


class Lib:
    def __init__(self, path=DEFAULT_PATH):
        if not os.path.exists(path):
            raise RuntimeError(
                "%s not found: the HIP extension is not built (run `python -m rangedet_amd.build`). "
                "There is no CPU fallback." % path)
        self.path = path
        if os.path.basename(path).startswith("librangedet_hip"):
            try:
                import torch
            except ImportError:
                pass
        self.cdll = ctypes.CDLL(path)
        for name, (res, args) in SIGNATURES.items():
            fn = getattr(self.cdll, name)
            fn.restype = res
            fn.argtypes = args
        self.rd_last_error_string = self.cdll.rd_last_error_string

    def call(self, name, *args):
        rc = getattr(self.cdll, name)(*args)
        if rc < 0:
            raise RangeDetError(rc, self.cdll.rd_last_error_string().decode())
        return rc

    def raw(self, name):
        return getattr(self.cdll, name)

    def pack_conv_weight(self, w_oihw, dtype):
        w = np.ascontiguousarray(w_oihw, dtype=np.float32)
        cout, cin, kh, kw = w.shape
        out = np.zeros(self.cdll.rd_conv_packed_bytes(kh * kw, cin, cout, dtype), dtype=np.uint8)
        self.call("rd_pack_conv_weight_host", w.ctypes.data, cout, cin, kh, kw, dtype, out.ctypes.data)
        return out

    def pack_conv3x3_ex(self, w_oihw, stride_w, x_cstride, fold_scale=None, dtype=RD_BF16):
        w = np.ascontiguousarray(w_oihw, dtype=np.float32)
        cout, cin = w.shape[:2]
        assert w.shape[2:] == (3, 3)
        fs = None if fold_scale is None else np.ascontiguousarray(fold_scale, dtype=np.float32)
        out = np.zeros(self.cdll.rd_conv3x3_ex_packed_bytes(cin, cout, stride_w, x_cstride), dtype=np.uint8)
        self.call("rd_pack_conv3x3_ex_host", w.ctypes.data, None if fs is None else fs.ctypes.data, cout, cin, stride_w,
                  x_cstride, dtype, out.ctypes.data)
        return out

    def pack_conv3x3_m16(self, w_oihw, fold_scale, dtype=RD_BF16):
        w = np.ascontiguousarray(w_oihw, dtype=np.float32)
        cout, cin = w.shape[:2]
        assert w.shape[2:] == (3, 3)
        fs = np.ascontiguousarray(fold_scale, dtype=np.float32)
        out = np.zeros(self.cdll.rd_conv3x3_ex_packed_bytes(cin, cout, 1, cin), dtype=np.uint8)
        self.call("rd_pack_conv3x3_m16_host", w.ctypes.data, fs.ctypes.data, cout, cin, dtype, out.ctypes.data)
        return out

    def pack_conv3x3_cat(self, w_oihw, cin1, cin2, fold_scale=None, dtype=RD_BF16):
        w = np.ascontiguousarray(w_oihw, dtype=np.float32)
        cout = w.shape[0]
        assert w.shape[1:] == (cin1 + cin2, 3, 3)
        fs = None if fold_scale is None else np.ascontiguousarray(fold_scale, dtype=np.float32)
        out = np.zeros(self.cdll.rd_conv3x3_cat_packed_bytes(cin1, cin2, cout), dtype=np.uint8)
        self.call("rd_pack_conv3x3_cat_host", w.ctypes.data, None if fs is None else fs.ctypes.data, cout, cin1, cin2, dtype, out.ctypes.data)
        return out

    def pack_conv1x1_sc(self, w_oi, fold_scale=None, dtype=RD_BF16):
        w = np.ascontiguousarray(w_oi, dtype=np.float32).reshape(w_oi.shape[0], -1)
        cout, cin = w.shape
        fs = None if fold_scale is None else np.ascontiguousarray(fold_scale, dtype=np.float32)
        out = np.zeros(self.cdll.rd_conv1x1_sc_packed_bytes(cin, cout), dtype=np.uint8)
        self.call("rd_pack_conv1x1_sc_host", w.ctypes.data, None if fs is None else fs.ctypes.data, cout, cin, dtype, out.ctypes.data)
        return out

    def pack_block64(self, w1_oihw, scale1, w2_oihw, scale2, dtype=RD_BF16, m16=False):
        w1, w2 = (np.ascontiguousarray(w, dtype=np.float32) for w in (w1_oihw, w2_oihw))
        s1, s2 = (np.ascontiguousarray(v, dtype=np.float32) for v in (scale1, scale2))
        cin = w1.shape[1]
        assert w1.shape == (64, cin, 3, 3) and w2.shape == (64, 64, 3, 3) and s1.shape == (64,) and s2.shape == (64,)
        out = np.zeros(self.cdll.rd_block64_packed_bytes(cin), dtype=np.uint8)
        if m16:
            assert cin == 64
            self.call("rd_pack_block64_m16_host", w1.ctypes.data, s1.ctypes.data, w2.ctypes.data, s2.ctypes.data, dtype, out.ctypes.data)
        else:
            self.call("rd_pack_block64_host", w1.ctypes.data, s1.ctypes.data, w2.ctypes.data, s2.ctypes.data, cin, dtype, out.ctypes.data)
        return out

    def pack_conv1x1_sc_m16(self, w_oi, fold_scale, dtype=RD_BF16):
        w = np.ascontiguousarray(w_oi, dtype=np.float32).reshape(64, 64)
        fs = np.ascontiguousarray(fold_scale, dtype=np.float32)
        out = np.zeros(self.cdll.rd_conv1x1_sc_packed_bytes(64, 64), dtype=np.uint8)
        self.call("rd_pack_conv1x1_sc_m16_host", w.ctypes.data, fs.ctypes.data, dtype, out.ctypes.data)
        return out

    def pack_deconv_weight(self, w_iohw, stride_w, pad_w, phase, dtype, fold_scale=None):
        w = np.ascontiguousarray(w_iohw, dtype=np.float32)
        cin, cout, kh, kw = w.shape
        nt = self.cdll.rd_deconv_phase_taps(kh, kw, stride_w, pad_w, phase)
        if nt < 0:
            raise RangeDetError(nt, "deconv phase taps")
        out = np.zeros(self.cdll.rd_conv_packed_bytes(nt, cin, cout, dtype), dtype=np.uint8)
        fs = None if fold_scale is None else np.ascontiguousarray(fold_scale, dtype=np.float32)
        self.call("rd_pack_deconv_weight_folded_host", w.ctypes.data, None if fs is None else fs.ctypes.data, cin, cout, kh, kw,
                  stride_w, pad_w, phase, dtype, out.ctypes.data)
        return out

    def pack_deconv_phase_pair(self, img_a, img_b, cin, dtype):
        assert img_a.nbytes == img_b.nbytes
        out = np.empty(2 * img_a.nbytes, np.uint8)
        a, b = np.ascontiguousarray(img_a), np.ascontiguousarray(img_b)
        self.call("rd_pack_deconv_phase_pair_host", a.ctypes.data, b.ctypes.data, cin, dtype, out.ctypes.data)
        return out

    def pack_head_weight(self, w, dtype=RD_BF16, m16=False):
        w = np.ascontiguousarray(w, dtype=np.float32)
        out = np.zeros(self.cdll.rd_head_m16_packed_bytes() if m16 else self.cdll.rd_head_packed_bytes(), dtype=np.uint8)
        self.call("rd_pack_head_weight_m16_host" if m16 else "rd_pack_head_weight_host", w.ctypes.data, w.shape[0], w.shape[1], dtype, out.ctypes.data)
        return out

    def pack_meta(self, w0, b0, w1, b1, s1, t1, agg, s2, t2, dtype):
        arrs = [np.ascontiguousarray(a, dtype=np.float32) for a in (w0, b0, w1, b1, s1, t1, agg, s2, t2)]
        assert arrs[0].shape == (32, 3) and arrs[2].shape == (64, 32) and arrs[6].shape == (64, 576)
        out = np.zeros(self.cdll.rd_meta_packed_bytes(dtype), dtype=np.uint8)
        self.call("rd_pack_meta_host", *[a.ctypes.data for a in arrs], dtype, out.ctypes.data)
        return out

    def wnms_order_host(self, dets):
        d = np.ascontiguousarray(dets, dtype=np.float32).reshape(-1, 12)
        order = np.empty(d.shape[0], dtype=np.int32)
        self.call("rd_wnms_order_host", d.ctypes.data, d.shape[0], order.ctypes.data)
        return order

    def prof(self):
        out = {}
        ms, n = ctypes.c_double(), c_long()
        for k, v in PROF_KINDS.items():
            self.call("rd_prof_get", v, ctypes.byref(ms), ctypes.byref(n))
            out[k] = (ms.value, n.value)
        return out


_LIB = None


def get_lib():
    global _LIB
    if _LIB is None:
        _LIB = Lib(DEFAULT_PATH)
    return _LIB
```

Before: 1003.

## Schedule block64 tiles as vertical runs reusing carried conv1 rows

Replaces the fixed per-workgroup tile stride with a schedule of vertical runs of 8-row tiles, chosen on the host to minimise the maximum per-workgroup load. In the m16 path, later tiles in a run reuse the bottom two rows of the first conv's output kept in LDS, so they skip recomputing and refetching those halo rows. The run length is capped by an env switch that defaults to 1, so by default runs are single tiles and only the new scheduling logic is exercised. It also adds APIs to query and supply schedules, and adds decode overhead and complexity in the kernel loop.

New measurement: 972.1. 0.97x the previous value.

```diff
diff --git a/include/rangedet_hip.h b/include/rangedet_hip.h
--- a/include/rangedet_hip.h
+++ b/include/rangedet_hip.h
@@ -69,6 +69,11 @@
 int rd_pack_conv1x1_sc_m16_host(const float* w_oi_host, const float* fold_scale_host, int dtype, void* packed_host);
 int rd_block64_m16_bn_act(const void* x, int x_cstride, int x_coff, const void* w_packed, const float* shift1, const float* shift2,
                           const void* sc_w_packed, void* y, int y_cstride, int y_coff, int B, int H, int W, int dtype, void* stream);
+int rd_block64_schedule_host(int B, int H, int W, int slots, int max_len, int* run_strips, long long* max_units, long long* total_units);
+int rd_block64_schedule_runs_host(int B, int H, int W, int slots, const int* run_strips, int cap, int* runs_out);
+int rd_block64_m16_bn_act_runs(const void* x, int x_cstride, int x_coff, const void* w_packed, const float* shift1, const float* shift2,
+                               const void* sc_w_packed, void* y, int y_cstride, int y_coff, int B, int H, int W, int dtype, const int* run_strips,
+                               void* stream);
 
 size_t rd_head_packed_bytes(void);
 int rd_pack_head_weight_host(const float* w, int nout, int cin, int dtype, void* out_host);
diff --git a/rangedet_amd/csrc/k_block.h b/rangedet_amd/csrc/k_block.h
--- a/rangedet_amd/csrc/k_block.h
+++ b/rangedet_amd/csrc/k_block.h
@@ -1,9 +1,34 @@
 #pragma once
+#include <array>
+#include <map>
 #include "k_conv3.h"
 
 namespace rd {
 
+constexpr int BK_STRIP = 8, BK_NPH = 4;
+struct BlockSched {
+  int len[BK_NPH], runs[BK_NPH], s0[BK_NPH];
+  int nitems;
+};
+struct BlockRun { int ct, b, rb, len; };
+__host__ __device__ __forceinline__ bool bk_run_decode(const BlockSched& s, int ncol, int nrow, int B, int xcd, int item, BlockRun& r) {
+  const int e0 = s.runs[0], e1 = e0 + s.runs[1], e2 = e1 + s.runs[2];
+  const int p = (item >= e0 ? 1 : 0) + (item >= e1 ? 1 : 0) + (item >= e2 ? 1 : 0);
+  const int rho = item - (p == 0 ? 0 : p == 1 ? e0 : p == 2 ? e1 : e2);
+  const int L = p == 0 ? s.len[0] : p == 1 ? s.len[1] : p == 2 ? s.len[2] : s.len[3];
+  const int s0 = p == 0 ? s.s0[0] : p == 1 ? s.s0[1] : p == 2 ? s.s0[2] : s.s0[3];
+  const int rps = BK_STRIP / L, q = xcd ? rho >> 3 : rho;
+  const int strip = s0 + (xcd ? 8 * (q / rps) + (rho & 7) : q / rps), part = q % rps;
+  const int ncs = ncol * B, sv = strip / ncs, cs = strip - sv * ncs;
+  r.b = cs / ncol;
+  r.ct = cs - r.b * ncol;
+  r.rb = sv * BK_STRIP + part * L;
+  r.len = nrow - r.rb < L ? nrow - r.rb : L;
+  return r.len > 0;
+}
+
 struct BlockArgs {
+  BlockSched sched;
   const bf16_t* x; int x_cs, x_co; long x_bs;
   const unsigned char* w;
   const float* shift1; const float* shift2;
@@ -21,6 +46,10 @@
 constexpr int BK_TP = 34;
 constexpr int BK_SLAB = 4096;
 constexpr size_t BK_LDS = 2 * BK_BUF + BK_R * BK_SLAB;
+constexpr int BK_CARRY = BK_BUF - 2 * BK_TP * 64;
+constexpr int BK_XLAST_LATER = 22;
+static_assert((BK_XLAST_LATER + 1) * 1024 <= BK_CARRY && (BK_XLAST_LATER + 1) * 16 >= 10 * BK_XP, "a later tile's x chunk ends below the carried rows");
+__host__ __device__ constexpr int bk_later_base(int wave) { return wave < 2 ? 80 * wave : 32 + 64 * wave; }
 
 constexpr int bk_nsteps(bool first) { return first ? 23 : 36; }
 constexpr int bk_unit(bool first, int g) { return first ? (g < 5 ? 0 : g < 14 ? 2 : 3) : g / 9; }
@@ -67,8 +96,6 @@
   }
 
   const int G = gridDim.x, wg = blockIdx.x;
-  const int ntl = (a.ntiles - wg + G - 1) / G;
-  const int tiles_img = a.ncol * a.nrow;
 
 #if defined(__HIP_DEVICE_COMPILE__)
   const unsigned lds0 = __builtin_amdgcn_readfirstlane((unsigned)(uintptr_t)(__attribute__((address_space(3))) void*)smem);
@@ -90,54 +117,71 @@
 #endif
   };
 
-  const int xdq = (G >> 3) / a.nrow;
-  const int g_ct = a.xcd ? (8 * xdq) % a.ncol : G % a.ncol, g_rb = a.xcd ? (G >> 3) % a.nrow : (G / a.ncol) % a.nrow,
-            g_b = a.xcd ? (8 * xdq) / a.ncol : G / tiles_img;
-  const int g_ct1 = (8 * xdq + 8) % a.ncol, g_b1 = (8 * xdq + 8) / a.ncol;
-  auto tile_advance = [&](int& ct, int& rb, int& b) __attribute__((always_inline)) {
-    int& d0 = a.xcd ? rb : ct;
-    int& d1 = a.xcd ? ct : rb;
-    const int r0 = a.xcd ? a.nrow : a.ncol, r1 = a.xcd ? a.ncol : a.nrow;
-    d0 += a.xcd ? g_rb : g_ct;
-    const int c1 = d0 >= r0 ? 1 : 0;
-    d0 -= c1 ? r0 : 0;
-    d1 += a.xcd ? (c1 ? g_ct1 : g_ct) : g_rb + c1;
-    const int c2 = d1 >= r1 ? 1 : 0;
-    d1 -= c2 ? r1 : 0;
-    b += (a.xcd && c1 ? g_b1 : g_b) + c2;
+  struct Cur { int item, ct, b, rb, left; bool first, valid; };
+  auto cur_seek = [&](Cur& c) __attribute__((always_inline)) {
+    BlockRun r;
+    c.valid = false;
+    while (c.item < a.sched.nitems) {
+      if (bk_run_decode(a.sched, a.ncol, a.nrow, a.B, a.xcd, c.item, r)) {
+        c.ct = r.ct; c.b = r.b; c.rb = r.rb; c.left = r.len; c.first = true; c.valid = true;
+        break;
+      }
+      c.item += G;
+    }
+    c.item = __builtin_amdgcn_readfirstlane(c.item); c.ct = __builtin_amdgcn_readfirstlane(c.ct); c.b = __builtin_amdgcn_readfirstlane(c.b);
+    c.rb = __builtin_amdgcn_readfirstlane(c.rb); c.left = __builtin_amdgcn_readfirstlane(c.left);
+    c.first = __builtin_amdgcn_readfirstlane((int)c.first) != 0; c.valid = __builtin_amdgcn_readfirstlane((int)c.valid) != 0;
   };
-  const int xs0 = ((wg >> 3) / a.nrow) * 8 + (wg & 7);
-  int f_ct = a.xcd ? xs0 % a.ncol : wg % a.ncol, f_rb = a.xcd ? (wg >> 3) % a.nrow : (wg / a.ncol) % a.nrow,
-      f_b = a.xcd ? xs0 / a.ncol : wg / tiles_img;
-  int c_ct = f_ct, c_rb = f_rb, c_b = f_b;
-
-  int hk = 0, hc = 0;
+  auto cur_next = [&](Cur& c) __attribute__((always_inline)) {
+    if (c.left > 1) { --c.left; ++c.rb; c.first = false; }
+    else { c.item += G; cur_seek(c); }
+    c.rb = __builtin_amdgcn_readfirstlane(c.rb); c.left = __builtin_amdgcn_readfirstlane(c.left);
+    c.first = __builtin_amdgcn_readfirstlane((int)c.first) != 0;
+  };
+  Cur fcur = {wg, 0, 0, 0, 0, true, false};
+  cur_seek(fcur);
+  if (!fcur.valid) return;
+  Cur ccur = fcur;
+
+  int hc = 0;
   int hh0 = 0, hw0 = 0;
+  bool hlater = false;
   const unsigned char* htile = nullptr;
   const unsigned char* hbase = nullptr;
   bool hnew = true;
   auto halo_begin = [&]() {
     if (hnew) {
-      hh0 = f_rb * 8 - 2; hw0 = f_ct * 32 - 2;
-      htile = (const unsigned char*)(a.x + (size_t)f_b * a.x_bs + a.x_co) + ((long)hh0 * a.W + hw0) * (long)a.x_cs * 2;
+      hlater = M16 && !fcur.first;
+      hh0 = fcur.rb * 8 - (hlater ? 0 : 2); hw0 = fcur.ct * 32 - 2;
+      htile = (const unsigned char*)(a.x + (size_t)fcur.b * a.x_bs + a.x_co) + ((long)hh0 * a.W + hw0) * (long)a.x_cs * 2;
       hnew = false;
     }
     hbase = htile + hc * 64;
     if (!FIRST && hc == 0) hc = 1;
-    else if (hk + 1 < ntl) { ++hk; hc = 0; tile_advance(f_ct, f_rb, f_b); hnew = true; }
+    else {
+      Cur n = fcur;
+      cur_next(n);
+      if (n.valid) { fcur = n; hc = 0; hnew = true; }
+    }
   };
   auto halo_piece = [&](int buf, int j) {
-    const int q = wave * BK_XPIECES + j;
+    const int q0 = wave * BK_XPIECES + j, q = hlater && q0 > BK_XLAST_LATER ? BK_XLAST_LATER : q0;
     int ol = lane;
     asm volatile("" : "+v"(ol));
     const int pp = 16 * q + (ol >> 2), r = (pp * 1821) >> 16, cc = pp - BK_XP * r;
     const int hs = (ol & 3) ^ ((ol >> 4) & 3);
-    const bool ok = pp < 12 * BK_XP && (unsigned)(hh0 + r) < (unsigned)a.H && (unsigned)(hw0 + cc) < (unsigned)a.W && (!FIRST || hs < a.nslots1);
+    const bool ok = pp < (hlater ? 10 : 12) * BK_XP && (unsigned)(hh0 + r) < (unsigned)a.H && (unsigned)(hw0 + cc) < (unsigned)a.W && (!FIRST || hs < a.nslots1);
     const unsigned char* src = hbase + (long)((r * a.W + cc) * a.x_cs * 2 + hs * 16);
     dma_v(ok ? (const void*)src : (const void*)a.zero16, buf + q * 1024);
   };
   int fslot = 0, fslab = 0;
-  auto slab_piece = [&]() { dma_s(a.w + (size_t)fslab * SLAB + wave * 1024, lane * 16, RING + fslot * SLAB + wave * 1024); };
+  auto slab_piece = [&]() {
+    const int sl = __builtin_amdgcn_readfirstlane(fslab), so = __builtin_amdgcn_readfirstlane(fslot);
+    const uintptr_t wp = (uintptr_t)a.w;
+    const unsigned wlo = __builtin_amdgcn_readfirstlane((unsigned)wp), whi = __builtin_amdgcn_readfirstlane((unsigned)((unsigned long long)wp >> 32));
+    const unsigned char* wb = (const unsigned char*)(uintptr_t)(((unsigned long long)whi << 32) | wlo);
+    dma_s(wb + (size_t)sl * SLAB + wave * 1024, lane * 16, RING + so * SLAB + wave * 1024);
+  };
   auto slab_advance = [&]() {
     fslot = fslot + 1 == R ? 0 : fslot + 1;
     fslab = fslab + 1 == bk_nsteps(FIRST) ? 0 : fslab + 1;
@@ -284,12 +328,16 @@
     slab_advance();                                                                                                \
     rslot = rnext_;                                                                                                \
   }
-#define BK_C1M(U_, S_)                                                                                             \
-  BK_STEP16(6, 9 * (U_) + (S_), BK_BUF, (((U_) == 1 && (S_) == 8) ? 0 : 6), 2048,                                  \
-            ((S_) == 8 ? a1[0][0] + BK_BUF : a1[(((S_) + 1) % 9) / 3][((S_) + 1) % 3] + (U_) * BK_BUF))
+#define BK_C1M(F_, D_, U_, S_)                                                                                     \
+  BK_STEP16(F_, 9 * (U_) + (S_), BK_BUF, (((U_) == 1 && (S_) == 8) ? 0 : (F_)), 2048,                              \
+            ((S_) == 8 ? a1[0][0] + BK_BUF : a1[(((S_) + 1) % 9) / 3][((S_) + 1) % 3] + (U_) * BK_BUF) + (D_))
+#define BK_C1M18(F_, D_)                                                                                           \
+  BK_C1M(F_, D_, 0, 0) BK_C1M(F_, D_, 0, 1) BK_C1M(F_, D_, 0, 2) BK_C1M(F_, D_, 0, 3) BK_C1M(F_, D_, 0, 4) BK_C1M(F_, D_, 0, 5)     \
+  BK_C1M(F_, D_, 0, 6) BK_C1M(F_, D_, 0, 7) BK_C1M(F_, D_, 0, 8) BK_C1M(F_, D_, 1, 0) BK_C1M(F_, D_, 1, 1) BK_C1M(F_, D_, 1, 2)     \
+  BK_C1M(F_, D_, 1, 3) BK_C1M(F_, D_, 1, 4) BK_C1M(F_, D_, 1, 5) BK_C1M(F_, D_, 1, 6) BK_C1M(F_, D_, 1, 7) BK_C1M(F_, D_, 1, 8)
 #define BK_C2M(C_, S_)                                                                                             \
   BK_STEP16(4, 18 + 9 * (C_) + (S_), 0, (((C_) == 1 && (S_) == 8) ? 6 : 4), (((C_) == 1 && (S_) == 8) ? 2048 : ROWB2), \
-            ((S_) == 8 ? ((C_) == 1 ? a1[0][0] : a2[0] + BK_BUF) : a2[((S_) + 1) % 3] + ((((S_) + 1) % 9) / 3) * ROWB2 + (C_) * BK_BUF))
+            ((S_) == 8 ? ((C_) == 1 ? a1[0][0] + dnext : a2[0] + BK_BUF) : a2[((S_) + 1) % 3] + ((((S_) + 1) % 9) / 3) * ROWB2 + (C_) * BK_BUF))
 
   halo_begin();
 #pragma unroll
@@ -308,7 +356,7 @@
   for (int kk = 0; kk < 3 + NCT; ++kk) BK_RD(3, 2048, 0, kk, a1[0][0], boff + rslot * SLAB, 0)
   }
 
-  for (int k = 0; k < ntl; ++k) {
+  while (ccur.valid) {
     if constexpr (M16) {
       unsigned z0 = 0u, b1 = bz1m, b2 = bz2m;
       int oq = lane >> 4;
@@ -334,36 +382,59 @@
           }
         BK_FENCE();
       };
-      init_acc(b1, 6);
-      BK_C1M(0, 0) BK_C1M(0, 1) BK_C1M(0, 2) BK_C1M(0, 3) BK_C1M(0, 4) BK_C1M(0, 5) BK_C1M(0, 6) BK_C1M(0, 7) BK_C1M(0, 8)
-      BK_C1M(1, 0) BK_C1M(1, 1) BK_C1M(1, 2) BK_C1M(1, 3) BK_C1M(1, 4) BK_C1M(1, 5) BK_C1M(1, 6) BK_C1M(1, 7) BK_C1M(1, 8)
-      const int ct = c_ct, rb = c_rb, b = c_b;
-      tile_advance(c_ct, c_rb, c_b);
-      {
-        int el = lane;
-        asm volatile("" : "+v"(el));
-        const int en = el & 15, eq = el >> 4;
-#pragma unroll
-        for (int h = 0; h < 6; ++h) {
-          const int J = 96 * wave + 16 * h + en, rr = (J * 1821) >> 16, cc = J - BK_XP * rr;
-          const bool keep = cc < BK_TP && rr < 10;
-          const bool inside = (unsigned)(rb * 8 - 1 + rr) < (unsigned)a.H && (unsigned)(ct * 32 - 1 + cc) < (unsigned)a.W;
-          const int doff = (rr * BK_TP + cc) * 64 + (((eq ^ (cc >> 2)) & 3) << 4);
-#pragma unroll
-          for (int j = 0; j < 2; ++j) {
-            BK_FENCE();
-            unsigned pk[4];
-#pragma unroll
-            for (int w2 = 0; w2 < 4; ++w2) {
-              const f32x4 av = acc6[h][2 * j + (w2 >> 1)];
-              unsigned p2 = H16<DT>::pk(av[2 * (w2 & 1)], av[2 * (w2 & 1) + 1]);
-              p2 = __builtin_bit_cast(unsigned, __builtin_elementwise_max(__builtin_bit_cast(s16x2, p2), (s16x2){0, 0}));
-              pk[w2] = inside ? p2 : 0u;
-            }
-            if (keep) *(Slot16*)(smem + j * BK_BUF + doff) = Slot16{pk[0], pk[1], pk[2], pk[3]};
-          }
-        }
-      }
+      const int ct = ccur.ct, rb = ccur.rb, b = ccur.b;
+      const bool later = !ccur.first;
+      cur_next(ccur);
+      const bool carry_out = ccur.valid && !ccur.first;
+      const int dlater = (bk_later_base(wave) - 96 * wave) * 64;
+      const int dnext = carry_out ? dlater : 0;
+#define BK_TWRITE(NH_, JB_, LATER_)                                                                                \
+      {                                                                                                            \
+        int el = lane;                                                                                             \
+        asm volatile("" : "+v"(el));                                                                               \
+        const int en = el & 15, eq = el >> 4;                                                                      \
+        _Pragma("unroll") for (int h = 0; h < (NH_); ++h) {                                                        \
+          const int J = (JB_) + 16 * h + en, rq = (J * 1821) >> 16, cc = J - BK_XP * rq, rr = rq + ((LATER_) ? 2 : 0); \
+          const bool keep = cc < BK_TP && rr < 10;                                                                 \
+          const bool inside = (unsigned)(rb * 8 - 1 + rr) < (unsigned)a.H && (unsigned)(ct * 32 - 1 + cc) < (unsigned)a.W; \
+          const int sw = ((eq ^ (cc >> 2)) & 3) << 4;                                                              \
+          const int doff = (rr * BK_TP + cc) * 64 + sw;                                                            \
+          const bool crow = keep && rr >= 8;                                                                       \
+          const int coff = BK_CARRY + ((rr - 8) * BK_TP + cc) * 64 + sw;                                           \
+          _Pragma("unroll") for (int j = 0; j < 2; ++j) {                                                          \
+            BK_FENCE();                                                                                            \
+            unsigned pk[4];                                                                                        \
+            _Pragma("unroll") for (int w2 = 0; w2 < 4; ++w2) {                                                     \
+              const f32x4 av = acc6[h][2 * j + (w2 >> 1)];                                                         \
+              unsigned p2 = H16<DT>::pk(av[2 * (w2 & 1)], av[2 * (w2 & 1) + 1]);                                   \
+              p2 = __builtin_bit_cast(unsigned, __builtin_elementwise_max(__builtin_bit_cast(s16x2, p2), (s16x2){0, 0})); \
+              pk[w2] = inside ? p2 : 0u;                                                                           \
+            }                                                                                                      \
+            if (keep) *(Slot16*)(smem + j * BK_BUF + doff) = Slot16{pk[0], pk[1], pk[2], pk[3]};                   \
+            if (crow) {                                                                                            \
+              if (LATER_) {                                                                                        \
+                const Slot16 up = *(const Slot16*)(smem + j * BK_BUF + coff);                                      \
+                *(Slot16*)(smem + j * BK_BUF + doff - 8 * ROWB2) = up;                                             \
+              }                                                                                                    \
+              if (carry_out) *(Slot16*)(smem + j * BK_BUF + coff) = Slot16{pk[0], pk[1], pk[2], pk[3]};            \
+            }                                                                                                      \
+          }                                                                                                        \
+        }                                                                                                          \
+      }
+      if (!later) {
+        init_acc(b1, 6);
+        BK_C1M18(6, 0)
+        BK_TWRITE(6, 96 * wave, false)
+      } else if (wave < 2) {
+        init_acc(b1, 5);
+        BK_C1M18(5, dlater)
+        BK_TWRITE(5, 80 * wave, true)
+      } else {
+        init_acc(b1, 4);
+        BK_C1M18(4, dlater)
+        BK_TWRITE(4, 32 + 64 * wave, true)
+      }
+#undef BK_TWRITE
       init_acc(b2, 4);
       BK_SYNC(63, 0)
 #pragma unroll
@@ -377,7 +448,7 @@
         int el = lane;
         asm volatile("" : "+v"(el));
         const int en = el & 15, eq = el >> 4;
-        unsigned char* scr = smem + BK_BUF + wave * (BK_BUF / 4);
+        unsigned char* scr = smem + BK_BUF + wave * 4096;
         bf16_t* __restrict__ yrow0 = a.y + (size_t)b * a.y_bs + (size_t)oh0 * a.W * a.y_cs + a.y_co;
         const bf16_t* __restrict__ rimg0 = a.x + (size_t)b * a.x_bs + a.x_co;
         if constexpr (SC) {
@@ -471,8 +542,8 @@
       BK_C1(1, 0) BK_C1(1, 1) BK_C1(1, 2) BK_C1(1, 3) BK_C1(1, 4) BK_C1(1, 5) BK_C1(1, 6) BK_C1(1, 7) BK_C1(1, 8)
     }
 
-    const int ct = c_ct, rb = c_rb, b = c_b;
-    tile_advance(c_ct, c_rb, c_b);
+    const int ct = ccur.ct, rb = ccur.rb, b = ccur.b;
+    cur_next(ccur);
     {
       int em = m, ehi = hi;
       asm volatile("" : "+v"(em), "+v"(ehi));
@@ -595,6 +666,7 @@
   }
   __builtin_amdgcn_s_waitcnt(RD_VMCNT_IMM(0));
 #undef BK_C2M
+#undef BK_C1M18
 #undef BK_C1M
 #undef BK_STEP16
 #undef BK_MM16
@@ -640,8 +712,74 @@
                  [&](int co, int ci, int t) { return (s2 ? s2[co] : 1.f) * w2[((size_t)co * 64 + ci) * 9 + t]; }, dt);
 }
 
+constexpr int BK_UNITS_FIRST = 20, BK_UNITS_LATER = 17;
+inline int bk_nstrips(int ncol, int nrow, int B) { return ncol * B * ((nrow + BK_STRIP - 1) / BK_STRIP); }
+inline BlockSched bk_make_sched(const int strips[BK_NPH]) {
+  BlockSched s;
+  int s0 = 0;
+  s.nitems = 0;
+  for (int p = 0; p < BK_NPH; ++p) {
+    s.len[p] = BK_STRIP >> p; s.s0[p] = s0; s.runs[p] = strips[p] * (1 << p);
+    s0 += strips[p]; s.nitems += s.runs[p];
+  }
+  return s;
+}
+inline bool bk_sched_valid(const int strips[BK_NPH], int ncol, int nrow, int B, int xcd) {
+  int n = 0;
+  for (int p = 0; p < BK_NPH; ++p) {
+    if (strips[p] < 0 || (xcd && strips[p] % 8)) return false;
+    n += strips[p];
+  }
+  return n == bk_nstrips(ncol, nrow, B);
+}
+inline void bk_sched_units(const BlockSched& s, int ncol, int nrow, int B, int xcd, int grid, long* max_units, long* total_units) {
+  std::vector<long> load((size_t)grid, 0);
+  long tot = 0, mx = 0;
+  BlockRun r;
+  for (int i = 0; i < s.nitems; ++i)
+    if (bk_run_decode(s, ncol, nrow, B, xcd, i, r)) {
+      const long u = BK_UNITS_FIRST + (long)BK_UNITS_LATER * (r.len - 1);
+      load[(size_t)(i % grid)] += u;
+      tot += u;
+    }
+  for (long v : load) mx = std::max(mx, v);
+  *max_units = mx; *total_units = tot;
+}
+inline void bk_pick_strips(int ncol, int nrow, int B, int xcd, int grid, int max_len, int strips[BK_NPH]) {
+  const int ns = bk_nstrips(ncol, nrow, B), step = xcd ? 8 : 1;
+  long best_m = -1, best_t = -1;
+  for (int pa = 0; pa < BK_NPH; ++pa) {
+    if ((BK_STRIP >> pa) > max_len) continue;
+    for (int pb = pa; pb < BK_NPH; ++pb)
+      for (int na = pb == pa ? ns : step; na <= (pb == pa ? ns : ns - step); na += step) {
+        int c[BK_NPH] = {0, 0, 0, 0};
+        c[pa] = na;
+        c[pb] += ns - na;
+        long m, t;
+        bk_sched_units(bk_make_sched(c), ncol, nrow, B, xcd, grid, &m, &t);
+        if (best_m < 0 || m < best_m || (m == best_m && t < best_t)) { best_m = m; best_t = t; memcpy(strips, c, sizeof(c)); }
+      }
+  }
+}
+inline BlockSched bk_pick_sched(int ncol, int nrow, int B, int xcd, int grid, int max_len) {
+  static std::mutex mu;
+  static std::map<std::array<int, 6>, BlockSched> cache;
+  const std::array<int, 6> key = {ncol, nrow, B, xcd, grid, max_len};
+  std::lock_guard<std::mutex> lk(mu);
+  auto it = cache.find(key);
+  if (it != cache.end()) return it->second;
+  int strips[BK_NPH];
+  bk_pick_strips(ncol, nrow, B, xcd, grid, max_len, strips);
+  return cache[key] = bk_make_sched(strips);
+}
+inline void bk_launch_geometry(int B, int H, int W, int slots, int* ncol, int* nrow, int* grid, int* xcd) {
+  *ncol = (W + 31) / 32; *nrow = (H + 7) / 8;
+  *grid = std::min(*ncol * *nrow * B, slots);
+  *xcd = dev_switches().conv_xcd && (*ncol * B) % 8 == 0 && *grid % 8 == 0;
+}
+
 inline int launch_block64(const void* x, int x_cs, int x_co, int cin, const void* w, const float* shift1, const float* shift2, const void* sc_w,
-                          void* y, int y_cs, int y_co, int B, int H, int W, int dt, hipStream_t st, bool m16 = false) {
+                          void* y, int y_cs, int y_co, int B, int H, int W, int dt, hipStream_t st, bool m16 = false, const int* run_strips = nullptr) {
   RD_REQUIRE(is_h16(dt), RD_EINVAL, "block64: dtype %d (RD_BF16 or RD_F16)", dt);
   const bool first = block64_first(cin);
   RD_REQUIRE(!m16 || !first, RD_ESHAPE, "block64: the 16 x 16 x 32 form takes 64 input channels");
@@ -655,9 +793,13 @@
   a.zero16 = (const unsigned char*)w + block64_body_bytes(cin);
   a.H = H; a.W = W; a.B = B;
   a.nslots1 = std::min(2, (x_cs - x_co) / 8);
-  a.ncol = (W + 31) / 32; a.nrow = (H + 7) / 8; a.ntiles = a.ncol * a.nrow * B;
-  const int grid = std::min(a.ntiles, conv_num_cus() * 2);
-  a.xcd = dev_switches().conv_xcd && (a.ncol * B) % 8 == 0 && grid % 8 == 0;
+  int grid;
+  bk_launch_geometry(B, H, W, conv_num_cus() * 2, &a.ncol, &a.nrow, &grid, &a.xcd);
+  a.ntiles = a.ncol * a.nrow * B;
+  RD_REQUIRE(!run_strips || (m16 && bk_sched_valid(run_strips, a.ncol, a.nrow, B, a.xcd)), RD_EINVAL,
+             "block64: run schedule (strips per run length 8, 4, 2, 1: non-negative, %d in all%s; the 16 x 16 x 32 form)", bk_nstrips(a.ncol, a.nrow, B),
+             a.xcd ? ", multiples of 8" : "");
+  a.sched = run_strips ? bk_make_sched(run_strips) : bk_pick_sched(a.ncol, a.nrow, B, a.xcd, grid, m16 ? dev_switches().block_runs : 1);
   ProfScope ps(RD_PROF_BLOCK, st);
   static std::atomic<unsigned long long> seen{0};
   once_per_device(seen, [] {
diff --git a/rangedet_amd/csrc/rd_api.hip b/rangedet_amd/csrc/rd_api.hip
--- a/rangedet_amd/csrc/rd_api.hip
+++ b/rangedet_amd/csrc/rd_api.hip
@@ -347,6 +347,49 @@
   RD_REQUIRE(y_cstride % 8 == 0 && y_coff % 8 == 0 && y_coff >= 0 && y_coff + 64 <= y_cstride, RD_ESHAPE, "block64_m16: y channel stride / offset");
   RD_REQUIRE(x != y, RD_EINVAL, "block64_m16: in-place (a tile's halo is another tile's output)");
   return launch_block64(x, x_cstride, x_coff, 64, w_packed, shift1, shift2, sc_w_packed, y, y_cstride, y_coff, B, H, W, dtype, (hipStream_t)stream, true);
+}
+
+int rd_block64_m16_bn_act_runs(const void* x, int x_cstride, int x_coff, const void* w_packed, const float* shift1, const float* shift2,
+                               const void* sc_w_packed, void* y, int y_cstride, int y_coff, int B, int H, int W, int dtype, const int* run_strips,
+                               void* stream) {
+  RD_REQUIRE(x && w_packed && shift1 && shift2 && y && run_strips, RD_EINVAL, "block64_m16_runs: null pointer");
+  RD_REQUIRE(is_h16(dtype), RD_EINVAL, "block64_m16_runs: dtype %d (RD_BF16 or RD_F16)", dtype);
+  RD_REQUIRE(B > 0 && H > 0 && W > 0, RD_ESHAPE, "block64_m16_runs: shape");
+  RD_REQUIRE(x_cstride % 8 == 0 && x_coff % 8 == 0 && x_coff >= 0 && x_coff + 64 <= x_cstride, RD_ESHAPE, "block64_m16_runs: x channel stride / offset");
+  RD_REQUIRE(y_cstride % 8 == 0 && y_coff % 8 == 0 && y_coff >= 0 && y_coff + 64 <= y_cstride, RD_ESHAPE, "block64_m16_runs: y channel stride / offset");
+  RD_REQUIRE(x != y, RD_EINVAL, "block64_m16_runs: in-place (a tile's halo is another tile's output)");
+  return launch_block64(x, x_cstride, x_coff, 64, w_packed, shift1, shift2, sc_w_packed, y, y_cstride, y_coff, B, H, W, dtype, (hipStream_t)stream, true, run_strips);
+}
+
+int rd_block64_schedule_host(int B, int H, int W, int slots, int max_len, int* run_strips, long long* max_units, long long* total_units) {
+  RD_REQUIRE(run_strips, RD_EINVAL, "block64_schedule: null pointer");
+  RD_REQUIRE(B > 0 && H > 0 && W > 0 && slots > 0, RD_ESHAPE, "block64_schedule: shape");
+  RD_REQUIRE(max_len == 1 || max_len == 2 || max_len == 4 || max_len == 8, RD_EINVAL, "block64_schedule: longest run %d (1, 2, 4 or 8)", max_len);
+  int ncol, nrow, grid, xcd;
+  bk_launch_geometry(B, H, W, slots, &ncol, &nrow, &grid, &xcd);
+  bk_pick_strips(ncol, nrow, B, xcd, grid, max_len, run_strips);
+  long m, t;
+  bk_sched_units(bk_make_sched(run_strips), ncol, nrow, B, xcd, grid, &m, &t);
+  if (max_units) *max_units = m;
+  if (total_units) *total_units = t;
+  return RD_OK;
+}
+int rd_block64_schedule_runs_host(int B, int H, int W, int slots, const int* run_strips, int cap, int* runs_out) {
+  RD_REQUIRE(run_strips && (runs_out || cap == 0), RD_EINVAL, "block64_schedule_runs: null pointer");
+  RD_REQUIRE(B > 0 && H > 0 && W > 0 && slots > 0, RD_ESHAPE, "block64_schedule_runs: shape");
+  int ncol, nrow, grid, xcd;
+  bk_launch_geometry(B, H, W, slots, &ncol, &nrow, &grid, &xcd);
+  RD_REQUIRE(bk_sched_valid(run_strips, ncol, nrow, B, xcd), RD_EINVAL, "block64_schedule_runs: strips per run length (non-negative, %d in all%s)",
+             bk_nstrips(ncol, nrow, B), xcd ? ", multiples of 8" : "");
+  const BlockSched s = bk_make_sched(run_strips);
+  BlockRun r;
+  int n = 0;
+  for (int i = 0; i < s.nitems; ++i)
+    if (bk_run_decode(s, ncol, nrow, B, xcd, i, r)) {
+      if (n < cap) { int* o = runs_out + 5 * (size_t)n; o[0] = i % grid; o[1] = r.b; o[2] = r.ct; o[3] = r.rb; o[4] = r.len; }
+      ++n;
+    }
+  return n;
 }
 
 size_t rd_conv3x3_cat_packed_bytes(int cin1, int cin2, int cout) { return conv_packed_bytes(9, cin1 + cin2, cout, RD_BF16); }
diff --git a/rangedet_amd/csrc/rd_common.h b/rangedet_amd/csrc/rd_common.h
--- a/rangedet_amd/csrc/rd_common.h
+++ b/rangedet_amd/csrc/rd_common.h
@@ -51,8 +51,9 @@
   bool wnms_scan1;
   int wnms_ct;
   bool wnms_no_skip;
-};
-constexpr DevSwitches kDevSwitchDefaults = {false, 1, 2, 1, 1, 1, 1, 1, false, false, 0, false, 8, false};
+  int block_runs;
+};
+constexpr DevSwitches kDevSwitchDefaults = {false, 1, 2, 1, 1, 1, 1, 1, false, false, 0, false, 8, false, 1};
 #ifdef RD_DEV_SWITCHES
 inline const DevSwitches& dev_switches() {
   static const DevSwitches s = [] {
@@ -72,6 +73,7 @@
     d.wnms_scan1 = getenv("RD_WNMS_SCAN1") != nullptr;
     d.wnms_no_skip = getenv("RD_WNMS_NO_SKIP") != nullptr;
     d.wnms_bal = num("RD_WNMS_BAL", 0);
+    d.block_runs = num("RD_BLOCK_RUNS", 1);
     return d;
   }();
   return s;
diff --git a/rangedet_amd/lib.py b/rangedet_amd/lib.py
--- a/rangedet_amd/lib.py
+++ b/rangedet_amd/lib.py
@@ -70,6 +70,10 @@
     "rd_pack_conv1x1_sc_m16_host": (c_int, [c_void_p, c_void_p, c_int, c_void_p]),
     "rd_block64_m16_bn_act": (c_int, [c_void_p, c_int, c_int, c_void_p, c_void_p, c_void_p, c_void_p, c_void_p, c_int, c_int, c_int, c_int,
                                       c_int, c_int, c_void_p]),
+    "rd_block64_schedule_host": (c_int, [c_int, c_int, c_int, c_int, c_int, c_void_p, c_void_p, c_void_p]),
+    "rd_block64_schedule_runs_host": (c_int, [c_int, c_int, c_int, c_int, c_void_p, c_int, c_void_p]),
+    "rd_block64_m16_bn_act_runs": (c_int, [c_void_p, c_int, c_int, c_void_p, c_void_p, c_void_p, c_void_p, c_void_p, c_int, c_int, c_int, c_int,
+                                           c_int, c_int, c_void_p, c_void_p]),
     "rd_block64_bn_act": (c_int, [c_void_p, c_int, c_int, c_int, c_void_p, c_void_p, c_void_p, c_void_p, c_void_p, c_int, c_int, c_int, c_int,
                                   c_int, c_int, c_void_p]),
     "rd_head_packed_bytes": (c_size_t, []),
```
